# JuliaLinearAlgebra/AlgebraicMultigrid.jl

Measured on AMD Instinct MI355X. Metric: V-cycle unknowns/sec + fine-level SpMV GB/s (% HBM peak), 3-D Poisson 256^3, higher is better.
Workload: dtype f64

## Files before the change

__graft_entry__.py:

```python
import os
import subprocess
import sys

ROOT = os.path.dirname(os.path.abspath(__file__))
PKG = os.path.join(ROOT, "algebraicmultigrid.jl_amd")
if ROOT not in sys.path:
    sys.path.insert(0, ROOT)

HIPCC = os.environ.get("HIPCC", "/opt/rocm/bin/hipcc")
HIP_FLAGS = ["--offload-arch=gfx950", "-O3", "-std=c++17", "-ffp-contract=off", "-fPIC", "-shared",
             "-pthread", "-Wall", "-Wno-unused-value", "-Wno-unused-result"] + os.environ.get("AMGH_EXTRA_HIP_FLAGS", "").split()
CXX_FLAGS = ["-O3", "-std=c++17", "-fopenmp", "-fPIC", "-shared", "-Wall", "-Wextra"]


def _stale(out, srcs):
    if not os.path.exists(out):
        return True
    t = os.path.getmtime(out)
    return any(os.path.getmtime(s) > t for s in srcs)


def build(only_missing=False):
    hip_src = [os.path.join(PKG, "csrc", "hip", f) for f in ("amghip.hip", "amghip_kernels.hpp", "amghip_internal.hpp",
                                                             "gs_schedule.hpp", "csr_ops.hpp")]
    hip_src.append(os.path.join(PKG, "csrc", "hip", "amghip_dist.hpp"))
    hip_src.append(os.path.join(PKG, "csrc", "hip", "amghip_ipc.hpp"))
    hip_src.append(os.path.join(PKG, "csrc", "hip", "amghip_setup.hpp"))
    hip_src.append(os.path.join(PKG, "csrc", "hip", "dev_scan.hpp"))
    hip_src.append(os.path.join(PKG, "csrc", "hip", "gs_merge_dev.hpp"))
    hip_src.append(os.path.join(PKG, "csrc", "hip", "gs_blocks.hpp"))
    hip_src.append(os.path.join(PKG, "csrc", "hip", "gs_flow.hpp"))
    hip_src.append(os.path.join(PKG, "csrc", "hip", "gs_relay.hpp"))
    hip_src.append(os.path.join(PKG, "csrc", "hip", "gmres_kernels.hpp"))
    hip_src.append(os.path.join(PKG, "csrc", "hip", "pcg_block_kernels.hpp"))
    hip_src.append(os.path.join(PKG, "csrc", "hip", "chebyshev.hpp"))
    hip_src.append(os.path.join(PKG, "csrc", "hip", "dist_pcg_kernels.hpp"))
    hip_src.append(os.path.join(ROOT, "include", "amghip.h"))
    hip_out = os.path.join(PKG, "libamghip.so")
    if _stale(hip_out, hip_src) and not (only_missing and os.path.exists(hip_out) and not os.path.exists(HIPCC)):
        extra = os.environ.get("AMGH_EXTRA_HIP_FLAGS", "").split()
        if extra:
            for tool in ("flow_asm_audit.py", "flow_asm_linear.py"):
                r = subprocess.run([sys.executable, os.path.join(ROOT, "tools", tool)], env=dict(os.environ, AUDIT_HIP_FLAGS=" ".join(extra)),
                                   stdout=subprocess.PIPE, stderr=subprocess.STDOUT)
                if r.returncode != 0:
                    raise RuntimeError("AMGH_EXTRA_HIP_FLAGS=%r: tools/%s does not pass with these flags:\n%s" % (" ".join(extra), tool, r.stdout.decode(errors="replace")[-2000:]))
        subprocess.check_call([HIPCC] + HIP_FLAGS + [hip_src[0], "-o", hip_out])
    f32_out = os.path.join(PKG, "libamghip_f32.so")
    if _stale(f32_out, hip_src) and not (only_missing and os.path.exists(f32_out) and not os.path.exists(HIPCC)):
        subprocess.check_call([HIPCC] + HIP_FLAGS + ["-DAMGH_REAL=float", "-DAMGH_NO_SETUP", hip_src[0], "-o", f32_out])
    set_src = [os.path.join(PKG, "csrc", "setup", "amg_setup.cpp"), os.path.join(ROOT, "include", "amgsetup.h")]
    set_out = os.path.join(PKG, "libamgsetup.so")
    if _stale(set_out, set_src):
        subprocess.check_call(["g++"] + CXX_FLAGS + [set_src[0], "-o", set_out])
    tool_src = os.path.join(ROOT, "tools", "spmv_bench.hip")
    tool_out = os.path.join(ROOT, "tools", "spmv_bench")
    if os.path.exists(tool_src) and _stale(tool_out, [tool_src, hip_src[1]]) and os.path.exists(HIPCC):
        subprocess.check_call([HIPCC, "--offload-arch=gfx950", "-O3", "-std=c++17", "-ffp-contract=off", tool_src,
                               "-o", tool_out])
    from oracle import oracle as O
    O.build()
    import amg_amd
    amg_amd.setup_lib()
    amg_amd.hip_lib()
    amg_amd.hip_lib("float32")


def smoke():
    import numpy as np
    build(only_missing=True)
    import amg_amd as AMG
    from oracle import oracle as O
    if not AMG.gpu_available():
        raise RuntimeError("smoke(): no HIP device visible")
    A = AMG.poisson((24, 24, 24))
    b = A @ np.ones(A.m)
    ml = AMG.ruge_stuben(A)
    x, hist = AMG._solve(ml, b, log=True)
    xo, ho, _ = O.OracleHierarchy(ml).solve(b)
    err = np.linalg.norm(x - xo) / np.linalg.norm(xo)
    assert len(hist) == len(ho) and err < 1e-10, (len(hist), len(ho), err)
    jac = AMG.Jacobi(2.0 / 3.0)
    ml2 = AMG.smoothed_aggregation(AMG.poisson((64, 64)), presmoother=jac, postsmoother=jac)
    r = np.linspace(0.0, 1.0, ml2.levels[0].A.m)
    z = AMG.aspreconditioner(ml2).ldiv(r)
    zo = O.OracleHierarchy(ml2).precond(r)
    err2 = np.linalg.norm(z - zo) / np.linalg.norm(zo)
    assert err2 < 1e-10, err2
    print(f"smoke ok: RS/GS solve {len(hist) - 1} cycles rel.err {err:.2e}; SA/Jacobi ldiv rel.err {err2:.2e}")


if __name__ == "__main__":
    build()
    if len(sys.argv) > 1 and sys.argv[1] == "smoke":
        smoke()
```

algebraicmultigrid.jl_amd/_libs.py:

```python
import ctypes as C
import os

_HERE = os.path.dirname(os.path.abspath(__file__))
SETUP_SO = os.path.join(_HERE, "libamgsetup.so")
HIP_SO = os.path.join(_HERE, "libamghip.so")
HIP_F32_SO = os.path.join(_HERE, "libamghip_f32.so")

i32p = C.POINTER(C.c_int32)
f64p = C.POINTER(C.c_double)
i64 = C.c_int64
vp = C.c_void_p


class AMGError(RuntimeError):
    pass


class amgs_options(C.Structure):
    _fields_ = [("theta", C.c_double), ("max_levels", C.c_int32), ("max_coarse", C.c_int32),
                ("hermitian", C.c_int32), ("sa_omega", C.c_double), ("sa_improve_iters", C.c_int32),
                ("sa_B_is_vector", C.c_int32)]


class amgh_smoother_t(C.Structure):
# ... 11 lines not shown

def setup_lib():
    global _setup
    if _setup is not None:
        return _setup
    if not os.path.exists(SETUP_SO):
        raise AMGError(f"{SETUP_SO} not built: run `python -c 'import __graft_entry__ as g; g.build()'`")
    L = C.CDLL(SETUP_SO)
    L.amgs_last_error.restype = C.c_char_p
    L.amgs_set_threads.argtypes = [C.c_int]
    L.amgs_set_threads_here.argtypes = [C.c_int]
    L.amgs_mat_create.restype = vp
    L.amgs_mat_create.argtypes = [i64, i64, vp, vp, vp]
    L.amgs_mat_alloc.restype = vp
    L.amgs_mat_alloc.argtypes = [i64, i64, i64]
    L.amgs_mat_free.argtypes = [vp]
    for f in ("amgs_mat_rows", "amgs_mat_cols", "amgs_mat_nnz"):
        getattr(L, f).restype = i64
        getattr(L, f).argtypes = [vp]
    for f in ("amgs_mat_colptr", "amgs_mat_rowval", "amgs_mat_nzval"):
        getattr(L, f).restype = vp
        getattr(L, f).argtypes = [vp]
    L.amgs_mat_transpose.restype = vp
    L.amgs_mat_transpose.argtypes = [vp]
    L.amgs_mat_spgemm.restype = vp
    L.amgs_mat_spgemm.argtypes = [vp, vp]
    L.amgs_mat_is_symmetric.argtypes = [vp]
    L.amgs_poisson.restype = vp
    L.amgs_poisson.argtypes = [C.c_int, C.POINTER(i64)]
    L.amgs_classical_strength.argtypes = [vp, C.c_double, C.POINTER(vp), C.POINTER(vp)]
    L.amgs_symmetric_strength.restype = vp
    L.amgs_symmetric_strength.argtypes = [vp, C.c_double, C.c_int]
    L.amgs_rs_splitting.argtypes = [vp, vp]
    L.amgs_rs_cf_splitting_patterns.argtypes = [i64, vp, vp, vp, vp, vp]
    L.amgs_direct_interpolation.restype = vp
    L.amgs_direct_interpolation.argtypes = [vp, vp, vp]
    L.amgs_standard_aggregation.restype = vp
    L.amgs_standard_aggregation.argtypes = [vp]
    L.amgs_fit_candidates.restype = vp
    L.amgs_fit_candidates.argtypes = [vp, vp, C.c_int, C.c_int, C.c_double, C.POINTER(vp), C.POINTER(i64)]
    L.amgs_jacobi_prolongation.restype = vp
    L.amgs_jacobi_prolongation.argtypes = [vp, vp, C.c_double]
    L.amgs_improve_candidates.argtypes = [vp, vp, C.c_int, C.c_int]
    L.amgs_free.argtypes = [vp]
    L.amgs_default_options_rs.argtypes = [C.POINTER(amgs_options)]
    L.amgs_default_options_sa.argtypes = [C.POINTER(amgs_options)]
    L.amgs_ruge_stuben.restype = vp
    L.amgs_ruge_stuben.argtypes = [vp, C.POINTER(amgs_options)]
    L.amgs_smoothed_aggregation.restype = vp
    L.amgs_smoothed_aggregation.argtypes = [vp, vp, C.c_int, C.POINTER(amgs_options)]
    L.amgs_hier_free.argtypes = [vp]
    L.amgs_hier_num_levels.argtypes = [vp]
    L.amgs_hier_get.restype = vp
    L.amgs_hier_get.argtypes = [vp, C.c_int, C.c_int]
    _setup = L
    return L


def _bind_solve_phase(L, creal, coarse_fn):
    L.amgh_strerror.restype = C.c_char_p
    L.amgh_strerror.argtypes = [C.c_int]
    L.amgh_create.argtypes = [C.POINTER(vp), C.c_int, C.c_int]
    L.amgh_destroy.argtypes = [vp]
    L.amgh_destroy.restype = None
    L.amgh_push_level.argtypes = [vp, i64, i64] + [vp] * 12 + [C.POINTER(amgh_smoother_t), C.POINTER(amgh_smoother_t)]
    L.amgh_push_level_begin.argtypes = [vp, i64] + [vp] * 6 + [C.POINTER(amgh_smoother_t), C.POINTER(amgh_smoother_t)]
    L.amgh_push_level_end.argtypes = [vp, i64] + [vp] * 6
    L.amgh_push_level_abort.argtypes = [vp]
    L.amgh_level_prepare.argtypes = [C.c_int, i64] + [vp] * 6 + [C.POINTER(amgh_smoother_t), C.POINTER(amgh_smoother_t), C.POINTER(vp)]
    L.amgh_level_prepare_nrhs.argtypes = [C.c_int, C.c_int, i64] + [vp] * 6 + [C.POINTER(amgh_smoother_t), C.POINTER(amgh_smoother_t), C.POINTER(vp)]
    L.amgh_push_level_prepared.argtypes = [vp, vp]
    L.amgh_level_free.argtypes = [vp]
    L.amgh_level_free.restype = None
    L.amgh_set_coarse.argtypes = [vp, i64, vp, vp, vp, vp]
    L.amgh_set_coarse_host.argtypes = [vp, i64, vp, vp, vp, coarse_fn, vp]
    L.amgh_finalize.argtypes = [vp]
    L.amgh_set_chebyshev_bounds.argtypes = [vp, C.c_int, C.c_int, C.c_double, C.c_double, C.c_int]
    L.amgh_chebyshev_bounds.argtypes = [vp, C.c_int, C.c_int, f64p, f64p]
    L.amgh_chebyshev_coefficients.argtypes = [C.c_int, C.c_double, C.c_double, vp]
    L.amgh_level_spectral_radius.argtypes = [vp, C.c_int, C.c_int, f64p]
    L.amgh_csr_spectral_radius.argtypes = [vp, C.c_int, f64p, vp]
    L.amgh_csr_chebyshev_d.argtypes = [vp, C.c_int, C.c_double, C.c_double, vp, vp, vp, vp]
    L.amgh_num_levels.argtypes = [vp]
    L.amgh_tail_dense_build.argtypes = [vp, C.c_int]
    L.amgh_tail_dense_info.argtypes = [vp, C.c_int, C.POINTER(C.c_int), C.POINTER(i64), C.POINTER(C.c_double)]
    L.amgh_level_size.restype = i64
    L.amgh_level_size.argtypes = [vp, C.c_int]
    L.amgh_device_bytes.restype = i64
    L.amgh_device_bytes.argtypes = [vp]
    L.amgh_device_bytes_detail.argtypes = [vp, vp]
    L.amgh_gs_num_dependency_levels.argtypes = [vp, C.c_int]
    L.amgh_gs_num_sweep_steps.argtypes = [vp, C.c_int, C.c_int]
    L.amgh_gs_sweep_stats.argtypes = [vp, C.c_int, C.c_int, vp]
    solve_args = [vp, vp, vp, C.c_int, C.c_int, C.c_double, C.c_double, C.c_int, vp, C.POINTER(C.c_int)]
    L.amgh_solve.argtypes = solve_args
    L.amgh_solve_d.argtypes = solve_args
    L.amgh_precond_apply.argtypes = [vp, vp, vp, C.c_int]
    L.amgh_precond_apply_d.argtypes = [vp, vp, vp, C.c_int]
    pcg_args = [vp, vp, vp, C.c_int, C.c_int, C.c_int, C.c_double, C.c_double, vp, C.POINTER(C.c_int)]
    L.amgh_pcg.argtypes = pcg_args
    L.amgh_pcg_d.argtypes = pcg_args
    gmres_args = [vp, vp, vp, C.c_int, C.c_int, C.c_int, C.c_int, C.c_double, C.c_double, vp, C.POINTER(C.c_int)]
    L.amgh_gmres.argtypes = gmres_args
    L.amgh_gmres_d.argtypes = gmres_args
    L.amgh_debug_gmres_reorth.argtypes = [vp]
    pcg_block_args = [vp, vp, vp, C.c_int, C.c_int, C.c_int, C.c_double, C.c_double, vp, C.c_int, vp]
    L.amgh_pcg_block.argtypes = pcg_block_args
    L.amgh_pcg_block_d.argtypes = pcg_block_args
    L.amgh_level_spmv.argtypes = [vp, C.c_int, C.c_int, vp, vp]
    L.amgh_level_spmv_d.argtypes = [vp, C.c_int, C.c_int, vp, vp]
    L.amgh_level_residual_d.argtypes = [vp, C.c_int, vp, vp, vp]
    L.amgh_level_smooth.argtypes = [vp, C.c_int, C.c_int, vp, vp]
    L.amgh_level_smooth_d.argtypes = [vp, C.c_int, C.c_int, vp, vp]
    L.amgh_debug_level_smooth_block_d.argtypes = [vp, C.c_int, C.c_int, vp, vp]
    L.amgh_csr_create.argtypes = [C.POINTER(vp), C.c_int, i64, i64, vp, vp, vp]
    L.amgh_csr_destroy.argtypes = [vp]
    L.amgh_csr_destroy.restype = None
    L.amgh_csr_prepare.argtypes = [vp, C.c_int, C.c_int]
    L.amgh_csr_spmv_d.argtypes = [vp, vp, vp, vp]
    L.amgh_csr_residual_d.argtypes = [vp, vp, vp, vp, vp]
    L.amgh_csr_spmv_add_d.argtypes = [vp, vp, vp, vp]
    L.amgh_csr_jacobi_d.argtypes = [vp, C.c_double, vp, vp, vp, vp]
    L.amgh_csr_gs_d.argtypes = [vp, C.c_int, C.c_double, C.c_int, vp, vp, vp]
    L.amgh_csr_gs_ex_d.argtypes = [vp, C.c_int, C.c_double, C.c_int, vp, vp, vp, C.c_int]
    L.amgh_gather_d.argtypes = [C.c_int, i64, vp, vp, vp, vp]
    L.amgh_dot_d.argtypes = [C.c_int, i64, vp, vp, vp, C.POINTER(creal), vp]
    L.amgh_cycle_d.argtypes = [vp, C.c_int, vp, vp, C.c_int]
    L.amgh_set_stream.argtypes = [vp, vp]
    L.amgh_dev_alloc.argtypes = [C.c_int, i64, C.POINTER(vp)]
    L.amgh_dev_free.argtypes = [C.c_int, vp]
    L.amgh_dev_upload.argtypes = [C.c_int, vp, vp, i64]
    L.amgh_dev_download.argtypes = [C.c_int, vp, vp, i64]
    L.amgh_dev_sync.argtypes = [C.c_int]
    L.amgh_stream.restype = vp
    L.amgh_stream.argtypes = [vp]
    L.amgh_timer_begin.argtypes = [vp]
    L.amgh_timer_end.argtypes = [vp, C.POINTER(C.c_double)]
    L.amgh_bench_op.argtypes = [vp, C.c_int, C.c_int, C.c_int, C.c_int, C.POINTER(C.c_double)]
    L.amgh_debug_chain_timing.argtypes = [C.c_int, vp]
    L.amgh_debug_merged_sweep_host.argtypes = [i64, i64, vp, vp, vp, C.c_int, C.c_int, C.c_double, vp, vp]
    L.amgh_debug_bw_poll_giveups.argtypes = [vp, C.c_int]
    L.amgh_debug_bw_mode.argtypes = [vp, C.c_int]
    L.amgh_debug_bw_dict.argtypes = [vp, C.c_int]
    L.amgh_debug_bw_late.argtypes = [vp, C.c_int]
    L.amgh_debug_coded_ops.argtypes = [vp, C.c_int]
    L.amgh_debug_set_sell_stream.argtypes = [C.c_int, i64, C.c_int]
    L.amgh_debug_sell_stream_launches.argtypes = [vp, C.c_int, C.c_int]
    L.amgh_debug_sell_stream_padded.argtypes = [vp, C.c_int, C.c_int]
    L.amgh_debug_sell_stream_padded.restype = i64
    L.amgh_debug_csr_sell.argtypes = [vp, C.c_int]
    L.amgh_debug_csr_sell.restype = i64
    L.amgh_debug_csr_sell_launches.argtypes = [vp]
    L.amgh_debug_csr_sell_apply.argtypes = [vp, C.c_int, vp, vp, vp]
    L.amgh_debug_bw_sweep_host.argtypes = [i64, vp, vp, vp, C.c_int, C.c_int, C.c_double, vp, vp, vp]
    L.amgh_debug_bw_dict_sweep_host.argtypes = [i64, vp, vp, vp, C.c_int, C.c_int, vp, vp, vp]
    L.amgh_debug_set_tunable.argtypes = [C.c_char_p, C.c_int]
    L.amgh_debug_get_tunable.argtypes = [C.c_char_p, C.POINTER(C.c_int)]
    L.amgh_profile_enable.argtypes = [vp, C.c_int]
    L.amgh_profile_read.argtypes = [vp, vp, C.c_int]
    L.amgh_set_use_graph.argtypes = [vp, C.c_int]


def _bind_dist(L):
    i64p = C.POINTER(i64)
    L.amgh_dist_rccl_available.argtypes = []
    L.amgh_dist_unique_id.argtypes = [vp]
    L.amgh_dist_create_rccl.argtypes = [C.POINTER(vp), C.c_int, C.c_int, C.c_int, vp]
    L.amgh_local_group_create.argtypes = [C.POINTER(vp), C.c_int]
    L.amgh_local_group_destroy.argtypes = [vp]
    L.amgh_local_group_destroy.restype = None
    L.amgh_local_group_abort.argtypes = [vp]
    L.amgh_local_group_abort.restype = None
    L.amgh_dist_create_local.argtypes = [C.POINTER(vp), C.c_int, C.c_int, vp]
    L.amgh_dist_create_ipc.argtypes = [C.POINTER(vp), C.c_int, C.c_int, C.c_int, C.c_char_p]
    L.amgh_dist_destroy.argtypes = [vp]
    L.amgh_dist_destroy.restype = None
    L.amgh_dist_push_level.argtypes = [vp, i64, i64, vp, vp] + [vp] * 12 + [C.POINTER(amgh_smoother_t),
                                                                            C.POINTER(amgh_smoother_t)]
    L.amgh_dist_set_tail.argtypes = [vp, vp]
    L.amgh_dist_set_host_tail.argtypes = [vp, vp, vp]
    L.amgh_dist_finalize.argtypes = [vp]
    L.amgh_dist_set_gs_mode.argtypes = [vp, C.c_int]
    L.amgh_dist_gs_pipelined.argtypes = [vp, C.c_int]
    L.amgh_dist_pipe_serialized.argtypes = [vp]
    L.amgh_dist_pipe_protocol_failed.argtypes = [vp]
    L.amgh_dist_num_sharded_levels.argtypes = [vp]
    L.amgh_dist_local_range.argtypes = [vp, C.c_int, i64p, i64p]
    L.amgh_dist_precond_apply_d.argtypes = [vp, vp, vp, C.c_int]
    L.amgh_dist_solve_d.argtypes = [vp, vp, vp, C.c_int, C.c_int, C.c_double, C.c_double, C.c_int, vp, C.POINTER(C.c_int)]
    L.amgh_dist_pcg_d.argtypes = [vp, vp, vp, C.c_int, C.c_int, C.c_int, C.c_double, C.c_double, vp, C.POINTER(C.c_int)]
    L.amgh_dist_spmv_d.argtypes = [vp, C.c_int, vp, vp]
    L.amgh_dist_sync.argtypes = [vp]
    L.amgh_dist_barrier.argtypes = [vp]
    L.amgh_dist_allreduce.argtypes = [vp, vp, C.c_int, C.c_int]
    L.amgh_dist_stats.argtypes = [vp, vp, C.c_int]
    L.amgh_dist_device_bytes.restype = i64
    L.amgh_dist_device_bytes.argtypes = [vp]
    L.amgh_dist_stream.restype = vp
    L.amgh_dist_stream.argtypes = [vp]
    L.amgh_dist_plan_info.argtypes = [vp, C.c_int, vp, vp, vp, vp, vp]
    L.amgh_dist_plan_info2.argtypes = [vp, C.c_int, C.c_int, vp, vp, vp, vp, vp]


def hip_lib(dtype=None):
    global _hip
    if dtype is not None and _np_dtype(dtype).itemsize == 4:
        return hip_lib_f32()
    if _hip is not None:
        return _hip
    if not os.path.exists(HIP_SO):
        raise AMGError(f"{HIP_SO} not built: run `python -c 'import __graft_entry__ as g; g.build()'` "
                       "(the solve phase has no CPU fallback)")
    L = C.CDLL(HIP_SO)
    L.real_dtype = "float64"
    _bind_solve_phase(L, C.c_double, COARSE_FN)
    _bind_dist(L)
    L.amgh_dmat_upload.argtypes = [C.POINTER(vp), C.c_int, i64, i64, vp, vp, vp]
    L.amgh_dmat_download.argtypes = [vp, vp, vp, vp]
    L.amgh_dmat_free.argtypes = [vp]
    L.amgh_dmat_free.restype = None
    for f in ("amgh_dmat_rows", "amgh_dmat_cols", "amgh_dmat_nnz"):
        getattr(L, f).restype = i64
        getattr(L, f).argtypes = [vp]
    L.amgh_setup_transpose.argtypes = [vp, C.POINTER(vp)]
    L.amgh_dmat_equal.argtypes = [vp, vp, C.POINTER(C.c_int)]
    L.amgh_setup_classical_strength.argtypes = [vp, C.c_double, C.POINTER(vp), C.POINTER(vp), C.POINTER(vp), C.POINTER(vp)]
    L.amgh_setup_symmetric_strength.restype = C.c_int
    L.amgh_setup_symmetric_strength.argtypes = [vp, C.c_double, C.c_int, C.POINTER(vp)]
    L.amgh_setup_fit_candidates_vector.restype = C.c_int
    L.amgh_setup_fit_candidates_vector.argtypes = [vp, vp, C.c_double, C.POINTER(vp), vp]
    L.amgh_setup_direct_interpolation.argtypes = [vp, vp, vp, C.POINTER(vp), C.POINTER(vp)]
    L.amgh_setup_spgemm.argtypes = [vp, vp, C.POINTER(vp)]
    L.amgh_setup_jacobi_prolongation.argtypes = [vp, vp, C.c_double, C.POINTER(vp)]
    _hip = L
    return L


def _np_dtype(dtype):
    import numpy as np
    return np.dtype(dtype)


def hip_lib_f32():
    global _hip_f32
    if _hip_f32 is not None:
        return _hip_f32
    if not os.path.exists(HIP_F32_SO):
        raise AMGError(f"{HIP_F32_SO} not built: run `python -c 'import __graft_entry__ as g; g.build()'` "
                       "(the solve phase has no CPU fallback)")
    L = C.CDLL(HIP_F32_SO)
    L.real_dtype = "float32"
    _bind_solve_phase(L, C.c_float, COARSE_FN_F32)
    _bind_dist(L)
    _hip_f32 = L
    return L


def hip_check(rc, what=""):
    if rc != 0:
        msg = hip_lib().amgh_strerror(rc).decode()
        raise AMGError(f"libamghip: {what}: {msg} (rc={rc})")


def gpu_available():
    try:
        return hip_lib().amgh_device_count() > 0
    except (AMGError, OSError):
        return False
```

algebraicmultigrid.jl_amd/csrc/hip/amghip.hip:

```cpp
#include "amghip_internal.hpp"
#include "gs_schedule.hpp"
#include "csr_ops.hpp"
#include "chebyshev.hpp"
#include "gmres_kernels.hpp"
#include "pcg_block_kernels.hpp"
#include "dist_pcg_kernels.hpp"

namespace {

constexpr int64_t kGraphAutoRows = 65536;

struct Level {
  int64_t n = 0, nc = 0;
  amgh_csr A, S, P, R;
  bool has_S = false;
  amgh_smoother_t pre{}, post{};
  real *res = nullptr, *cx = nullptr, *cb = nullptr, *tmp = nullptr;
  real* cheb_d = nullptr;
  ChebSide cheb[2];
  const ChebSide& cheb_of(const amgh_smoother_t& s) const { return &s == &post ? cheb[1] : cheb[0]; }
  real* il = nullptr;
  amgh_csr* smat() { return has_S ? &S : &A; }
  amgh_csr Pp, Rp;
  bool lo_ok = false;
// ... 1178 lines not shown
  if ((post ? L->post : L->pre).kind != AMGH_SMOOTH_CHEBYSHEV) return AMGH_EINVAL;
  if (lo) *lo = L->cheb[post].lo;
  if (hi) *hi = L->cheb[post].hi;
  return AMGH_OK;
}

int amgh_chebyshev_coefficients(int degree, double lo, double hi, double* c1c2) {
  if (degree < 1 || degree > kChebMaxDegree || !c1c2 || !cheb_bounds_valid(lo, hi)) return AMGH_EINVAL;
  cheb_coefficients(degree, lo, hi, c1c2);
  return AMGH_OK;
}

int amgh_level_spectral_radius(amgh_t* h, int level, int steps, double* rho) {
  RC_TRY(check_ready(h));
  if (level < 0 || level >= (int)h->levels.size() || !rho || steps < 0) return AMGH_EINVAL;
  HIP_TRY(hipSetDevice(h->device));
  amgh_csr* M = h->levels[level]->smat();
  if (!M->rowptr || !M->col || !M->val) return AMGH_EINVAL;
  return csr_spectral_radius(M, steps ? steps : kLanczosSteps, 0, h->stream, rho);
}

int amgh_csr_spectral_radius(amgh_csr_t* op, int steps, double* rho, void* stream) {
  if (!op || !rho || steps < 0) return AMGH_EINVAL;
  HIP_TRY(hipSetDevice(op->device));
  return csr_spectral_radius(op, steps ? steps : kLanczosSteps, 0, (hipStream_t)stream, rho);
}

int amgh_csr_chebyshev_d(amgh_csr_t* op, int degree, double lo, double hi, real* x_d, const real* b_d, real* work_d, void* stream) {
  if (!op || !x_d || !b_d || !work_d || op->nrows != op->ncols) return AMGH_EINVAL;
  if (degree < 1 || degree > kChebMaxDegree || !cheb_bounds_valid(lo, hi)) return AMGH_EINVAL;
  HIP_TRY(hipSetDevice(op->device));
  hipStream_t st = (hipStream_t)stream;
  RC_TRY(csr_ensure_coded(op, st));
  double c[2 * kChebMaxDegree];
  cheb_coefficients(degree, lo, hi, c);
  const int64_t n = op->nrows;
  real *xc = x_d, *xo = work_d, *d = work_d + n;
  for (int k = 0; k < degree; ++k) {
    RC_TRY(csr_chebyshev(op, (real)c[2 * k], (real)c[2 * k + 1], k == 0, xc, b_d, d, xo, st));
    std::swap(xc, xo);
  }
  if (xc != x_d) HIP_TRY(hipMemcpyAsync(x_d, xc, sizeof(real) * n, hipMemcpyDeviceToDevice, st));
  return AMGH_OK;
}

int amgh_finalize(amgh_t* h) {
  if (!h) return AMGH_EINVAL;
  if (h->finalized || h->ncoarse < 0 || h->pending_level) return AMGH_ESTATE;
  if (h->levels.empty() && !h->has_finalA) return AMGH_ESTATE;
  HIP_TRY(hipSetDevice(h->device));
  for (Level* L : h->levels)
    if (L->pre.kind == AMGH_SMOOTH_CHEBYSHEV || L->post.kind == AMGH_SMOOTH_CHEBYSHEV) RC_TRY(level_chebyshev_setup(h, L));
  int64_t ws = 0;
  h->tail_level = -2;
  if (g_tail_dense_rows > 0 && !h->coarse_fn)
    for (size_t l = 0; l < h->levels.size(); ++l)
      if (h->levels[l]->n <= g_tail_dense_rows) { h->tail_level = (int)l; break; }
  if (h->tail_level >= 0) {
    h->tail_cols = 64;
    h->tail_lo = h->tail_level >= 1 && h->levels[h->tail_level - 1]->coarse_lo;
  }
  for (size_t l = 0; l < h->levels.size(); ++l) {
    Level* L = h->levels[l];
    const int64_t wc = (h->tail_level >= 0 && (int)l >= h->tail_level) ? std::max(h->nrhs, h->tail_cols) : h->nrhs;
    RC_TRY(dev_alloc(&L->res, L->n * wc));
    RC_TRY(dev_alloc(&L->cx, L->nc * wc));
    RC_TRY(dev_alloc(&L->cb, L->nc * wc));
    ws += kRealB * (L->n + 2 * L->nc) * wc;
    if (h->nrhs == 2 || h->nrhs == 4 || h->nrhs == 8 || h->nrhs == 16) {
      RC_TRY(dev_alloc(&L->il, std::max(L->n, L->nc) * h->nrhs));
      ws += kRealB * std::max(L->n, L->nc) * h->nrhs;
    }
    const bool cheb = L->pre.kind == AMGH_SMOOTH_CHEBYSHEV || L->post.kind == AMGH_SMOOTH_CHEBYSHEV;
    if (L->pre.kind == AMGH_SMOOTH_JACOBI || L->post.kind == AMGH_SMOOTH_JACOBI || cheb) {
      RC_TRY(dev_alloc(&L->tmp, L->n * wc));
      ws += kRealB * L->n * wc;
      RC_TRY(csr_ensure_diag(L->smat(), h->stream));
    }
    if (cheb) {
      RC_TRY(dev_alloc(&L->cheb_d, L->n * wc));
      ws += kRealB * L->n * wc;
    }
  }
  for (Level* L : h->levels) {
    GsSchedule* g = L->smat()->gs;
    if (!L->lo_ok || !g || g->nblk != 0 || !g->rowptr || g->compacted) continue;
    RC_TRY(code_values(g->col, L->lo_val ? L->lo_val : g->val, L->n, g->ncols, g->nnz, &L->lo_cc, h->stream));
    RC_TRY(code_values(L->Rp.col, L->Rp.val, L->Rp.nrows, L->Rp.ncols, L->Rp.nnz, &L->Rp.cc, h->stream));
    RC_TRY(code_values(L->Pp.col, L->Pp.val, L->Pp.nrows, L->Pp.ncols, L->Pp.nnz, &L->Pp.cc, h->stream));
    ws += L->lo_cc.bytes + L->Rp.cc.bytes + L->Pp.cc.bytes;
    if (L->il && il_block(h->nrhs) && g_rhs_il == 1) {
      const int bs = h->nrhs;
      const int64_t n = L->n, nc = L->nc;
      auto timed = [&](auto&& fn, double* ms) -> int {
        hipEvent_t e0, e1;
        if (hipEventCreate(&e0) != hipSuccess) return -1001;
        if (hipEventCreate(&e1) != hipSuccess) { hipEventDestroy(e0); return -1001; }
        int rc = fn();
        if (rc == AMGH_OK && hipEventRecord(e0, h->stream) != hipSuccess) rc = -1001;
        for (int r = 0; r < 2 && rc == AMGH_OK; ++r) rc = fn();
        float t = 0.f;
        if (rc == AMGH_OK && (hipEventRecord(e1, h->stream) != hipSuccess || hipEventSynchronize(e1) != hipSuccess ||
                              hipEventElapsedTime(&t, e0, e1) != hipSuccess)) rc = -1001;
        hipEventDestroy(e0); hipEventDestroy(e1);
        *ms = t;
        return rc;
      };
      if (L->Rp.cc.ccol) {
        double t_il = 0, t_st = 0;
        RC_TRY(hipMemsetAsync(L->res, 0, sizeof(real) * n * bs, h->stream) == hipSuccess ? AMGH_OK : -1001);
        RC_TRY(timed([&] { return il_apply(bs, false, L->Rp.rowptr, L->Rp.col, L->Rp.val, nc, L->res, n, n, L->il, L->cb, nc, h->stream, &L->Rp.cc); }, &t_il));
        RC_TRY(timed([&] { return csr_apply(&L->Rp, M_SPMV, L->res, nullptr, L->cb, h->stream, bs); }, &t_st));
        L->r_stream = t_st < 0.95 * t_il;
        if (getenv("AMGH_VERBOSE")) fprintf(stderr, "[amghip] n=%lld restriction of %d columns: interleaved %.3f ms, column by column %.3f ms\n", (long long)n, bs, t_il / 2, t_st / 2);
      }
      if (L->Pp.cc.ccol) {
        double t_il = 0, t_st = 0;
        RC_TRY(hipMemsetAsync(L->cx, 0, sizeof(real) * nc * bs, h->stream) == hipSuccess ? AMGH_OK : -1001);
        RC_TRY(hipMemsetAsync(L->res, 0, sizeof(real) * n * bs, h->stream) == hipSuccess ? AMGH_OK : -1001);
        RC_TRY(timed([&] { return il_apply(bs, true, L->Pp.rowptr, L->Pp.col, L->Pp.val, n, L->cx, nc, nc, L->il, L->res, n, h->stream, &L->Pp.cc); }, &t_il));
        RC_TRY(timed([&] { return raw_apply(M_ADD, L->Pp.rowptr, L->Pp.col, L->Pp.val, n, L->cx, nc, nullptr, 0, L->res, n, h->stream, bs, &L->Pp.cc); }, &t_st));
        L->p_stream = t_st < 0.95 * t_il;
        if (getenv("AMGH_VERBOSE")) fprintf(stderr, "[amghip] n=%lld prolongation of %d columns: interleaved %.3f ms, column by column %.3f ms\n", (long long)n, bs, t_il / 2, t_st / 2);
      }
    }
  }
  if (h->nrhs == 1)
    for (Level* L : h->levels) {
      if (!L->lo_ok || !L->Rp.rowptr || L->Rp.nrows < (1 << 18)) continue;
      if (hipMemsetAsync(L->res, 0, sizeof(real) * L->n, h->stream) != hipSuccess) return -1001;
      double ms[2] = {0, 0};
      int rc = AMGH_OK;
      for (int v = 0; v < 2 && rc == AMGH_OK; ++v) {
        L->Rp.xcd_map = v == 1;
        rc = csr_apply(&L->Rp, M_SPMV, L->res, nullptr, L->cb, h->stream, 1);
        if (rc == AMGH_OK && hipEventRecord(h->t0, h->stream) != hipSuccess) rc = -1001;
        for (int r = 0; r < 4 && rc == AMGH_OK; ++r) rc = csr_apply(&L->Rp, M_SPMV, L->res, nullptr, L->cb, h->stream, 1);
        float t = 0.f;
        if (rc == AMGH_OK && (hipEventRecord(h->t1, h->stream) != hipSuccess || hipEventSynchronize(h->t1) != hipSuccess ||
                              hipEventElapsedTime(&t, h->t0, h->t1) != hipSuccess)) rc = -1001;
        ms[v] = t;
      }
      L->Rp.xcd_map = false;
      RC_TRY(rc);
      L->Rp.xcd_map = ms[1] < 0.93 * ms[0];
      if (getenv("AMGH_VERBOSE")) fprintf(stderr, "[amghip] n=%lld restriction: %.3f ms, XCD-contiguous %.3f ms -> %s\n", (long long)L->n, ms[0] / 4, ms[1] / 4, L->Rp.xcd_map ? "XCD-contiguous" : "plain");
    }
  if (h->nrhs == 1)
    for (Level* L : h->levels) {
      GsSchedule* g = L->smat()->gs;
      const bool cd = g_stream_code != 0;
      if (!(L->lo_ok && g && g->nblk == 0)) {
        for (amgh_csr* M : {&L->A, &L->R, &L->P})
          if (M->rowptr) { RC_TRY(sell_build(M->rowptr, cd ? M->cc.ccol : nullptr, M->col, M->val, M->nrows, M->nnz, &M->sc, h->stream)); ws += M->sc.bytes; }
        continue;
      }
      if (!g->rowptr || g->compacted) continue;
      RC_TRY(sell_build(g->rowptr, cd ? L->lo_cc.ccol : nullptr, g->col, L->lo_val ? L->lo_val : g->val, L->n, g->nnz, &L->lo_sc, h->stream));
      RC_TRY(sell_build(L->Rp.rowptr, cd ? L->Rp.cc.ccol : nullptr, L->Rp.col, L->Rp.val, L->Rp.nrows, L->Rp.nnz, &L->Rp.sc, h->stream));
      RC_TRY(sell_build(L->Pp.rowptr, cd ? L->Pp.cc.ccol : nullptr, L->Pp.col, L->Pp.val, L->Pp.nrows, L->Pp.nnz, &L->Pp.sc, h->stream));
      if (L->n >= (1 << 18) && g_sell_min_rows >= ((int64_t)1 << 18)) {
        real* ty = nullptr;
        RC_TRY(dev_alloc(&ty, L->n));
        int rc = AMGH_OK;
        if (hipMemsetAsync(ty, 0, sizeof(real) * L->n, h->stream) != hipSuccess || hipMemsetAsync(L->res, 0, sizeof(real) * L->n, h->stream) != hipSuccess ||
            hipMemsetAsync(L->cx, 0, sizeof(real) * L->nc, h->stream) != hipSuccess) rc = -1001;
        const real* val = L->lo_val ? L->lo_val : g->val;
        auto run = [&](int which) -> int {
          if (which == AMGH_OP_A) return raw_apply(M_RESID, g->rowptr, g->col, val, L->n, L->res, L->n, L->res, L->n, ty, L->n, h->stream, 1, &L->lo_cc, &L->lo_sc);
          if (which == AMGH_OP_R) return csr_apply(&L->Rp, M_SPMV, L->res, nullptr, L->cb, h->stream, 1, true);
          return raw_apply(M_ADD, L->Pp.rowptr, L->Pp.col, L->Pp.val, L->n, L->cx, L->nc, nullptr, 0, ty, L->n, h->stream, 1, &L->Pp.cc, &L->Pp.sc);
        };
        const int keep = g_sell_stream;
        for (int which : {AMGH_OP_A, AMGH_OP_R, AMGH_OP_P}) {
          SellCols* sc = which == AMGH_OP_A ? &L->lo_sc : which == AMGH_OP_R ? &L->Rp.sc : &L->Pp.sc;
          if (!sc->w || (which == AMGH_OP_R ? L->Rp.nrows : L->n) < (1 << 18)) continue;
          double ms[2] = {0, 0};
          for (int v = 0; v < 2 && rc == AMGH_OK; ++v) {
            g_sell_stream = v;
            rc = run(which);
            if (rc == AMGH_OK && hipEventRecord(h->t0, h->stream) != hipSuccess) rc = -1001;
            for (int r = 0; r < 4 && rc == AMGH_OK; ++r) rc = run(which);
            float t = 0.f;
            if (rc == AMGH_OK && (hipEventRecord(h->t1, h->stream) != hipSuccess || hipEventSynchronize(h->t1) != hipSuccess ||
                                  hipEventElapsedTime(&t, h->t0, h->t1) != hipSuccess)) rc = -1001;
            ms[v] = t;
          }
          sc->launches = 0;
          if (rc != AMGH_OK) break;
          if (getenv("AMGH_VERBOSE")) fprintf(stderr, "[amghip] n=%lld operator %d: csr_stream_kernel %.3f ms, sliced-ELL %.3f ms\n", (long long)L->n, which, ms[0] / 4, ms[1] / 4);
          if (!(ms[1] < 0.97 * ms[0])) sc->free_dev();
        }
        g_sell_stream = keep;
        if (hipStreamSynchronize(h->stream) != hipSuccess && rc == AMGH_OK) rc = -1001;
        hipFree(ty);
        RC_TRY(rc);
      }
      ws += L->lo_sc.bytes + L->Rp.sc.bytes + L->Pp.sc.bytes;
      if (getenv("AMGH_VERBOSE"))
        fprintf(stderr, "[amghip] n=%lld sliced-ELL padded / entries: A %.3f  R %.3f  P %.3f (0: not taken)\n", (long long)L->n, (double)L->lo_sc.padded / std::max<int64_t>(1, g->nnz),
                (double)L->Rp.sc.padded / std::max<int64_t>(1, L->Rp.nnz), (double)L->Pp.sc.padded / std::max<int64_t>(1, L->Pp.nnz));
    }
  if (gs_trim() && g_stream_code && g_trim_coded) {
    HIP_TRY(hipStreamSynchronize(h->stream));
    for (Level* L : h->levels) {
      for (amgh_csr* M : {&L->Rp, &L->Pp})
        if (M->cc.ccol && M->col && M->val) {
          hipFree(M->col); hipFree(M->val); M->col = nullptr; M->val = nullptr;
          M->bytes -= M->nnz * kEntB;
        }
      amgh_csr* S = L->smat();
      GsSchedule* g = S->gs;
      if (L->lo_cc.ccol && g && g->bw.on && g->bw.flow.on && !g->bw.rec && g->segs.empty() && !g->mf && !g->mb && g->col && g->val) {
        hipFree(g->col); hipFree(g->val); g->col = nullptr; g->val = nullptr;
        int64_t freed = g->nnz * kEntB;
        if (L->lo_val) { hipFree(L->lo_val); L->lo_val = nullptr; }
        g->csr_bytes -= freed; g->bytes -= freed; S->bytes -= freed;
      }
    }
  }
  for (size_t l = 0; l + 1 < h->levels.size(); ++l)
    if (h->levels[l]->coarse_lo) RC_TRY(gs_ensure_cols(h->levels[l + 1]->smat(), h->nrhs, h->stream));
  const int64_t n = fine_n(h);
  if (h->levels.empty()) { RC_TRY(dev_alloc(&h->res_final, n * h->nrhs)); ws += kRealB * n * h->nrhs; }
  RC_TRY(dev_alloc(&h->partial, kRedBlocks));
  RC_TRY(dev_alloc(&h->scal, 8));
  RC_TRY(dev_alloc(&h->x0, n * h->nrhs));
  RC_TRY(dev_alloc(&h->b0, n * h->nrhs));
  ws += 2 * kRealB * n * h->nrhs;
  h->ws_bytes = ws;
  if (h->graph_auto && !h->levels.empty() && getenv("AMGH_GRAPH_AUTO") && getenv("AMGH_GRAPH_AUTO")[0] == '1') {
    int64_t widest = 0;
    for (Level* L : h->levels) widest = std::max(widest, L->n);
    h->use_graph = widest <= kGraphAutoRows;
  }
  HIP_TRY(hipStreamSynchronize(h->stream));
  h->finalized = true;
  return AMGH_OK;
}

int amgh_num_levels(const amgh_t* h) { return h ? (int)h->levels.size() : 0; }
int amgh_tail_dense_build(amgh_t* h, int cycle_) {
  RC_TRY(check_ready(h));
  if (cycle_ < 0 || cycle_ > 2) return AMGH_EINVAL;
  HIP_TRY(hipSetDevice(h->device));
  if (!g_tail_dense || h->tail_level < 0) return AMGH_OK;
  RC_TRY(tail_dense_build(h, cycle_));
  if (cycle_ == AMGH_CYCLE_F) RC_TRY(tail_dense_build(h, AMGH_CYCLE_V));
  return AMGH_OK;
}
int amgh_tail_dense_info(const amgh_t* h, int cycle_, int* level, int64_t* rows, double* build_ms) {
  if (!h || cycle_ < 0 || cycle_ > 2) return AMGH_EINVAL;
  const bool on = h->finalized && h->tail_level >= 0 && h->tail[cycle_].built;
  if (level) *level = on ? h->tail_level : -1;
  if (rows) *rows = on ? h->levels[h->tail_level]->n : 0;
  if (build_ms) *build_ms = h->tail_build_ms;
  return AMGH_OK;
}
int64_t amgh_level_size(const amgh_t* h, int l) {
  if (!h || l < 0 || l > (int)h->levels.size()) return -1;
  return l == (int)h->levels.size() ? h->ncoarse : h->levels[l]->n;
}
int64_t amgh_device_bytes(const amgh_t* h) {
  if (!h) return 0;
  int64_t b = h->ws_bytes + ((h->ncoarse > 0 && h->coarse_op) ? h->ncoarse * h->ncoarse * kRealB : 0) + h->finalA.bytes;
  for (Level* L : h->levels) b += L->A.bytes + L->S.bytes + L->P.bytes + L->R.bytes + L->Pp.bytes + L->Rp.bytes;
  return b;
}
int amgh_device_bytes_detail(const amgh_t* h, int64_t* out8) {
  if (!h || !out8) return AMGH_EINVAL;
  for (int q = 0; q < 8; ++q) out8[q] = 0;
  for (Level* L : h->levels) {
    for (const amgh_csr* op : {&L->A, &L->S, &L->P, &L->R})
      if (op->rowptr) out8[0] += (op->nrows + 1) * 4 + op->nnz * kEntB;
    out8[1] += L->Pp.bytes + L->Rp.bytes;
    const GsSchedule* g = L->smat()->gs;
    if (!g) continue;
    out8[1] += g->csr_bytes;
    out8[2] += g->slot_bytes;
    int64_t known = g->csr_bytes + g->slot_bytes;
    for (const GsSchedule* c : {g->mf, g->mb})
      if (c) { out8[3] += c->csr_bytes; out8[4] += c->bytes - c->csr_bytes; known += c->bytes; }
    const int64_t tri = (g->tri_nnz + g->tri_nnz_b) * kEntB + ((g->tri_nnz ? 1 : 0) + (g->tri_nnz_b ? 1 : 0)) * (g->n + 1) * 4;
    out8[5] += tri;
    known += tri;
    out8[6] += std::max<int64_t>(0, g->bytes - known);
  }
  out8[0] += h->finalA.bytes;
  out8[7] = h->ws_bytes + ((h->ncoarse > 0 && h->coarse_op) ? h->ncoarse * h->ncoarse * kRealB : 0);
  return AMGH_OK;
}
int amgh_debug_bw_poll_giveups(const amgh_t* h, int l) {
  if (!h || l < 0 || l >= (int)h->levels.size()) return -1;
  amgh_csr* M = h->levels[l]->smat();
  const GsSchedule* g = M->gs;
  if (!g || !g->bw.on || !g->bw.err) return -1;
  if (hipSetDevice(h->device) != hipSuccess || hipDeviceSynchronize() != hipSuccess) return -1;
  return (int)*(volatile int32_t*)g->bw.err;
}
int amgh_debug_bw_mode(const amgh_t* h, int l) {
  if (!h || l < 0 || l >= (int)h->levels.size()) return -1;
  amgh_csr* M = h->levels[l]->smat();
  const GsSchedule* g = M->gs;
  if (!g || !g->bw.on) return 0;
  if (g->bw.flow.on && (g_gs_bw_flow || !g->bw.rec)) return 3;
  return (g_gs_bw_chain && g->bw.flags) ? 2 : 1;
}
int amgh_debug_bw_dict(const amgh_t* h, int l) {
  if (!h || l < 0 || l >= (int)h->levels.size()) return -1;
  const GsSchedule* g = h->levels[l]->smat()->gs;
  return g && g->bw.on && g->bw.flow.on && g->bw.flow.dict_on && (g_gs_bw_dict || !g->bw.flow.srec) && (g_gs_bw_flow || !g->bw.rec) ? 1 : 0;
}
int amgh_debug_bw_late(const amgh_t* h, int l) {
  if (!h || l < 0 || l >= (int)h->levels.size()) return -1;
  const GsSchedule* g = h->levels[l]->smat()->gs;
  return g && g->bw.on && g->bw.flow.on && g->bw.flow.late_ok && !g_gs_bw_inorder && g_gs_bw_relay > 0 && h->nrhs == 1 && (g_gs_bw_flow || !g->bw.rec) ? 1 : 0;
}
int amgh_debug_coded_ops(const amgh_t* h, int l) {
  if (!h || l < 0 || l >= (int)h->levels.size()) return -1;
  const Level* L = h->levels[l];
  const GsSchedule* g = (L->has_S ? L->S : L->A).gs;
  const bool a_on = L->lo_cc.ccol && (g_stream_code || (g && !g->col));
  const bool r_on = L->Rp.cc.ccol && (g_stream_code || !L->Rp.col), p_on = L->Pp.cc.ccol && (g_stream_code || !L->Pp.col);
  const amgh_csr& M = L->has_S ? L->S : L->A;
  const bool s_on = M.cc.ccol && (g_stream_code || !M.col);
  return (a_on ? 1 : 0) | (r_on ? 2 : 0) | (p_on ? 4 : 0) | (s_on ? 8 : 0);
}
int amgh_gs_num_dependency_levels(const amgh_t* h, int l) {
  if (!h || l < 0 || l >= (int)h->levels.size()) return -1;
  amgh_csr* M = h->levels[l]->smat();
  return M->gs ? M->gs->nlev : 0;
}
int amgh_gs_num_sweep_steps(const amgh_t* h, int l, int backward) {
  if (!h || l < 0 || l >= (int)h->levels.size()) return -1;
  amgh_csr* M = h->levels[l]->smat();
  const GsSchedule* g = M->gs;
  if (!g) return 0;
  if (g->dti_f && g_gs_dense_tri && g_gs_block_inverse) return (int)g->dti_off.size() - 1;
  if (g->nblk > 0 && g_gs_block_inverse) return g->nblk;
  if (g->bw.on) return (int)g->bw.launch_ptr.size() - 1;
  const GsSchedule* c = backward ? g->mb : g->mf;
  return (c && g_gs_merge > 1) ? c->nlev : g->nlev;
}

int amgh_gs_sweep_stats(const amgh_t* h, int l, int backward, int64_t* out6) {
  if (!h || l < 0 || l >= (int)h->levels.size() || !out6) return AMGH_EINVAL;
  for (int q = 0; q < 6; ++q) out6[q] = 0;
  amgh_csr* M = h->levels[l]->smat();
  const GsSchedule* g = M->gs;
  if (!g) return AMGH_OK;
  if (g->dti_f && g_gs_dense_tri && g_gs_block_inverse) {
// ... 761 lines not shown
  }
  for (int64_t p = 0; p < n; ++p) x[P.perm[p]] = xp[p];
  return AMGH_OK;
}

int amgh_debug_merged_sweep_host(int64_t nrows, int64_t ncols, const int32_t* rowptr, const int32_t* col,
                                 const real* val, int m, int backward, double omega, real* x, const real* b) {
  if (nrows < 0 || ncols < nrows || !rowptr || m < 1 || !x || !b || omega == 0.0) return AMGH_EINVAL;
  const int64_t n = nrows;
  HostLevelCsr base;
  std::vector<int32_t> perm;
  level_order(n, ncols, rowptr, col, val, base, perm);
  HostLevelCsr scaled = base;
  for (real& dd : scaled.pdiag) dd /= omega;
  const real shift = (1.0 - omega) / omega;
  MergeResult R = merge_build(scaled, ncols, m, backward != 0);
  if (R.max_row > kBigSlot) return AMGH_EUNSUPPORTED;
  const HostLevelCsr& S = R.sys;
  std::vector<real> ext(ncols + n);
  for (int64_t c = 0; c < ncols; ++c) ext[c] = c < n ? x[perm[c]] : x[c];
  std::vector<int32_t> lev_of(n);
  for (int l = 0; l < base.nlev; ++l)
    for (int32_t p = base.lvl_ptr[l]; p < base.lvl_ptr[l + 1]; ++p) lev_of[p] = l;
  for (int64_t p = 0; p < n; ++p) {
    real s = b[perm[p]];
    for (int32_t j = base.prow[p]; j < base.prow[p + 1]; ++j) {
      const int32_t c = base.pcol[j];
      if (c == p) continue;
      const bool other = c >= n || (backward ? lev_of[c] < lev_of[p] : lev_of[c] > lev_of[p]);
      if (other) s -= base.pval[j] * ext[c];
    }
    if (base.pdiag[p] != 0.0) s += shift * base.pdiag[p] * ext[p];
    ext[ncols + p] = s;
  }
  for (int k = 0; k < S.nlev; ++k) {
    const int q = backward ? S.nlev - 1 - k : k;
    std::vector<real> xn(S.lvl_ptr[q + 1] - S.lvl_ptr[q]);
    for (int32_t p = S.lvl_ptr[q]; p < S.lvl_ptr[q + 1]; ++p) {
      real acc = 0.0;
      for (int32_t j = S.prow[p]; j < S.prow[p + 1]; ++j) acc += S.pval[j] * ext[S.pcol[j]];
      xn[p - S.lvl_ptr[q]] = S.pdiag[p] != 0.0 ? (ext[ncols + p] - acc) / S.pdiag[p] : ext[p];
    }
    for (int32_t p = S.lvl_ptr[q]; p < S.lvl_ptr[q + 1]; ++p) ext[p] = xn[p - S.lvl_ptr[q]];
  }
  for (int64_t p = 0; p < n; ++p) x[perm[p]] = ext[p];
  return S.nlev;
}

int amgh_debug_set_tunable(const char* name, int value) {
  if (!name) return AMGH_EINVAL;
  if (!strcmp(name, "gs_block_inverse")) g_gs_block_inverse = value;
  else if (!strcmp(name, "gs_lpr")) g_gs_lpr = value;
  else if (!strcmp(name, "gs_il")) g_gs_il = value;
  else if (!strcmp(name, "trim_coded")) g_trim_coded = value;
  else if (!strcmp(name, "gs_wave_quad")) g_gs_wave_quad = value;
  else if (!strcmp(name, "pcg_fused")) g_pcg_fused = value;
  else if (!strcmp(name, "tail_dense_rows")) g_tail_dense_rows = value < 0 ? 0 : value;
  else if (!strcmp(name, "tail_dense")) { g_tail_dense = value; g_sched_epoch++; }
  else if (!strcmp(name, "gs_lean")) g_gs_lean = value;
  else if (!strcmp(name, "gs_sell")) g_gs_sell = value;
  else if (!strcmp(name, "gs_tiny")) g_gs_tiny = value;
  else if (!strcmp(name, "gs_bw")) g_gs_bw = value;
  else if (!strcmp(name, "gs_bw_rows")) g_gs_bw_rows = value;
  else if (!strcmp(name, "gs_bw_chain")) g_gs_bw_chain = value;
  else if (!strcmp(name, "gs_bw_flow")) g_gs_bw_flow = value;
  else if (!strcmp(name, "gs_bw_spin")) g_gs_bw_spin = value;
  else if (!strcmp(name, "gs_bw_nc")) g_gs_bw_nc = value;
  else if (!strcmp(name, "gs_bw_nrhs")) g_gs_bw_nrhs = value;
  else if (!strcmp(name, "gs_bw_skip_pub")) g_gs_bw_skip_pub = value;
  else if (!strcmp(name, "gs_bw_two_min_rows")) g_gs_bw_two_min_rows = value;
  else if (!strcmp(name, "gs_flow_xzero")) g_gs_flow_xzero = value;
  else if (!strcmp(name, "gs_bw_dict")) g_gs_bw_dict = value != 0;
  else if (!strcmp(name, "gs_bw_inorder")) g_gs_bw_inorder = value != 0;
  else if (!strcmp(name, "stream_code")) g_stream_code = value != 0;
  else if (!strcmp(name, "gs_bw_relay")) g_gs_bw_relay = value == 0 ? 0 : BW_RELAY_W;
  else if (!strcmp(name, "rhs_il")) g_rhs_il = value;
  else if (!strcmp(name, "jacobi_zero")) g_jacobi_zero = value;
  else if (!strcmp(name, "gs_ept")) g_gs_ept = value;
  else if (!strcmp(name, "gs_merge")) g_gs_merge = value;
  else if (!strcmp(name, "gs_coarse_lo")) g_gs_coarse_lo = value;
  else if (!strcmp(name, "gs_dense_tri")) g_gs_dense_tri = value;
  else if (!strcmp(name, "gs_dense_blk")) g_gs_dense_blk = value;
  else if (!strcmp(name, "gs_bigslot")) g_gs_bigslot = value;
  else if (!strcmp(name, "gs_super")) g_gs_super = value;
  else if (!strcmp(name, "gs_block_pipe")) g_gs_block_pipe = value;
  else return AMGH_EINVAL;
  ++g_sched_epoch;
  return AMGH_OK;
}

int amgh_debug_get_tunable(const char* name, int* value) {
  if (!name || !value) return AMGH_EINVAL;
  if (!strcmp(name, "gs_block_inverse")) *value = g_gs_block_inverse;
  else if (!strcmp(name, "gs_lpr")) *value = g_gs_lpr;
  else if (!strcmp(name, "gs_il")) *value = g_gs_il;
  else if (!strcmp(name, "trim_coded")) *value = g_trim_coded;
  else if (!strcmp(name, "gs_wave_quad")) *value = g_gs_wave_quad;
  else if (!strcmp(name, "pcg_fused")) *value = g_pcg_fused;
  else if (!strcmp(name, "tail_dense_rows")) *value = g_tail_dense_rows;
  else if (!strcmp(name, "tail_dense")) *value = g_tail_dense;
  else if (!strcmp(name, "gs_lean")) *value = g_gs_lean;
  else if (!strcmp(name, "gs_sell")) *value = g_gs_sell;
  else if (!strcmp(name, "gs_tiny")) *value = g_gs_tiny;
  else if (!strcmp(name, "gs_bw")) *value = g_gs_bw;
  else if (!strcmp(name, "gs_bw_rows")) *value = g_gs_bw_rows;
  else if (!strcmp(name, "gs_bw_chain")) *value = g_gs_bw_chain;
  else if (!strcmp(name, "gs_bw_flow")) *value = g_gs_bw_flow;
  else if (!strcmp(name, "gs_bw_spin")) *value = g_gs_bw_spin;
  else if (!strcmp(name, "gs_bw_nc")) *value = g_gs_bw_nc;
  else if (!strcmp(name, "gs_bw_nrhs")) *value = g_gs_bw_nrhs;
  else if (!strcmp(name, "gs_bw_skip_pub")) *value = g_gs_bw_skip_pub;
  else if (!strcmp(name, "gs_bw_two_min_rows")) *value = g_gs_bw_two_min_rows;
  else if (!strcmp(name, "gs_flow_xzero")) *value = g_gs_flow_xzero;
  else if (!strcmp(name, "gs_bw_dict")) *value = g_gs_bw_dict;
  else if (!strcmp(name, "gs_bw_inorder")) *value = g_gs_bw_inorder;
  else if (!strcmp(name, "stream_code")) *value = g_stream_code;
  else if (!strcmp(name, "gs_bw_relay")) *value = g_gs_bw_relay;
  else if (!strcmp(name, "rhs_il")) *value = g_rhs_il;
  else if (!strcmp(name, "jacobi_zero")) *value = g_jacobi_zero;
  else if (!strcmp(name, "gs_ept")) *value = g_gs_ept;
  else if (!strcmp(name, "gs_merge")) *value = g_gs_merge;
  else if (!strcmp(name, "gs_coarse_lo")) *value = g_gs_coarse_lo;
  else if (!strcmp(name, "gs_dense_tri")) *value = g_gs_dense_tri;
  else if (!strcmp(name, "gs_dense_blk")) *value = g_gs_dense_blk;
  else if (!strcmp(name, "gs_bigslot")) *value = g_gs_bigslot;
  else if (!strcmp(name, "gs_super")) *value = g_gs_super;
  else if (!strcmp(name, "gs_block_pipe")) *value = g_gs_block_pipe;
  else return AMGH_EINVAL;
  return AMGH_OK;
}

int amgh_debug_set_perm_io(int on) {
  g_gs_flow_perm_io = on != 0;
  ++g_sched_epoch;
  return AMGH_OK;
}
int amgh_debug_get_perm_io(void) { return g_gs_flow_perm_io; }
int amgh_debug_perm_io_sweeps(int which) { return (which == 0 || which == 1) ? (int)(g_perm_io_sweeps[which] & 0x7fffffffu) : -1; }

int amgh_debug_set_sell_stream(int on, int64_t min_rows, int cap_pct) {
  g_sell_stream = on != 0;
  g_sell_min_rows = min_rows > 0 ? min_rows : (int64_t)1 << 18;
  g_sell_cap_pct = cap_pct > 0 ? cap_pct : 0;
  ++g_sched_epoch;
  return AMGH_OK;
}
int amgh_debug_get_sell_stream(void) { return g_sell_stream; }
static const SellCols* sell_of(const amgh_t* h, int level, int which) {
  if (!h || level < 0 || level >= (int)h->levels.size()) return nullptr;
  const Level* L = h->levels[level];
  const GsSchedule* g = (L->has_S ? L->S : L->A).gs;
  if (!(L->lo_ok && g && g->nblk == 0))
    return which == AMGH_OP_A ? &L->A.sc : which == AMGH_OP_R ? &L->R.sc : which == AMGH_OP_P ? &L->P.sc : nullptr;
  return which == AMGH_OP_A ? &L->lo_sc : which == AMGH_OP_R ? &L->Rp.sc : which == AMGH_OP_P ? &L->Pp.sc : nullptr;
}
int amgh_debug_sell_stream_launches(const amgh_t* h, int level, int which) {
  const SellCols* sc = sell_of(h, level, which);
  return sc ? (int)(sc->launches & 0x7fffffffu) : -1;
}
int64_t amgh_debug_sell_stream_padded(const amgh_t* h, int level, int which) {
  const SellCols* sc = sell_of(h, level, which);
  return sc ? (sc->w ? sc->padded : 0) : -1;
}

int64_t amgh_debug_csr_sell(amgh_csr_t* op, int coded) {
  if (!op) return AMGH_EINVAL;
  HIP_TRY(hipSetDevice(op->device));
  if (coded && !op->cc.ccol) {
    RC_TRY(code_values(op->col, op->val, op->nrows, op->ncols, op->nnz, &op->cc, nullptr, 1));
    op->bytes += op->cc.bytes;
  }
  RC_TRY(sell_build(op->rowptr, coded ? op->cc.ccol : nullptr, op->col, op->val, op->nrows, op->nnz, &op->sc, nullptr));
  op->bytes += op->sc.bytes;
  return op->sc.w ? op->sc.padded : 0;
}
int amgh_debug_csr_sell_apply(amgh_csr_t* op, int mode, const real* x_d, const real* b_d, real* y_d) {
  if (!op || !x_d || !y_d || mode < M_SPMV || mode > M_ADD || (mode == M_RESID && !b_d)) return AMGH_EINVAL;
  HIP_TRY(hipSetDevice(op->device));
  RC_TRY(csr_apply(op, mode, x_d, b_d, y_d, nullptr, 1, true));
  HIP_TRY(hipDeviceSynchronize());
  return AMGH_OK;
}
int amgh_debug_csr_sell_launches(const amgh_csr_t* op) { return op ? (int)(op->sc.launches & 0x7fffffffu) : -1; }

int amgh_debug_chain_timing(int enable, unsigned long long* out8) {
  if (enable && !g_chain_tim) {
    HIP_TRY(hipMalloc((void**)&g_chain_tim, 8 * sizeof(unsigned long long)));
    HIP_TRY(hipMemset(g_chain_tim, 0, 8 * sizeof(unsigned long long)));
  }
  if (out8 && g_chain_tim) {
    HIP_TRY(hipDeviceSynchronize());
    HIP_TRY(hipMemcpy(out8, g_chain_tim, 8 * sizeof(unsigned long long), hipMemcpyDeviceToHost));
    HIP_TRY(hipMemset(g_chain_tim, 0, 8 * sizeof(unsigned long long)));
  }
  if (!enable && g_chain_tim) { hipFree(g_chain_tim); g_chain_tim = nullptr; }
  return AMGH_OK;
}

int amgh_profile_enable(amgh_t* h, int on) {
  if (!h) return AMGH_EINVAL;
  h->profile = on != 0;
  return AMGH_OK;
}
int amgh_profile_read(amgh_t* h, double* out, int reset) {
  if (!h || !out) return AMGH_EINVAL;
  RC_TRY(prof_flush(h));
  const int L1 = (int)h->levels.size() + 1;
  if ((int)h->prof_ms.size() != AMGH_T_COUNT * L1) h->prof_ms.assign(AMGH_T_COUNT * L1, 0.0);
  std::copy(h->prof_ms.begin(), h->prof_ms.end(), out);
  if (reset) std::fill(h->prof_ms.begin(), h->prof_ms.end(), 0.0);
  return AMGH_OK;
}
int amgh_set_use_graph(amgh_t* h, int on) {
  if (!h) return AMGH_EINVAL;
  h->use_graph = on != 0;
  h->graph_auto = false;
  return AMGH_OK;
}

}

#include "amghip_dist.hpp"
#ifndef AMGH_NO_SETUP
#include "amghip_setup.hpp"
#endif
```

algebraicmultigrid.jl_amd/csrc/hip/amghip_internal.hpp:

```cpp
#pragma once
#include "amghip_kernels.hpp"
#include "gs_blocks.hpp"
#include "gs_flow.hpp"

#include <algorithm>
#include <chrono>
#include <cmath>
#include <cstdio>
#include <cstring>
#include <atomic>
#include <mutex>
#include <string>
#include <system_error>
#include <thread>
#include <utility>
#include <vector>

#include "../../../include/amghip.h"

using namespace amgh;

#define HIP_TRY(expr)                                   \
  do {                                                  \
    hipError_t e_ = (expr);                             \
    if (e_ != hipSuccess) return -(1000 + (int)e_);     \
  } while (0)
#define RC_TRY(expr)            \
  do {                          \
    int rc_ = (expr);           \
    if (rc_ != AMGH_OK) return rc_; \
  } while (0)

namespace {

constexpr int64_t kRealB = (int64_t)sizeof(real);
constexpr int64_t kEntB = 4 + (int64_t)sizeof(real);

template <class T>
int dev_alloc(T** p, int64_t count) {
  *p = nullptr;
  if (count <= 0) count = 1;
  hipError_t e = hipMalloc((void**)p, sizeof(T) * (size_t)count);
  if (e == hipErrorOutOfMemory) return AMGH_ENOMEM;
  if (e != hipSuccess) return -(1000 + (int)e);
  return AMGH_OK;
}
struct StageLane {
  hipStream_t stream = nullptr;
  void* buf[2] = {nullptr, nullptr};
  hipEvent_t ev[2] = {nullptr, nullptr};
};
struct StageSet {
  int device = -1;
  std::vector<StageLane> lanes;
};
constexpr size_t kStagePiece = size_t(8) << 20;
constexpr int kStageLanes = 8;
inline std::mutex& stage_mutex() { static std::mutex m; return m; }
inline std::vector<StageSet*>& stage_pool() { static std::vector<StageSet*> p; return p; }

inline StageSet* stage_acquire(int device) {
  {
    std::lock_guard<std::mutex> lk(stage_mutex());
    auto& pool = stage_pool();
    for (size_t i = 0; i < pool.size(); ++i)
      if (pool[i]->device == device) { StageSet* s = pool[i]; pool.erase(pool.begin() + i); return s; }
  }
  StageSet* s = new StageSet;
  s->device = device;
  s->lanes.resize(kStageLanes);
  bool ok = true;
  for (StageLane& L : s->lanes) {
    ok = ok && hipStreamCreateWithFlags(&L.stream, hipStreamNonBlocking) == hipSuccess;
    for (int k = 0; k < 2; ++k) {
      ok = ok && hipHostMalloc(&L.buf[k], kStagePiece, hipHostMallocDefault) == hipSuccess;
      ok = ok && hipEventCreateWithFlags(&L.ev[k], hipEventDisableTiming) == hipSuccess;
    }
  }
  if (!ok) {
    for (StageLane& L : s->lanes) {
      for (int k = 0; k < 2; ++k) { if (L.buf[k]) hipHostFree(L.buf[k]); if (L.ev[k]) hipEventDestroy(L.ev[k]); }
      if (L.stream) hipStreamDestroy(L.stream);
    }
    delete s;
    return nullptr;
  }
  return s;
}
inline void stage_release(StageSet* s) {
  std::lock_guard<std::mutex> lk(stage_mutex());
  stage_pool().push_back(s);
}

inline hipError_t staged_copy(void* dst, const void* src, size_t bytes, hipMemcpyKind kind) {
  if (bytes < 4 * kStagePiece) return hipMemcpy(dst, src, bytes, kind);
  int device = 0;
  hipError_t e0 = hipGetDevice(&device);
  if (e0 != hipSuccess) return e0;
  StageSet* set = stage_acquire(device);
  if (!set) { (void)hipGetLastError(); return hipMemcpy(dst, src, bytes, kind); }
  const size_t npiece = (bytes + kStagePiece - 1) / kStagePiece;
  const int T = (int)std::min<size_t>(kStageLanes, npiece / 2);
  std::vector<hipError_t> err(T, hipSuccess);
  auto lane_fn = [&](int t) {
    hipSetDevice(device);
    StageLane& L = set->lanes[t];
    const size_t p0 = npiece * t / T, p1 = npiece * (t + 1) / T;
    auto piece_len = [&](size_t p) { return std::min(kStagePiece, bytes - p * kStagePiece); };
    hipError_t e = hipSuccess;
    if (kind == hipMemcpyDeviceToHost) {
      if (p0 < p1) {
        e = hipMemcpyAsync(L.buf[0], (const char*)src + p0 * kStagePiece, piece_len(p0), kind, L.stream);
        if (e == hipSuccess) e = hipEventRecord(L.ev[0], L.stream);
      }
      for (size_t p = p0; p < p1 && e == hipSuccess; ++p) {
        const int k = (int)((p - p0) & 1);
        if (p + 1 < p1) {
          e = hipMemcpyAsync(L.buf[k ^ 1], (const char*)src + (p + 1) * kStagePiece, piece_len(p + 1), kind, L.stream);
          if (e == hipSuccess) e = hipEventRecord(L.ev[k ^ 1], L.stream);
          if (e != hipSuccess) break;
        }
        e = hipEventSynchronize(L.ev[k]);
        if (e == hipSuccess) std::memcpy((char*)dst + p * kStagePiece, L.buf[k], piece_len(p));
      }
    } else {
      for (size_t p = p0; p < p1 && e == hipSuccess; ++p) {
        const int k = (int)((p - p0) & 1);
        if (p >= p0 + 2) e = hipEventSynchronize(L.ev[k]);
        if (e != hipSuccess) break;
        std::memcpy(L.buf[k], (const char*)src + p * kStagePiece, piece_len(p));
        e = hipMemcpyAsync((char*)dst + p * kStagePiece, L.buf[k], piece_len(p), kind, L.stream);
        if (e == hipSuccess) e = hipEventRecord(L.ev[k], L.stream);
      }
    }
    hipError_t es = hipStreamSynchronize(L.stream);
    err[t] = e != hipSuccess ? e : es;
  };
  {
    std::vector<std::thread> th;
    int started = 0;
    for (; started < T - 1; ++started) {
      try { th.emplace_back(lane_fn, started); } catch (const std::system_error&) { break; }
    }
    for (int t = started; t < T; ++t) lane_fn(t);
    for (auto& x : th) x.join();
  }
  stage_release(set);
  for (hipError_t e : err) if (e != hipSuccess) return e;
  return hipSuccess;
}

inline hipError_t dev_zero(void* p, size_t bytes, hipStream_t st) {
  const size_t piece = size_t(1) << 30;
  for (size_t o = 0; o < bytes; o += piece) {
    const hipError_t e = hipMemsetAsync((char*)p + o, 0, std::min(piece, bytes - o), st);
    if (e != hipSuccess) return e;
  }
  return hipSuccess;
}

inline void dbg_pending(const char* where) {
  if (!getenv("AMGH_VERBOSE")) return;
  const hipError_t e = hipGetLastError();
  if (e != hipSuccess) fprintf(stderr, "[amghip] pending HIP error at %s: %s\n", where, hipGetErrorString(e));
}

template <class T>
int dev_upload(T** p, const T* src, int64_t count) {
  RC_TRY(dev_alloc(p, count));
  if (count > 0) HIP_TRY(staged_copy(*p, src, sizeof(T) * (size_t)count, hipMemcpyHostToDevice));
  return AMGH_OK;
}
inline int grid_for(int64_t n, int threads = 256) {
  int64_t g = (n + threads - 1) / threads;
  return (int)std::max<int64_t>(1, std::min<int64_t>(g, 256 * 8));
}

struct GsSchedule {
  int nlev = 0;
  std::vector<int32_t> lvl_ptr;
  int32_t* d_lvl_ptr = nullptr;
  int32_t* rowptr = nullptr;
  int32_t* col = nullptr;
  real* val = nullptr;
  int32_t* perm = nullptr;
  int32_t* dpos = nullptr;
  real* diag = nullptr;
  bool diag_shared = false;
  bool tiny_ok = false;
  struct Bw {
    bw::Desc* blocks = nullptr; unsigned char* rec = nullptr; int32_t* ext_col = nullptr;
    std::vector<int32_t> launch_ptr;
    size_t lds_max = 0; int maxk = 0;
    int64_t rec_bytes = 0, rec_entries = 0, sum_depth = 0;
    double est_seconds = 0.0;
    int32_t *dep_ptr = nullptr, *dep = nullptr, *sdep_ptr = nullptr, *sdep = nullptr;
    unsigned int* flags = nullptr; unsigned long long* head = nullptr;
    int32_t* err = nullptr;
    int32_t nblocks = 0;
    bool on = false;
    struct FlowDev {
      bw::FlowDesc* fd = nullptr; unsigned char* srec = nullptr; uint32_t* aux = nullptr;
      int32_t* fl_mb = nullptr; uint16_t* fl_slot = nullptr; void* mbox = nullptr;
      int64_t nmail = 0; size_t lds_max = 0; int64_t bytes = 0;
      int64_t mail_stride = 0;
      int mcols = 0;
      bool on = false;
      bool late_ok = false;
      uint32_t* xaux = nullptr; int32_t* xfl_mb = nullptr; uint16_t* xfl_slot = nullptr; int32_t* xlist = nullptr;
      std::vector<int32_t> h_xfl_mb, h_row_cell_f, h_row_cell_b;
      bool xon = false;
      unsigned char* crec = nullptr; unsigned char* dict = nullptr; int32_t* dict_ent = nullptr;
      size_t dict_lds = 0; bool dict_on = false;
    } flow;
  } bw;
  unsigned char* ww_rec = nullptr; int ww_S = 0, ww_maxk = 0, ww_steps = 0; size_t ww_lds = 0;
  unsigned char* wq_rec = nullptr; int wq_E = 0, wq_steps = 0; size_t wq_lds = 0;
  i4_t* rowmeta = nullptr;
  i4_t* desc = nullptr;
  real* bp = nullptr;
  real* xp = nullptr;
  int cols_alloc = 1;
  real* xil = nullptr;
  int64_t xil_cap = 0;
  int xil_cols = 0;
  int bp_cols = 0;
  int32_t* permx = nullptr;
  std::vector<int32_t> h_perm;
  int64_t n = 0, ncols = 0;
  int64_t bytes = 0;
  bool compacted = false;
  int64_t csr_bytes = 0, slot_bytes = 0;
  int64_t nnz = 0;
  int64_t slot_total = 0;
  int64_t tri_nnz = 0;
  int64_t tri_nnz_b = 0;
  struct Seg {
    int l0, l1; bool chain; int rows; int slot0, nslots;
    int sell_k = 0, sell_chunk0 = 0, sell_nchunks = 0;
  };
  std::vector<Seg> segs;
  int32_t* wcol = nullptr; real* wval = nullptr; int32_t* slot_row = nullptr; i4_t* wmeta = nullptr;
  int slot_entries = kSlot;
  int32_t* scol = nullptr; real* sval = nullptr; i2_t* schunk = nullptr;
  int64_t sell_bytes = 0, sell_total = 0;
  struct Outer {
    int32_t* rowptr = nullptr; int32_t* col = nullptr; real* val = nullptr; real* tinv = nullptr;
    int32_t* near_ptr = nullptr; i2_t* near_pi = nullptr; real* near_val = nullptr;
    int32_t* nx_rowptr = nullptr; int32_t* nx_col = nullptr; real* nx_val = nullptr;
    int32_t* sp_rowptr = nullptr; int32_t* sp_col = nullptr; real* sp_val = nullptr;
  };
  Outer blk_f, blk_b;
  real* blk_diag = nullptr;
  real* blk_s = nullptr;
  int nblk = 0;
  int super = 0;
  double blk_cond = 0.0;
  real* dti_f = nullptr;
  real* dti_b = nullptr;
  int dti_B = 0;
  std::vector<int64_t> dti_off;
  double dti_cond = 0.0;
  GsSchedule* mf = nullptr;
  GsSchedule* mb = nullptr;
  struct Tri { int32_t* rowptr = nullptr; int32_t* col = nullptr; real* val = nullptr; };
  Tri dtri_f, dtri_b;
  Tri tri_f, tri_b;
  int merge_f = 1, merge_b = 1;
  int64_t xstride = 0;
  struct SorSet { real omega = 0.0; GsSchedule* f = nullptr; GsSchedule* b = nullptr; Tri tf, tb; bool built = false; };
  SorSet sor[2];
  int sor_next = 0;
  real s_key = 0.0;
  bool diag_nonzero = false;
  int s_dir = -1;
  void free_dev() {
    for (GsSchedule** c : {&mf, &mb})
      if (*c) { (*c)->free_dev(); delete *c; *c = nullptr; }
    for (Tri* t : {&tri_f, &tri_b}) { hipFree(t->rowptr); hipFree(t->col); hipFree(t->val); *t = Tri(); }
    for (SorSet& ss : sor) {
      for (GsSchedule** c : {&ss.f, &ss.b})
        if (*c) { (*c)->free_dev(); delete *c; *c = nullptr; }
      for (Tri* t : {&ss.tf, &ss.tb}) { hipFree(t->rowptr); hipFree(t->col); hipFree(t->val); *t = Tri(); }
      ss = SorSet();
    }
    for (Outer* o : {&blk_f, &blk_b}) {
      hipFree(o->rowptr); hipFree(o->col); hipFree(o->val); hipFree(o->tinv);
      hipFree(o->near_ptr); hipFree(o->near_pi); hipFree(o->near_val);
      hipFree(o->nx_rowptr); hipFree(o->nx_col); hipFree(o->nx_val);
      hipFree(o->sp_rowptr); hipFree(o->sp_col); hipFree(o->sp_val);
      *o = Outer();
    }
    hipFree(dti_f); if (dti_b != dti_f) hipFree(dti_b);
    dti_f = dti_b = nullptr;
    for (Tri* t : {&dtri_f, &dtri_b}) { hipFree(t->rowptr); hipFree(t->col); hipFree(t->val); *t = Tri(); }
    hipFree(blk_diag); blk_diag = nullptr;
    hipFree(blk_s); blk_s = nullptr;
    hipFree(wcol); hipFree(wval); hipFree(slot_row); hipFree(wmeta); wcol = slot_row = nullptr; wval = nullptr; wmeta = nullptr;
    hipFree(scol); hipFree(sval); hipFree(schunk); scol = nullptr; sval = nullptr; schunk = nullptr;
    hipFree(ww_rec); ww_rec = nullptr;
    hipFree(wq_rec); wq_rec = nullptr;
    hipFree(xil); xil = nullptr; xil_cap = 0; xil_cols = 0;
    hipFree(bw.blocks); hipFree(bw.rec); hipFree(bw.ext_col);
    hipFree(bw.dep_ptr); hipFree(bw.dep); hipFree(bw.sdep_ptr); hipFree(bw.sdep); hipFree(bw.flags); hipFree(bw.head);
    hipFree(bw.flow.fd); hipFree(bw.flow.srec); hipFree(bw.flow.aux); hipFree(bw.flow.fl_mb); hipFree(bw.flow.fl_slot); hipFree(bw.flow.mbox);
    hipFree(bw.flow.xaux); hipFree(bw.flow.xfl_mb); hipFree(bw.flow.xfl_slot); hipFree(bw.flow.xlist);
    hipFree(bw.flow.crec); hipFree(bw.flow.dict); hipFree(bw.flow.dict_ent);
    bw = Bw();
    hipFree(d_lvl_ptr); hipFree(rowptr); hipFree(col); hipFree(val);
    hipFree(perm); hipFree(dpos); if (!diag_shared) hipFree(diag);
    hipFree(rowmeta); hipFree(desc); hipFree(bp); hipFree(xp); hipFree(permx);
    d_lvl_ptr = rowptr = col = perm = dpos = nullptr; val = diag = bp = xp = nullptr; rowmeta = desc = nullptr; permx = nullptr;
  }
};

}

#include "dev_scan.hpp"

struct CodedCols {
  uint32_t* ccol = nullptr; real* vtab = nullptr; int n = 0;
  int64_t bytes = 0;
  void free_dev() { hipFree(ccol); hipFree(vtab); ccol = nullptr; vtab = nullptr; n = 0; bytes = 0; }
};

constexpr int kSellCapPct = 130, kSellCapPlainPct = 110;
constexpr int kSellLongSteps = 12;
struct SellCols {
  uint32_t* w = nullptr; real* v = nullptr; uint2* slice = nullptr; uint8_t* len8 = nullptr;
  int64_t nslices = 0, padded = 0, bytes = 0;
  unsigned launches = 0;
  void free_dev() { hipFree(w); hipFree(v); hipFree(slice); hipFree(len8); w = nullptr; v = nullptr; slice = nullptr; len8 = nullptr; nslices = padded = bytes = 0; }
};

struct amgh_csr {
  CodedCols cc;
  SellCols sc;
  bool cc_tried = false;
  bool xcd_map = false;
  int device = 0;
  int64_t nrows = 0, ncols = 0, nnz = 0;
  int32_t* rowptr = nullptr;
  int32_t* col = nullptr;
  real* val = nullptr;
  int32_t* dpos = nullptr;
  real* diag = nullptr;
  GsSchedule* gs = nullptr;
  int gs_nrhs_hint = 0;
  uint32_t pipe_epoch = 0; const void* pipe_rmbox = nullptr; int pipe_grid = 0;
  int64_t bytes = 0;
};

namespace {

int g_gs_block_pipe = 1;
int g_gs_super = 8;
int g_gs_coarse_lo = 1;
int g_gs_bigslot = 1;
int g_gs_merge = 16;
int g_jacobi_zero = 1;
int g_rhs_il = 1;
int g_gs_tiny = 1;
int g_gs_wave_quad = 1;
int g_gs_bw = 1;
int g_gs_bw_rows = 512;
int g_gs_bw_flow = 1;
int g_gs_bw_spin = 0;
int g_gs_bw_skip_pub = -1;
int g_gs_bw_nc = -1;
int g_gs_bw_nrhs = 1;
int g_gs_bw_chain = 1;
int g_stream_code = 1;
int g_trim_coded = 1;
int g_gs_bw_inorder = 0;
int g_gs_bw_dict = 1;
int g_gs_bw_relay = 3;
int g_gs_flow_xzero = 1;
int g_gs_flow_perm_io = 1;
int g_sell_stream = 1;
int64_t g_sell_min_rows = (int64_t)1 << 18;
int g_sell_cap_pct = 0;
unsigned int g_perm_io_sweeps[2] = {0, 0};
int g_gs_bw_two_min_rows = 200000;
int g_gs_sell = 1;
int g_gs_lean = -1;
int g_gs_ept = 0;
int g_gs_lpr = 0;
int g_gs_il = 1;
int g_pcg_fused = 1;
int g_tail_dense_rows = 6144;
int g_tail_dense = 1;
int g_gs_dense_blk = 4096;
int g_gs_dense_tri = 1;
int g_gs_block_inverse = 1;

std::atomic<unsigned long long> g_sched_epoch{0};

unsigned long long* g_chain_tim = nullptr;

constexpr int kChainWidth = 1024;

__global__ void find_diag_kernel(const int32_t* rowptr, const int32_t* col, const real* val, int n,
                                 int32_t* dpos, real* diag) {
  const int i = blockIdx.x * blockDim.x + threadIdx.x;
  if (i >= n) return;
  int dp = -1;
  real d = 0.0;
  for (int j = rowptr[i]; j < rowptr[i + 1]; ++j)
    if (col[j] == i) { dp = j; d = val[j]; }
  dpos[i] = dp;
  diag[i] = d;
}

int csr_upload(amgh_csr* op, int device, int64_t nrows, int64_t ncols, const int32_t* rowptr,
               const int32_t* col, const real* val) {
  if (nrows < 0 || ncols < 0 || !rowptr) return AMGH_EINVAL;
  if (nrows >= INT32_MAX || ncols >= INT32_MAX) return AMGH_EUNSUPPORTED;
  const int64_t nnz = rowptr[nrows];
  if (rowptr[0] != 0 || nnz < 0) return AMGH_EINVAL;
  if (nnz > 0 && (!col || !val)) return AMGH_EINVAL;
  op->device = device;
  op->nrows = nrows;
  op->ncols = ncols;
  op->nnz = nnz;
  RC_TRY(dev_upload(&op->rowptr, rowptr, nrows + 1));
  RC_TRY(dev_upload(&op->col, col, nnz));
  RC_TRY(dev_upload(&op->val, val, nnz));
  op->bytes = (nrows + 1) * 4 + nnz * kEntB;
  return AMGH_OK;
}

void csr_free(amgh_csr* op) {
  if (!op) return;
  hipFree(op->rowptr); hipFree(op->col); hipFree(op->val);
  hipFree(op->dpos); hipFree(op->diag);
  op->cc.free_dev();
  op->sc.free_dev();
  if (op->gs) { op->gs->free_dev(); delete op->gs; }
  op->rowptr = op->col = op->dpos = nullptr; op->val = op->diag = nullptr; op->gs = nullptr;
}

int csr_ensure_diag(amgh_csr* op, hipStream_t st) {
  if (op->dpos) return AMGH_OK;
  const int64_t n = std::min(op->nrows, op->ncols);
  RC_TRY(dev_alloc(&op->dpos, op->nrows));
  RC_TRY(dev_alloc(&op->diag, op->nrows));
  if (n < op->nrows) {
    HIP_TRY(hipMemsetAsync(op->dpos, 0xff, sizeof(int32_t) * op->nrows, st));
    HIP_TRY(hipMemsetAsync(op->diag, 0, sizeof(real) * op->nrows, st));
  }
  if (n > 0)
    hipLaunchKernelGGL(find_diag_kernel, dim3((unsigned)((n + 255) / 256)), dim3(256), 0, st, op->rowptr, op->col,
                       op->val, (int)n, op->dpos, op->diag);
  HIP_TRY(hipGetLastError());
  op->bytes += op->nrows * kEntB;
  return AMGH_OK;
}


}
```

algebraicmultigrid.jl_amd/csrc/hip/amghip_kernels.hpp:

```cpp
#pragma once
#include <hip/hip_runtime.h>
#include <stdint.h>

#ifndef AMGH_REAL
#define AMGH_REAL double
#endif

namespace amgh {

using real = AMGH_REAL;

constexpr int kWave = 64;
constexpr int kThreads = 256;
constexpr int kNumXcd = 8;

enum StreamMode : int {
  M_SPMV = 0,
  M_RESID = 1,
  M_ADD = 2,
  M_JACOBI = 3,
  M_GS = 4,
  M_SOR = 5,
  M_CHEB1 = 6,
  M_CHEB = 7
// ... 121 lines not shown
    __syncthreads();
  }
  constexpr bool SK = CFG::ROWS > 64;
  __shared__ real s_prod[LDSN + (LDSN >> 5) + 2];
  int bid, cv;
  multi_column_block(a.ncolv, bid, cv);
  if (cv > 0) {
    a.x += cv * a.ldx;
    a.y += cv * a.ldy;
    if (a.b) a.b += cv * a.ldb;
    if (MODE >= M_CHEB1) a.d += cv * a.ldd;
  }

  const int nrows = a.row_end - a.row_begin;
  const int nb = (nrows + CFG::ROWS - 1) / CFG::ROWS;
  const int lb = CFG::XCD ? xcd_block(bid, nb) : bid;
  if (lb >= nb) return;
  const int r0 = a.row_begin + lb * CFG::ROWS;
  const int r1 = min(r0 + CFG::ROWS, a.row_end);
  const int tid = threadIdx.x;

  int rs[RPT], re[RPT], dp[RPT], gi[RPT];
  real acc[RPT], gd[RPT], gb[RPT];
#pragma unroll
  for (int q = 0; q < RPT; ++q) {
    const int r = r0 + tid + q * T;
    gi[q] = 0; gd[q] = 0.0; gb[q] = 0.0;
    if (tid + q * T < CFG::ROWS && r < r1) {
      rs[q] = a.rowptr[r];
      re[q] = a.rowptr[r + 1];
      dp[q] = kSkipDiag<MODE> ? a.dpos[r] : -1;
      if (kLevelRows<MODE>) {
        gi[q] = a.perm ? a.perm[r] : r;
        gd[q] = a.diag[r];
        gb[q] = a.b[r];
      }
    } else {
      rs[q] = re[q] = 0;
      dp[q] = -1;
    }
    acc[q] = 0.0;
  }
  const int p0 = a.rowptr[r0];
  const int p1 = a.rowptr[r1];

  for (int c0 = p0; c0 < p1; c0 += LDSN) {
    const int c1 = min(c0 + LDSN, p1);
    if (VEC == 1) {
      for (int k = c0 + tid; k < c1; k += T) {
        const real v = ld_stream<NT>(a.val + k);
        const int c = ld_stream<NT>(a.col + k);
        s_prod[lidx<SK>(k - c0)] = v * a.x[c];
      }
    } else {
      const int a0 = c0 & ~(VEC - 1);
      for (int k = a0 + VEC * tid; k < c1; k += VEC * T) {
        if (k >= c0 && k + VEC <= c1) {
          real v[VEC];
          int c[VEC];
          if (VEC == 2) {
            const d2_t vv = ld_stream<NT>((const d2_t*)(a.val + k));
            const i2_t cc = ld_stream<NT>((const i2_t*)(a.col + k));
            v[0] = vv.x; v[1] = vv.y; c[0] = cc.x; c[1] = cc.y;
          } else if (CODED) {
            const u4_t cc = ld_stream<NT>((const u4_t*)(a.ccol + k));
            c[0] = (int)(cc.x & ((1u << kCodeBits) - 1)); c[1] = (int)(cc.y & ((1u << kCodeBits) - 1));
            c[VEC - 2] = (int)(cc.z & ((1u << kCodeBits) - 1)); c[VEC - 1] = (int)(cc.w & ((1u << kCodeBits) - 1));
            v[0] = s_tab[cc.x >> kCodeBits]; v[1] = s_tab[cc.y >> kCodeBits];
            v[VEC - 2] = s_tab[cc.z >> kCodeBits]; v[VEC - 1] = s_tab[cc.w >> kCodeBits];
          } else {
            const d2_t v0 = ld_stream<NT>((const d2_t*)(a.val + k));
            const d2_t v1 = ld_stream<NT>((const d2_t*)(a.val + k + 2));
            const i4_t cc = ld_stream<NT>((const i4_t*)(a.col + k));
            v[0] = v0.x; v[1] = v0.y; v[VEC - 2] = v1.x; v[VEC - 1] = v1.y;
            c[0] = cc.x; c[1] = cc.y; c[VEC - 2] = cc.z; c[VEC - 1] = cc.w;
          }
          real xv[VEC];
#pragma unroll
          for (int e = 0; e < VEC; ++e) xv[e] = a.x[c[e]];
#pragma unroll
          for (int e = 0; e < VEC; ++e) s_prod[lidx<SK>(k + e - c0)] = v[e] * xv[e];
        } else {
#pragma unroll
          for (int e = 0; e < VEC; ++e) {
            const int kk = k + e;
            if (CODED) {
              if (kk >= c0 && kk < c1) { const unsigned w = a.ccol[kk]; s_prod[lidx<SK>(kk - c0)] = s_tab[w >> kCodeBits] * a.x[w & ((1u << kCodeBits) - 1)]; }
            } else
            if (kk >= c0 && kk < c1) s_prod[lidx<SK>(kk - c0)] = a.val[kk] * a.x[a.col[kk]];
          }
        }
      }
    }
    __syncthreads();
#pragma unroll
    for (int q = 0; q < RPT; ++q) {
      const int lo = max(rs[q], c0), hi = min(re[q], c1);
      if (SK) acc[q] = seq_sum<kSkipDiag<MODE>>(s_prod, lo, hi, c0, dp[q], acc[q]);
      else acc[q] = seq_sum_skip(s_prod, lo - c0, hi - c0, kSkipDiag<MODE> ? dp[q] - c0 : -1, acc[q]);
    }
    if (c1 < p1) __syncthreads();
  }

#pragma unroll
  for (int q = 0; q < RPT; ++q) {
    const int r = r0 + tid + q * T;
    if (tid + q * T >= CFG::ROWS || r >= r1) continue;
    if (MODE == M_SPMV) {
      a.y[r] = acc[q];
    } else if (MODE == M_RESID) {
      a.y[r] = a.b[r] - acc[q];
    } else if (MODE == M_ADD) {
      a.y[r] = a.y[r] + acc[q];
    } else if (MODE == M_JACOBI) {
      const real d = a.diag[r];
      const real t = a.x[r];
      const real cand = (1.0 - a.omega) * t + a.omega * ((a.b[r] - acc[q]) / d);
      a.y[r] = (d == 0.0) ? t : cand;
    } else if (MODE == M_CHEB1 || MODE == M_CHEB) {
      const real dg = a.diag[r];
      const real t = a.x[r];
      real dn = a.c2 * ((a.b[r] - acc[q]) / dg);
      if (MODE == M_CHEB) dn = a.c1 * a.d[r] + dn;
      a.d[r] = (dg == 0.0) ? (real)0.0 : dn;
      a.y[r] = (dg == 0.0) ? t : t + dn;
    } else {
      const int i = gi[q];
      const real d = gd[q];
      if (d != 0.0) {
        if (MODE == M_GS) {
          a.y[i] = (gb[q] - acc[q]) / d;
        } else {
          a.y[i] = (1.0 - a.omega) * a.y[i] + (a.omega / d) * (gb[q] - acc[q]);
        }
      }
    }
  }
}

using DefaultCfg = StreamCfg<1024, 1024, 8192, 4, false, false>;

struct SellStreamArgs {
  const uint32_t* w;
  const real* v;
  const uint2* slice;
  const uint8_t* len;
  const int32_t* rowptr;
  const real* vtab;
  int32_t vtab_n;
  int32_t nrows, nslices;
  const real* x;
  const real* b;
  real* y;
};
template <int MODE, bool CODED, int B>
__global__ __launch_bounds__(kThreads) void sell_stream_kernel(SellStreamArgs a) {
  static_assert(MODE == M_SPMV || MODE == M_RESID || MODE == M_ADD, "SpMV-type passes only");
  __shared__ real s_tab[CODED ? kCodeMax : 1];
  if (CODED) {
    if ((int)threadIdx.x < a.vtab_n) s_tab[threadIdx.x] = a.vtab[threadIdx.x];
    __syncthreads();
  }
  const int s = (int)blockIdx.x * (kThreads / kWave) + __builtin_amdgcn_readfirstlane((int)(threadIdx.x >> 6));
  if (s >= a.nslices) return;
  const int lane = threadIdx.x & (kWave - 1);
  const int r = s * kWave + lane;
  const bool live = r < a.nrows;
  int len = 0;
  if (live) len = a.len ? (int)a.len[r] : a.rowptr[r + 1] - a.rowptr[r];
  const uint2 sd = a.slice[s];
  const int nit = (int)sd.y;
  const int64_t base = (int64_t)sd.x * kWave + lane;
  uint32_t w[B];
  real v[B];
#pragma unroll
  for (int e = 0; e < B; ++e) {
    w[e] = 0; v[e] = 0.0;
    if (e < nit) { w[e] = a.w[base + (int64_t)e * kWave]; if (!CODED) v[e] = a.v[base + (int64_t)e * kWave]; }
  }
  real acc = 0.0;
  for (int t = 0; t < nit; t += B) {
    uint32_t wn[B];
    real vn[B];
#pragma unroll
    for (int e = 0; e < B; ++e) {
      wn[e] = 0; vn[e] = 0.0;
      if (t + B + e < nit) { wn[e] = a.w[base + (int64_t)(t + B + e) * kWave]; if (!CODED) vn[e] = a.v[base + (int64_t)(t + B + e) * kWave]; }
    }
    real xv[B];
#pragma unroll
    for (int e = 0; e < B; ++e) {
      const uint32_t c = CODED ? (w[e] & ((1u << kCodeBits) - 1)) : w[e];
      xv[e] = t + e < len ? a.x[c] : (real)0.0;
      if (CODED) v[e] = s_tab[w[e] >> kCodeBits];
    }
#pragma unroll
    for (int e = 0; e < B; ++e)
      if (t + e < len) acc = acc + v[e] * xv[e];
#pragma unroll
    for (int e = 0; e < B; ++e) { w[e] = wn[e]; v[e] = vn[e]; }
  }
  if (!live) return;
  if (MODE == M_SPMV) a.y[r] = acc;
  else if (MODE == M_RESID) a.y[r] = a.b[r] - acc;
  else a.y[r] = a.y[r] + acc;
}
__global__ void sell_steps_kernel(const int32_t* rowptr, int nrows, int nslices, int32_t* steps) {
  const int s = blockIdx.x * blockDim.x + threadIdx.x;
  if (s >= nslices) return;
  const int r1 = min(s * kWave + kWave, nrows);
  int m = 0;
  for (int r = s * kWave; r < r1; ++r) m = max(m, rowptr[r + 1] - rowptr[r]);
  steps[s] = m;
}
__global__ void sell_stream_fill_kernel(const int32_t* rowptr, const uint32_t* w_in, const real* v_in, const uint2* slice, int nrows,
                                        int nslices, uint32_t* w, real* v, uint8_t* len8) {
  const int64_t gid = (int64_t)blockIdx.x * blockDim.x + threadIdx.x;
  const int s = (int)(gid >> 6), lane = (int)(gid & 63);
  if (s >= nslices) return;
  const uint2 sd = slice[s];
  const int r = s * kWave + lane;
  int32_t a0 = 0, len = 0;
  if (r < nrows) { a0 = rowptr[r]; len = rowptr[r + 1] - a0; if (len8) len8[r] = (uint8_t)len; }
  const int64_t base = (int64_t)sd.x * kWave + lane;
  for (int t = 0; t < (int)sd.y; ++t) {
    w[base + (int64_t)t * kWave] = t < len ? w_in[a0 + t] : 0u;
    if (v) v[base + (int64_t)t * kWave] = t < len ? v_in[a0 + t] : (real)0.0;
  }
}

__device__ __forceinline__ real seq_sum_range(const real* s, int lo, int hi, real acc) {
  int j = lo;
  if (hi - j >= 8) {
    real p[8], q[8];
#pragma unroll
    for (int e = 0; e < 8; ++e) p[e] = s[j + e];
    j += 8;
    while (hi - j >= 16) {
#pragma unroll
      for (int e = 0; e < 8; ++e) q[e] = s[j + e];
#pragma unroll
      for (int e = 0; e < 8; ++e) acc += p[e];
#pragma unroll
      for (int e = 0; e < 8; ++e) p[e] = s[j + 8 + e];
#pragma unroll
      for (int e = 0; e < 8; ++e) acc += q[e];
      j += 16;
    }
    if (hi - j >= 8) {
#pragma unroll
      for (int e = 0; e < 8; ++e) q[e] = s[j + e];
#pragma unroll
      for (int e = 0; e < 8; ++e) acc += p[e];
#pragma unroll
      for (int e = 0; e < 8; ++e) acc += q[e];
      j += 8;
    } else {
#pragma unroll
      for (int e = 0; e < 8; ++e) acc += p[e];
    }
  }
  if (j < hi) {
    real r[7];
#pragma unroll
    for (int e = 0; e < 7; ++e) r[e] = s[min(j + e, hi - 1)];
#pragma unroll
    for (int e = 0; e < 7; ++e)
      if (j + e < hi) acc += r[e];
  }
  return acc;
}
__device__ __forceinline__ real seq_sum_skip(const real* s, int lo, int hi, int dp, real acc) {
  if (dp >= lo && dp < hi) {
    acc = seq_sum_range(s, lo, dp, acc);
    return seq_sum_range(s, dp + 1, hi, acc);
  }
  return seq_sum_range(s, lo, hi, acc);
}

__global__ void gather_perm_kernel(const real* __restrict__ b, const int32_t* __restrict__ perm,
                                   real* __restrict__ bp, int n, int64_t ld_src, int64_t ld_dst) {
  b += blockIdx.y * ld_src;
  bp += blockIdx.y * ld_dst;
  for (int r = blockIdx.x * blockDim.x + threadIdx.x; r < n; r += gridDim.x * blockDim.x) bp[r] = b[perm[r]];
}
__global__ void scatter_perm_kernel(const real* __restrict__ xp, const int32_t* __restrict__ perm,
                                    real* __restrict__ x, int n, int64_t ld_src, int64_t ld_dst) {
  xp += blockIdx.y * ld_src;
  x += blockIdx.y * ld_dst;
  for (int r = blockIdx.x * blockDim.x + threadIdx.x; r < n; r += gridDim.x * blockDim.x) x[perm[r]] = xp[r];
}

__global__ void gs_flip_rhs_kernel(const real* __restrict__ bp, const real* __restrict__ diag,
                                   const real* __restrict__ xp, real* __restrict__ sp, int n, int64_t ldb, int64_t ldx,
                                   real scale) {
  bp += blockIdx.y * ldb;
  xp += blockIdx.y * ldx;
  sp += blockIdx.y * ldx;
  for (int r = blockIdx.x * blockDim.x + threadIdx.x; r < n; r += gridDim.x * blockDim.x)
    sp[r] = bp[r] - sp[r] + scale * (diag[r] * xp[r]);
}

__global__ void copy_cols_kernel(real* __restrict__ dst, const real* __restrict__ src, int n, int64_t ld_dst,
                                 int64_t ld_src) {
  dst += blockIdx.y * ld_dst;
  src += blockIdx.y * ld_src;
  for (int r = blockIdx.x * blockDim.x + threadIdx.x; r < n; r += gridDim.x * blockDim.x) dst[r] = src[r];
}

template <int BS>
__global__ void gs_flip_rhs_il_kernel(const real* __restrict__ bp, const real* __restrict__ diag, const real* __restrict__ xp,
                                      real* __restrict__ sp, int n, int64_t ldb, int64_t ldx, real scale, real* __restrict__ sil) {
  for (int r = blockIdx.x * blockDim.x + threadIdx.x; r < n; r += gridDim.x * blockDim.x) {
    const real d = diag[r];
#pragma unroll
    for (int q = 0; q < BS; ++q) {
      const real v = bp[r + q * ldb] - sp[r + q * ldx] + scale * (d * xp[r + q * ldx]);
      sp[r + q * ldx] = v;
      sil[(int64_t)r * BS + q] = v;
    }
  }
}
template <int BS>
__global__ void copy_cols_il_kernel(real* __restrict__ dst, const real* __restrict__ src, int n, int64_t ld_dst, int64_t ld_src,
                                    real* __restrict__ sil) {
  for (int r = blockIdx.x * blockDim.x + threadIdx.x; r < n; r += gridDim.x * blockDim.x) {
#pragma unroll
    for (int q = 0; q < BS; ++q) {
      const real v = src[r + q * ld_src];
      dst[r + q * ld_dst] = v;
      sil[(int64_t)r * BS + q] = v;
    }
  }
}

__device__ __forceinline__ void lds_barrier() {
  __builtin_amdgcn_fence(__ATOMIC_RELEASE, "workgroup", "local");
  __builtin_amdgcn_s_barrier();
  __builtin_amdgcn_fence(__ATOMIC_ACQUIRE, "workgroup", "local");
}

struct ChainArgs {
  const int32_t* col;
  const real* val;
  real* x;
  const real* bp;
  const real* diag;
  const i4_t* rowmeta;
  const i4_t* desc;
  real omega;
  int32_t lvl_begin;
  int32_t lvl_end;
  int32_t step;
  unsigned long long* tim;
  int64_t ldx, ldb;
};

constexpr int kChainThreads = 1024;
constexpr int kChainLds = 8192;
constexpr int kChainLdsX = 8192;

template <int PF>
struct ChainRow {
  i4_t m;
  real d, b;
  real pv[PF];
  int pc[PF];
};

template <int T, int PF>
__device__ __forceinline__ void chain_prefetch(const ChainArgs& a, const i4_t ds, int tid, ChainRow<PF>& o) {
  const int r = ds.x + tid;
  if (r < ds.y) {
    o.m = a.rowmeta[r];
    o.d = a.diag[r];
    o.b = a.bp[r];
// ... 1526 lines not shown
```

algebraicmultigrid.jl_amd/csrc/hip/csr_ops.hpp:

```cpp
#pragma once
#include <atomic>

namespace {


template <int MODE, class CFG = DefaultCfg, bool CODED = false>
int launch_stream(const StreamArgs& a0, hipStream_t st, int ncolv = 1) {
  const int nrows = a0.row_end - a0.row_begin;
  if (nrows <= 0) return AMGH_OK;
  StreamArgs a = a0;
  a.ncolv = ncolv;
  const int nb = (nrows + CFG::ROWS - 1) / CFG::ROWS;
  const int64_t grid = (CFG::XCD || ncolv > 1) ? (int64_t)((nb + kNumXcd - 1) / kNumXcd) * kNumXcd * ncolv : nb;
  hipLaunchKernelGGL((csr_stream_kernel<MODE, CFG, CODED>), dim3((unsigned)grid), dim3(CFG::THREADS), 0, st, a);
  HIP_TRY(hipGetLastError());
  return AMGH_OK;
}

constexpr int kGsBlockTarget = 256;
constexpr int kGsMinRows = 4;
constexpr int kGsNnzPerWg = 256;
template <int MODE>
int launch_gs_level(const StreamArgs& a, int rows, hipStream_t st, int ncolv = 1) {
  const int width = a.row_end - a.row_begin;
  const int avg16 = std::max(16, rows);
  rows = 256;
  while (rows > kGsMinRows && (int64_t)rows * avg16 > (int64_t)kGsNnzPerWg * 16) rows >>= 1;
  while (rows > kGsMinRows && width / rows < kGsBlockTarget && (int64_t)rows * avg16 > 16 * 64) rows >>= 1;
  switch (rows) {
    case 4: return launch_stream<MODE, StreamCfg<256, 4, 2048, 1, false, false>>(a, st, ncolv);
    case 8: return launch_stream<MODE, StreamCfg<256, 8, 2048, 1, false, false>>(a, st, ncolv);
    case 16: return launch_stream<MODE, StreamCfg<256, 16, 2048, 1, false, false>>(a, st, ncolv);
    case 32: return launch_stream<MODE, StreamCfg<256, 32, 2048, 1, false, false>>(a, st, ncolv);
    case 64: return launch_stream<MODE, StreamCfg<256, 64, 2048, 1, false, false>>(a, st, ncolv);
    case 128: return launch_stream<MODE, StreamCfg<256, 128, 2048, 1, false, false>>(a, st, ncolv);
    default: return launch_stream<MODE, StreamCfg<256, 256, 2048, 2, false, false>>(a, st, ncolv);
  }
}

using SmallCfg = StreamCfg<256, 64, 4096, 2, false, false>;
#ifndef AMGH_CODED_CFG
#define AMGH_CODED_CFG 1024, 1024, 8192, 4
#endif
using CodedCfg = StreamCfg<AMGH_CODED_CFG, false, false>;
template <int MODE>
int launch_stream_sized(const StreamArgs& a, hipStream_t st, int ncolv, bool xcd = false) {
  if (a.row_end - a.row_begin < (1 << 18)) return launch_stream<MODE, SmallCfg>(a, st, ncolv);
  if constexpr (MODE == M_SPMV) {
    if (xcd && ncolv == 1) {
      if (a.ccol && (g_stream_code || !a.col)) return launch_stream<MODE, StreamCfg<1024, 1024, 8192, 4, false, true>, true>(a, st, ncolv);
      return launch_stream<MODE, StreamCfg<1024, 1024, 8192, 4, false, true>>(a, st, ncolv);
    }
  }
  if (a.ccol && (g_stream_code || !a.col)) return launch_stream<MODE, CodedCfg, true>(a, st, ncolv);
  return launch_stream<MODE>(a, st, ncolv);
}

typedef std::conditional<sizeof(real) == 8, unsigned long long, unsigned int>::type rbits_t;
__device__ __forceinline__ rbits_t real_bits(real v) { rbits_t b; __builtin_memcpy(&b, &v, sizeof(real)); return b; }
constexpr int kCodeMiss = 4096;
__device__ __forceinline__ int code_find(const rbits_t* tab, int ntab, rbits_t v) {
  int lo = 0, hi = ntab;
  while (lo < hi) { const int mid = (lo + hi) >> 1; if (tab[mid] < v) lo = mid + 1; else hi = mid; }
  return (lo < ntab && tab[lo] == v) ? lo : -1;
}
__global__ void code_probe_kernel(const real* val, int64_t nnz, const real* tab, int ntab, unsigned* miss_cnt, real* miss) {
  __shared__ rbits_t s_tab[kCodeMax];
  if ((int)threadIdx.x < ntab) s_tab[threadIdx.x] = real_bits(tab[threadIdx.x]);
  __syncthreads();
  for (int64_t k = (int64_t)blockIdx.x * blockDim.x + threadIdx.x; k < nnz; k += (int64_t)gridDim.x * blockDim.x) {
    const real v = val[k];
    if (code_find(s_tab, ntab, real_bits(v)) >= 0) continue;
    if (__hip_atomic_load(miss_cnt, __ATOMIC_RELAXED, __HIP_MEMORY_SCOPE_AGENT) >= (unsigned)kCodeMiss) continue;
    const unsigned i = atomicAdd(miss_cnt, 1u);
    if (i < (unsigned)kCodeMiss) miss[i] = v;
  }
}
__global__ void code_encode_kernel(const int32_t* col, const real* val, int64_t nnz, const real* tab, int ntab, uint32_t* ccol) {
  __shared__ rbits_t s_tab[kCodeMax];
  if ((int)threadIdx.x < ntab) s_tab[threadIdx.x] = real_bits(tab[threadIdx.x]);
  __syncthreads();
  for (int64_t k = (int64_t)blockIdx.x * blockDim.x + threadIdx.x; k < nnz; k += (int64_t)gridDim.x * blockDim.x)
    ccol[k] = (uint32_t)col[k] | ((uint32_t)code_find(s_tab, ntab, real_bits(val[k])) << kCodeBits);
}
int code_values(const int32_t* col, const real* val, int64_t nrows, int64_t ncols, int64_t nnz, CodedCols* out, hipStream_t st,
                int64_t min_rows = (int64_t)1 << 18) {
  if (!g_stream_code || out->ccol || nrows < min_rows || ncols > ((int64_t)1 << kCodeBits) || nnz <= 0 || !col || !val) return AMGH_OK;
  unsigned* d_cnt = nullptr; real *d_miss = nullptr, *d_tab = nullptr;
  RC_TRY(dev_alloc(&d_cnt, 1));
  int rc = dev_alloc(&d_miss, kCodeMiss);
  if (rc == AMGH_OK) rc = dev_alloc(&d_tab, kCodeMax);
  std::vector<rbits_t> tab;
  std::vector<real> miss((size_t)kCodeMiss);
  bool ok = rc == AMGH_OK;
  for (int pass = 0; ok && pass < 8; ++pass) {
    const int64_t span = pass == 0 ? std::min<int64_t>(nnz, 1 << 20) : nnz;
    const int ntab = (int)tab.size();
    if (hipMemsetAsync(d_cnt, 0, 4, st) != hipSuccess) { rc = -1001; break; }
    if (ntab > 0) {
      std::vector<real> tv((size_t)ntab);
      for (int i = 0; i < ntab; ++i) std::memcpy(&tv[(size_t)i], &tab[(size_t)i], sizeof(real));
      if (hipMemcpyAsync(d_tab, tv.data(), sizeof(real) * (size_t)ntab, hipMemcpyHostToDevice, st) != hipSuccess) { rc = -1001; break; }
      if (hipStreamSynchronize(st) != hipSuccess) { rc = -1001; break; }
    }
    hipLaunchKernelGGL(code_probe_kernel, dim3((unsigned)std::min<int64_t>((span + 255) / 256, 8192)), dim3(256), 0, st, val, span, (const real*)d_tab, ntab, d_cnt, d_miss);
    unsigned cnt = 0;
    if (hipMemcpyAsync(&cnt, d_cnt, 4, hipMemcpyDeviceToHost, st) != hipSuccess || hipStreamSynchronize(st) != hipSuccess) { rc = -1001; break; }
    if (cnt == 0) { if (pass > 0) break; else continue; }
    const unsigned got = std::min<unsigned>(cnt, (unsigned)kCodeMiss);
    if (hipMemcpy(miss.data(), d_miss, sizeof(real) * got, hipMemcpyDeviceToHost) != hipSuccess) { rc = -1001; break; }
    for (unsigned i = 0; i < got; ++i) { rbits_t b; std::memcpy(&b, &miss[i], sizeof(real)); tab.push_back(b); }
    std::sort(tab.begin(), tab.end());
    tab.erase(std::unique(tab.begin(), tab.end()), tab.end());
    if ((int)tab.size() > kCodeMax) ok = false;
    if (pass == 7) ok = false;
  }
  if (rc == AMGH_OK && ok && !tab.empty()) {
    std::vector<real> tv(tab.size());
    for (size_t i = 0; i < tab.size(); ++i) std::memcpy(&tv[i], &tab[i], sizeof(real));
    rc = dev_alloc(&out->ccol, nnz + 4);
    if (rc == AMGH_OK) rc = dev_alloc(&out->vtab, kCodeMax);
    if (rc == AMGH_OK && hipMemcpyAsync(d_tab, tv.data(), sizeof(real) * tv.size(), hipMemcpyHostToDevice, st) != hipSuccess) rc = -1001;
    if (rc == AMGH_OK && hipMemcpyAsync(out->vtab, tv.data(), sizeof(real) * tv.size(), hipMemcpyHostToDevice, st) != hipSuccess) rc = -1001;
    if (rc == AMGH_OK) {
      hipLaunchKernelGGL(code_encode_kernel, dim3((unsigned)std::min<int64_t>((nnz + 255) / 256, 8192)), dim3(256), 0, st, col, val, nnz, (const real*)d_tab, (int)tab.size(), out->ccol);
      if (hipGetLastError() != hipSuccess || hipStreamSynchronize(st) != hipSuccess) rc = -1001;
    }
    if (rc == AMGH_OK) { out->n = (int)tab.size(); out->bytes = nnz * 4 + kCodeMax * kRealB; }
    else out->free_dev();
  }
  hipFree(d_cnt); hipFree(d_miss); hipFree(d_tab);
  if (rc == AMGH_ENOMEM) { (void)hipGetLastError(); out->free_dev(); return AMGH_OK; }
  return rc;
}

int sell_build(const int32_t* rowptr, const uint32_t* ccol, const int32_t* col, const real* val, int64_t nrows, int64_t nnz,
               SellCols* out, hipStream_t st) {
  if (out->w || nrows < g_sell_min_rows || nrows <= 0 || nnz <= 0 || !rowptr || (!ccol && !(col && val))) return AMGH_OK;
  const int64_t ns = (nrows + kWave - 1) / kWave;
  int32_t* d_steps = nullptr;
  RC_TRY(dev_alloc(&d_steps, ns));
  hipLaunchKernelGGL(sell_steps_kernel, dim3((unsigned)((ns + 255) / 256)), dim3(256), 0, st, rowptr, (int)nrows, (int)ns, d_steps);
  std::vector<int32_t> steps((size_t)ns);
  if (hipMemcpyAsync(steps.data(), d_steps, sizeof(int32_t) * ns, hipMemcpyDeviceToHost, st) != hipSuccess || hipStreamSynchronize(st) != hipSuccess) { hipFree(d_steps); return -1001; }
  hipFree(d_steps);
  std::vector<uint2> sd((size_t)ns);
  int64_t off = 0;
  int longest = 0;
  for (int64_t s = 0; s < ns; ++s) { sd[(size_t)s] = make_uint2((unsigned)off, (unsigned)steps[(size_t)s]); off += steps[(size_t)s]; longest = std::max(longest, steps[(size_t)s]); }
  const int64_t padded = off * kWave;
  const bool coded = ccol != nullptr;
  if (off >= ((int64_t)1 << 32) || padded * 100 > nnz * (int64_t)(g_sell_cap_pct > 0 ? g_sell_cap_pct : coded ? kSellCapPct : kSellCapPlainPct)) return AMGH_OK;
  int rc = dev_alloc(&out->w, padded);
  if (rc == AMGH_OK && !coded) rc = dev_alloc(&out->v, padded);
  if (rc == AMGH_OK) rc = dev_alloc(&out->slice, ns);
  if (rc == AMGH_OK && longest <= 255) rc = dev_alloc(&out->len8, nrows);
  if (rc == AMGH_OK && hipMemcpyAsync(out->slice, sd.data(), sizeof(uint2) * ns, hipMemcpyHostToDevice, st) != hipSuccess) rc = -1001;
  if (rc == AMGH_OK) {
    hipLaunchKernelGGL(sell_stream_fill_kernel, dim3((unsigned)((ns * kWave + 255) / 256)), dim3(256), 0, st, rowptr,
                       coded ? ccol : (const uint32_t*)col, coded ? (const real*)nullptr : val, (const uint2*)out->slice, (int)nrows, (int)ns,
                       out->w, out->v, out->len8);
    if (hipGetLastError() != hipSuccess || hipStreamSynchronize(st) != hipSuccess) rc = -1001;
  }
  if (rc != AMGH_OK) { out->free_dev(); if (rc == AMGH_ENOMEM) { (void)hipGetLastError(); return AMGH_OK; } return rc; }
  out->nslices = ns; out->padded = padded;
  out->bytes = padded * (coded ? 4 : kEntB) + ns * 8 + (out->len8 ? nrows : 0);
  return AMGH_OK;
}
bool sell_apply(int mode, const StreamArgs& a, const SellCols* sc, hipStream_t st, int ncolv, int* rc) {
  if (!sc || !sc->w || !g_sell_stream || ncolv != 1 || (!sc->v && !a.vtab)) return false;
  SellStreamArgs s{};
  s.w = sc->w; s.v = sc->v; s.slice = sc->slice; s.len = sc->len8; s.rowptr = a.rowptr; s.vtab = a.vtab; s.vtab_n = a.vtab_n;
  s.nrows = a.row_end; s.nslices = (int32_t)sc->nslices; s.x = a.x; s.b = a.b; s.y = a.y;
  const dim3 grid((unsigned)((sc->nslices + kThreads / kWave - 1) / (kThreads / kWave))), block(kThreads);
  const bool coded = sc->v == nullptr;
  const bool b8 = coded && sc->padded >= (int64_t)kSellLongSteps * kWave * sc->nslices;
#define AMGH_SELL_LAUNCH(M) \
  do { \
    if (b8) hipLaunchKernelGGL((sell_stream_kernel<M, true, 8>), grid, block, 0, st, s); \
    else if (coded) hipLaunchKernelGGL((sell_stream_kernel<M, true, 4>), grid, block, 0, st, s); \
    else hipLaunchKernelGGL((sell_stream_kernel<M, false, 4>), grid, block, 0, st, s); \
  } while (0)
  switch (mode) {
    case M_SPMV: AMGH_SELL_LAUNCH(M_SPMV); break;
    case M_RESID: AMGH_SELL_LAUNCH(M_RESID); break;
    case M_ADD: AMGH_SELL_LAUNCH(M_ADD); break;
    default: return false;
  }
#undef AMGH_SELL_LAUNCH
  ++const_cast<SellCols*>(sc)->launches;
  *rc = hipGetLastError() == hipSuccess ? AMGH_OK : -1001;
  return true;
}

int csr_apply(const amgh_csr* op, int mode, const real* x, const real* b, real* y, hipStream_t st,
              int ncolv = 1, bool sell = false) {
  StreamArgs a{};
  a.rowptr = op->rowptr; a.col = op->col; a.val = op->val;
  a.ccol = op->cc.ccol; a.vtab = op->cc.vtab; a.vtab_n = op->cc.n;
  a.x = x; a.y = y; a.b = b;
  a.row_begin = 0; a.row_end = (int32_t)op->nrows;
  a.ldx = op->ncols; a.ldy = op->nrows; a.ldb = op->nrows;
  int rc = AMGH_OK;
  if (sell && sell_apply(mode, a, &op->sc, st, ncolv, &rc)) return rc;
  switch (mode) {
    case M_SPMV: return launch_stream_sized<M_SPMV>(a, st, ncolv, op->xcd_map);
    case M_RESID: return launch_stream_sized<M_RESID>(a, st, ncolv);
    case M_ADD: return launch_stream_sized<M_ADD>(a, st, ncolv);
  }
  return AMGH_EINVAL;
}

int csr_jacobi(amgh_csr* op, real omega, const real* xin, const real* b, real* xout, hipStream_t st,
               int ncolv = 1) {
  RC_TRY(csr_ensure_diag(op, st));
  StreamArgs a{};
  a.rowptr = op->rowptr; a.col = op->col; a.val = op->val;
  a.x = xin; a.y = xout; a.b = b; a.dpos = op->dpos; a.diag = op->diag; a.omega = omega;
  a.row_begin = 0; a.row_end = (int32_t)op->nrows;
  a.ldx = op->ncols; a.ldy = op->nrows; a.ldb = op->nrows;
  return launch_stream_sized<M_JACOBI>(a, st, ncolv);
}

int csr_jacobi_zero(amgh_csr* op, real omega, const real* b, real* xout, hipStream_t st, int ncolv = 1) {
  RC_TRY(csr_ensure_diag(op, st));
  if (op->nrows > 0)
    hipLaunchKernelGGL(jacobi_zero_kernel, dim3((unsigned)std::min<int64_t>((op->nrows + 255) / 256, 1 << 20), ncolv), dim3(256), 0, st,
                       b, (const real*)op->diag, xout, (int64_t)op->nrows, omega, (int64_t)op->nrows, (int64_t)op->nrows);
  HIP_TRY(hipGetLastError());
  return AMGH_OK;
}

int csr_chebyshev(amgh_csr* op, real c1, real c2, bool first, const real* xin, const real* b, real* d, real* xout, hipStream_t st,
                  int ncolv = 1) {
  RC_TRY(csr_ensure_diag(op, st));
  StreamArgs a{};
  a.rowptr = op->rowptr; a.col = op->col; a.val = op->val;
  a.ccol = op->cc.ccol; a.vtab = op->cc.vtab; a.vtab_n = op->cc.n;
  a.x = xin; a.y = xout; a.b = b; a.diag = op->diag; a.d = d; a.c1 = c1; a.c2 = c2;
  a.row_begin = 0; a.row_end = (int32_t)op->nrows;
  a.ldx = op->ncols; a.ldy = op->nrows; a.ldb = op->nrows; a.ldd = op->nrows;
  return first ? launch_stream_sized<M_CHEB1>(a, st, ncolv) : launch_stream_sized<M_CHEB>(a, st, ncolv);
}
int csr_chebyshev_zero(amgh_csr* op, real c2, const real* b, real* d, real* xout, hipStream_t st, int ncolv = 1) {
  RC_TRY(csr_ensure_diag(op, st));
  if (op->nrows > 0)
    hipLaunchKernelGGL(cheb_zero_kernel, dim3((unsigned)std::min<int64_t>((op->nrows + 255) / 256, 1 << 20), ncolv), dim3(256), 0, st,
                       b, (const real*)op->diag, xout, d, (int64_t)op->nrows, c2, (int64_t)op->nrows, (int64_t)op->nrows, (int64_t)op->nrows);
  HIP_TRY(hipGetLastError());
  return AMGH_OK;
}
int csr_ensure_coded(amgh_csr* op, hipStream_t st) {
  if (op->cc_tried || !g_stream_code) return AMGH_OK;
  op->cc_tried = true;
  RC_TRY(code_values(op->col, op->val, op->nrows, op->ncols, op->nnz, &op->cc, st));
  op->bytes += op->cc.bytes;
  return AMGH_OK;
}

template <int T, int PF>
int launch_chain_t(const ChainArgs& c, bool sor, bool ldsx, int nx, hipStream_t st, int ncolv) {
  if (sor && ldsx) hipLaunchKernelGGL((gs_chain_kernel<true, true, T, PF>), dim3(ncolv), dim3(T), 0, st, c, nx);
  else if (sor) hipLaunchKernelGGL((gs_chain_kernel<true, false, T, PF>), dim3(ncolv), dim3(T), 0, st, c, nx);
  else if (ldsx) hipLaunchKernelGGL((gs_chain_kernel<false, true, T, PF>), dim3(ncolv), dim3(T), 0, st, c, nx);
  else hipLaunchKernelGGL((gs_chain_kernel<false, false, T, PF>), dim3(ncolv), dim3(T), 0, st, c, nx);
  HIP_TRY(hipGetLastError());
  return AMGH_OK;
}
template <int MAXK, int DIR>
int launch_wave_kd(const WaveArgs& a, bool sor, size_t lds, hipStream_t st, int ncolv) {
  static std::atomic<uint64_t> attr_set{0};
  int dev = 0;
  if (lds > 64 * 1024 && hipGetDevice(&dev) == hipSuccess && !((attr_set.load() >> (dev & 63)) & 1)) {
    (void)hipFuncSetAttribute((const void*)gs_wave_kernel<false, DIR, MAXK>, hipFuncAttributeMaxDynamicSharedMemorySize, 160 * 1024);
    (void)hipFuncSetAttribute((const void*)gs_wave_kernel<true, DIR, MAXK>, hipFuncAttributeMaxDynamicSharedMemorySize, 160 * 1024);
    attr_set.fetch_or((uint64_t)1 << (dev & 63));
  }
  if (sor) hipLaunchKernelGGL((gs_wave_kernel<true, DIR, MAXK>), dim3(ncolv), dim3(kWaveThreads), lds, st, a);
  else hipLaunchKernelGGL((gs_wave_kernel<false, DIR, MAXK>), dim3(ncolv), dim3(kWaveThreads), lds, st, a);
  HIP_TRY(hipGetLastError());
  return AMGH_OK;
}
template <int MAXK>
int launch_wave_k(const WaveArgs& a, bool sor, int dir, size_t lds, hipStream_t st, int ncolv) {
  switch (dir) {
    case 0: return launch_wave_kd<MAXK, 0>(a, sor, lds, st, ncolv);
    case 1: return launch_wave_kd<MAXK, 1>(a, sor, lds, st, ncolv);
    default: return launch_wave_kd<MAXK, 2>(a, sor, lds, st, ncolv);
  }
}
int launch_wave(const WaveArgs& a, int maxk, bool sor, int dir, size_t lds, hipStream_t st, int ncolv) {
  switch (maxk) {
    case 6: return launch_wave_k<6>(a, sor, dir, lds, st, ncolv);
    case 12: return launch_wave_k<12>(a, sor, dir, lds, st, ncolv);
    case 18: return launch_wave_k<18>(a, sor, dir, lds, st, ncolv);
    case 24: return launch_wave_k<24>(a, sor, dir, lds, st, ncolv);
    case 30: return launch_wave_k<30>(a, sor, dir, lds, st, ncolv);
    case 36: return launch_wave_k<36>(a, sor, dir, lds, st, ncolv);
  }
  return AMGH_EINVAL;
}
template <int E, int DIR>
int launch_waveq_ed(const WaveArgs& a, bool sor, size_t lds, hipStream_t st, int ncolv) {
  static std::atomic<uint64_t> attr_set{0};
  int dev = 0;
  if (lds > 64 * 1024 && hipGetDevice(&dev) == hipSuccess && !((attr_set.load() >> (dev & 63)) & 1)) {
    (void)hipFuncSetAttribute((const void*)gs_waveq_kernel<false, DIR, E>, hipFuncAttributeMaxDynamicSharedMemorySize, 160 * 1024);
    (void)hipFuncSetAttribute((const void*)gs_waveq_kernel<true, DIR, E>, hipFuncAttributeMaxDynamicSharedMemorySize, 160 * 1024);
    attr_set.fetch_or((uint64_t)1 << (dev & 63));
  }
  if (sor) hipLaunchKernelGGL((gs_waveq_kernel<true, DIR, E>), dim3(ncolv), dim3(kWaveThreads), lds, st, a);
  else hipLaunchKernelGGL((gs_waveq_kernel<false, DIR, E>), dim3(ncolv), dim3(kWaveThreads), lds, st, a);
  HIP_TRY(hipGetLastError());
  return AMGH_OK;
}
template <int E>
int launch_waveq_e(const WaveArgs& a, bool sor, int dir, size_t lds, hipStream_t st, int ncolv) {
  switch (dir) {
    case 0: return launch_waveq_ed<E, 0>(a, sor, lds, st, ncolv);
    case 1: return launch_waveq_ed<E, 1>(a, sor, lds, st, ncolv);
    default: return launch_waveq_ed<E, 2>(a, sor, lds, st, ncolv);
  }
}
int launch_waveq(const WaveArgs& a, int e, bool sor, int dir, size_t lds, hipStream_t st, int ncolv) {
  switch (e) {
    case 3: return launch_waveq_e<3>(a, sor, dir, lds, st, ncolv);
    case 5: return launch_waveq_e<5>(a, sor, dir, lds, st, ncolv);
    case 7: return launch_waveq_e<7>(a, sor, dir, lds, st, ncolv);
    case 9: return launch_waveq_e<9>(a, sor, dir, lds, st, ncolv);
  }
  return AMGH_EINVAL;
// ... 265 lines not shown
      else RC_TRY((launch_stream<M_RESID, StreamCfg<256, 64, 4096, 2, false, false>>(ra, st, ncolv)));
      const real* Xk = (const real*)((backward ? g->dti_b : g->dti_f) + g->dti_off[k]);
      constexpr int RB = 4;
      const unsigned rgrid = (unsigned)((rb + RB - 1) / RB);
      if (ncolv % 8 == 0) hipLaunchKernelGGL((tri_gemm_kernel<8, RB>), dim3(rgrid, ncolv / 8), dim3(kThreads), 0, st, Xk, (const real*)(g->blk_s + r0), x + r0, rb, backward ? 1 : 0, (int64_t)g->n, (int64_t)g->n);
      else if (ncolv % 4 == 0) hipLaunchKernelGGL((tri_gemm_kernel<4, RB>), dim3(rgrid, ncolv / 4), dim3(kThreads), 0, st, Xk, (const real*)(g->blk_s + r0), x + r0, rb, backward ? 1 : 0, (int64_t)g->n, (int64_t)g->n);
      else if (ncolv % 2 == 0) hipLaunchKernelGGL((tri_gemm_kernel<2, RB>), dim3(rgrid, ncolv / 2), dim3(kThreads), 0, st, Xk, (const real*)(g->blk_s + r0), x + r0, rb, backward ? 1 : 0, (int64_t)g->n, (int64_t)g->n);
      else hipLaunchKernelGGL(tri_gemv_kernel<1>, dim3((unsigned)rb, ncolv), dim3(kThreads), 0, st, Xk, (const real*)(g->blk_s + r0), x + r0, rb, backward ? 1 : 0, (int64_t)g->n, (int64_t)g->n);
    }
    HIP_TRY(hipGetLastError());
    return AMGH_OK;
  }
  if (g->nblk > 0 && g_gs_block_inverse && !sor) {
    g->bp_cols = 0;
    BlockArgs ba{};
    const GsSchedule::Outer& o = backward ? g->blk_b : g->blk_f;
    ba.rowptr = o.rowptr; ba.col = o.col; ba.val = o.val; ba.tinv = o.tinv; ba.diag = g->blk_diag;
    const bool single = g->nblk <= kBlkSingle;
    if (!single) {
      StreamArgs ra{};
      ra.rowptr = o.nx_rowptr; ra.col = o.nx_col; ra.val = o.nx_val;
      ra.x = x; ra.b = b; ra.y = g->blk_s;
      ra.row_begin = 0; ra.row_end = (int32_t)g->n;
      ra.ldx = g->n; ra.ldy = g->n; ra.ldb = g->n;
      RC_TRY((launch_stream<M_RESID, StreamCfg<256, 64, 4096, 2, false, false>>(ra, st, ncolv)));
    }
    ba.x = x; ba.b = single ? b : g->blk_s; ba.n = (int32_t)g->n; ba.backward = backward ? 1 : 0;
    ba.ld = g->n;
    ba.tim = g_chain_tim;
    ba.near_ptr = o.near_ptr; ba.near_pi = o.near_pi; ba.near_val = o.near_val;
    const int S = g->super > 0 ? g->super : g->nblk;
    const int nsuper = (g->nblk + S - 1) / S;
    for (int q = 0; q < nsuper; ++q) {
      const int J = backward ? nsuper - 1 - q : q;
      ba.blk0 = J * S;
      ba.nblk = std::min(S, g->nblk - ba.blk0);
      if (q > 0) {
        StreamArgs pa{};
        pa.rowptr = o.sp_rowptr; pa.col = o.sp_col; pa.val = o.sp_val;
        pa.x = x; pa.b = g->blk_s; pa.y = g->blk_s;
        pa.row_begin = ba.blk0 * kBlk; pa.row_end = (int32_t)std::min<int64_t>(g->n, (int64_t)(ba.blk0 + ba.nblk) * kBlk);
        pa.ldx = g->n; pa.ldy = g->n; pa.ldb = g->n;
        RC_TRY((launch_stream<M_RESID, StreamCfg<256, 16, 2048, 2, false, false>>(pa, st, ncolv)));
      }
      if (g_gs_block_pipe && !single) hipLaunchKernelGGL(gs_block_pipe_kernel, dim3(ncolv), dim3(kPipeThreads), 0, st, ba);
      else hipLaunchKernelGGL(gs_block_kernel, dim3(ncolv), dim3(kBlkThreads), 0, st, ba);
    }
    HIP_TRY(hipGetLastError());
    return AMGH_OK;
  }
  GsSchedule* lay = g;
  GsSchedule::Tri* tri = nullptr;
  real s_key = 0.0, flip_scale = 1.0;
  bool both_dirs = false;
  if (g_gs_merge > 1 && !sor && (backward ? g->mb : g->mf)) {
    lay = backward ? g->mb : g->mf;
    tri = backward ? &g->tri_b : &g->tri_f;
    s_key = 1.0;
    both_dirs = g->mf && g->mb;
  } else if (g_gs_merge > 1 && sor) {
    GsSchedule::SorSet* ss = sor_children(g, omega);
    if (ss && (ss->f || ss->b) && g->xstride == g->ncols && first && !x_resident) {
      HIP_TRY(hipStreamSynchronize(st));
      RC_TRY(gs_grow_xp_for_merged(g, &op->bytes));
    }
    if (ss && (backward ? ss->b : ss->f) && g->xstride > g->ncols) {
      lay = backward ? ss->b : ss->f;
      tri = backward ? &ss->tb : &ss->tf;
      s_key = omega;
      flip_scale = 2.0 - omega;
      both_dirs = ss->f && ss->b;
      sor = false;
    }
  }
  const int64_t xs = g->xstride;
  const bool il = g_gs_il && g_gs_lpr != 1 && lay != g && !g->bw.on && (ncolv == 8 || ncolv == 4 || ncolv == 2);
  if (first || !il) g->xil_cols = 0;
  bool il_s_ok = false;
  if (il && g->xil_cap < xs * ncolv) {
    HIP_TRY(hipStreamSynchronize(st));
    ++g_sched_epoch;
    hipFree(g->xil); g->xil = nullptr; g->xil_cap = 0;
    RC_TRY(dev_alloc(&g->xil, xs * ncolv));
    g->xil_cap = xs * ncolv;
    g->bytes += (int64_t)sizeof(real) * xs * ncolv; op->bytes += (int64_t)sizeof(real) * xs * ncolv;
    g->xil_cols = 0;
  }
  const bool perm_io = g_gs_flow_perm_io && ncolv == 1 && g->ncols == g->n && lay == g && !op->pipe_epoch && g_gs_bw_relay > 0 &&
                       g->bw.on && g->bw.flow.on && (g_gs_bw_flow || !g->bw.rec) &&
                       (int64_t)sizeof(real) * g->n < 0x7ffffff0ll;
  const bool fuse_b = perm_io && first && !(reuse_b && g->bp_cols == ncolv);
  const bool fuse_x = perm_io && last && !no_scatter && bw::relay_perm_x_ok<real>(g->bw.maxk, g->bw.flow.dict_on && (g_gs_bw_dict || !g->bw.flow.srec)) &&
                      ((g->bw.flow.dict_on && (g_gs_bw_dict || !g->bw.flow.srec)) ? g->bw.flow.dict_lds : g->bw.flow.lds_max) + bw::relay_perm_lds<real>(g->bw.flow.lds_max) <= 64 * 1024;
  if (first) {
    if (!(reuse_b && g->bp_cols == ncolv) && !fuse_b)
      hipLaunchKernelGGL(gather_perm_kernel, dim3(grid_for(g->n), ncolv), dim3(256), 0, st, b, g->perm, g->bp, (int)g->n,
                         (int64_t)g->n, (int64_t)g->n);
    g->bp_cols = ncolv;
    if (x_resident) {
    } else if (xzero) {
      const bool flow_zero = g_gs_flow_xzero && g->bw.on && g->bw.flow.on && (g_gs_bw_flow || !g->bw.rec) && g->ncols == g->n && lay == g;
      if (!flow_zero) {
        const int64_t cnt = xs * ncolv;
        hipLaunchKernelGGL(fill_kernel, dim3(grid_for(cnt)), dim3(256), 0, st, g->xp, cnt, 0.0);
        if (il) {
          const int64_t ci = g->ncols * ncolv;
          hipLaunchKernelGGL(fill_kernel, dim3(grid_for(ci)), dim3(256), 0, st, g->xil, ci, 0.0);
          g->xil_cols = ncolv;
        }
      }
    } else {
      hipLaunchKernelGGL(gather_perm_kernel, dim3(grid_for(g->ncols), ncolv), dim3(256), 0, st, (const real*)x, g->permx,
                         g->xp, (int)g->ncols, (int64_t)g->ncols, xs);
    }
    HIP_TRY(hipGetLastError());
  }
  real* xp = g->xp;
  const real* rhs = g->bp;
  int64_t ldb = g->n;
  if (first) g->s_dir = -1;
  if (lay != g) {
    const bool flip = g->ncols == g->n && g->diag_nonzero && both_dirs &&
                      g->s_dir == (backward ? 0 : 1) && g->s_key == s_key;
    if (flip) {
      if (il) {
        real* sil = g->xil + g->ncols * ncolv;
#define AMGH_FLIP_IL(BS_) hipLaunchKernelGGL((gs_flip_rhs_il_kernel<BS_>), dim3(grid_for(g->n)), dim3(256), 0, st, (const real*)g->bp, \
                         (const real*)lay->diag, (const real*)xp, xp + g->ncols, (int)g->n, (int64_t)g->n, xs, flip_scale, sil)
        if (ncolv == 8) AMGH_FLIP_IL(8); else if (ncolv == 4) AMGH_FLIP_IL(4); else AMGH_FLIP_IL(2);
#undef AMGH_FLIP_IL
        il_s_ok = true;
      } else
      hipLaunchKernelGGL(gs_flip_rhs_kernel, dim3(grid_for(g->n), ncolv), dim3(256), 0, st, (const real*)g->bp,
                         (const real*)lay->diag, (const real*)xp, xp + g->ncols, (int)g->n, (int64_t)g->n, xs,
                         flip_scale);
      HIP_TRY(hipGetLastError());
    } else if (first && xzero) {
      if (il) {
        real* sil = g->xil + g->ncols * ncolv;
#define AMGH_COPY_IL(BS_) hipLaunchKernelGGL((copy_cols_il_kernel<BS_>), dim3(grid_for(g->n)), dim3(256), 0, st, xp + g->ncols, \
                         (const real*)g->bp, (int)g->n, xs, (int64_t)g->n, sil)
        if (ncolv == 8) AMGH_COPY_IL(8); else if (ncolv == 4) AMGH_COPY_IL(4); else AMGH_COPY_IL(2);
#undef AMGH_COPY_IL
        il_s_ok = true;
      } else
      hipLaunchKernelGGL(copy_cols_kernel, dim3(grid_for(g->n), ncolv), dim3(256), 0, st, xp + g->ncols,
                         (const real*)g->bp, (int)g->n, xs, (int64_t)g->n);
      HIP_TRY(hipGetLastError());
    } else {
      if (!tri->rowptr && g->n > 0 && tri == (backward ? &g->tri_b : &g->tri_f)) {
        HIP_TRY(hipStreamSynchronize(st));
        const int64_t before = g->bytes;
        RC_TRY(tri_build_dev(tri, g, backward, &g->bytes, 0.0, backward ? &g->tri_nnz_b : &g->tri_nnz));
        op->bytes += g->bytes - before;
      }
      StreamArgs ra{};
      ra.rowptr = tri->rowptr; ra.col = tri->col; ra.val = tri->val;
      ra.x = xp; ra.b = g->bp; ra.y = xp + g->ncols;
      ra.row_begin = 0; ra.row_end = (int32_t)g->n;
      ra.ldx = xs; ra.ldy = xs; ra.ldb = g->n;
      RC_TRY(launch_stream<M_RESID>(ra, st, ncolv));
    }
    g->s_dir = backward ? 1 : 0;
    g->s_key = s_key;
    rhs = xp + g->ncols;
    ldb = xs;
  } else {
    g->s_dir = -1;
  }
  if (op->pipe_epoch && !(g->bw.on && g->bw.flow.on && (g_gs_bw_flow || !g->bw.rec))) return AMGH_ESTATE;
  if (g->bw.on) {
    hipError_t e = hipSuccess;
    const bool flow = g->bw.flow.on && (g_gs_bw_flow || !g->bw.rec);
    if (flow) {
      bw::FlowArgs<real> fa{g->bw.blocks, g->bw.flow.fd, g->bw.flow.srec, g->bw.flow.aux, g->bw.ext_col, g->bw.flow.fl_mb, g->bw.flow.fl_slot,
                            g->bw.flow.mbox, rhs, xp, omega, g->bw.head + 1, g->bw.nblocks, (int32_t)g->bw.flow.nmail,
                            g->bw.err, nullptr, (unsigned)g_gs_bw_spin, (int32_t)g_gs_bw_skip_pub};
      fa.ldb = ldb; fa.ldx = xs; fa.mail_stride = g->bw.flow.mail_stride;
      fa.xzero = (g_gs_flow_xzero && first && xzero && !x_resident && g->ncols == g->n) ? 1 : 0;
      if (ncolv > g->bw.flow.mcols) return AMGH_ESTATE;
      const bool dict = g->bw.flow.dict_on && (g_gs_bw_dict || !g->bw.flow.srec);
      if (op->pipe_epoch) {
        if (ncolv != 1 || !g->bw.flow.xon) return AMGH_ESTATE;
        fa.aux = g->bw.flow.xaux; fa.fl_mb = g->bw.flow.xfl_mb; fa.fl_slot = g->bw.flow.xfl_slot; fa.xlist = g->bw.flow.xlist;
        fa.epoch = op->pipe_epoch; fa.rmbox = op->pipe_rmbox; fa.grid = op->pipe_grid;
        if (dict) { fa.crec = g->bw.flow.crec; fa.dict = g->bw.flow.dict; fa.dict_ent = g->bw.flow.dict_ent; }
        e = bw::sweep_relay<real>(fa, g->bw.maxk, dict ? g->bw.flow.dict_lds : g->bw.flow.lds_max, sor, backward, st, BW_RELAY_W);
      } else if (ncolv == 1 && g_gs_bw_relay > 0) {
        constexpr int kBwGrid = 0, kBwGridLong = 512;
        fa.grid = g->bw.maxk > 6 ? (dict ? 0 : kBwGridLong) : kBwGrid;
        fa.late = (g->bw.flow.late_ok && !g_gs_bw_inorder) ? 1 : 0;
        if (dict) { fa.crec = g->bw.flow.crec; fa.dict = g->bw.flow.dict; fa.dict_ent = g->bw.flow.dict_ent; }
        if (fuse_b) { fa.perm_b = g->perm; fa.b_nat = b; }
        if (fuse_x) { fa.perm_x = g->perm; fa.x_nat = x; }
        if (fuse_b || fuse_x) {
          e = bw::sweep_relay_io<real>(fa, g->bw.maxk, dict ? g->bw.flow.dict_lds : g->bw.flow.lds_max, g->bw.flow.lds_max, sor, backward, st);
          g_perm_io_sweeps[0] += fuse_b ? 1u : 0u; g_perm_io_sweeps[1] += fuse_x ? 1u : 0u;
        } else
        e = bw::sweep_relay<real>(fa, g->bw.maxk, dict ? g->bw.flow.dict_lds : g->bw.flow.lds_max, sor, backward, st, BW_RELAY_W);
      } else {
        if (dict) {
          fa.crec = g->bw.flow.crec; fa.dict = g->bw.flow.dict; fa.dict_ent = g->bw.flow.dict_ent;
          fa.dict_lds = (int32_t)(g->bw.flow.dict_lds - g->bw.flow.lds_max);
        }
        e = bw::sweep_flow<real>(fa, g->bw.maxk, g->bw.flow.lds_max, sor, backward, st, ncolv, g_gs_bw_nc >= 0 ? g_gs_bw_nc : (fa.crec ? 3 : 2));
      }
    } else {
      bw::Args<real> ba{g->bw.blocks, g->bw.rec, g->bw.ext_col, rhs, xp, ldb, xs, omega, 0, nullptr};
      if (g_gs_bw_chain && ncolv == 1 && g->bw.flags) {
        bw::ChainArgs<real> ca{ba, backward ? g->bw.sdep_ptr : g->bw.dep_ptr, backward ? g->bw.sdep : g->bw.dep, g->bw.flags, g->bw.head,
                               g->bw.nblocks, g->bw.err};
        e = bw::sweep_chain<real>(ca, g->bw.maxk, g->bw.lds_max, sor, backward, st);
      } else {
        e = bw::sweep<real>(ba, g->bw.maxk, g->bw.launch_ptr, g->bw.lds_max, sor, backward, ncolv, st);
      }
    }
    if (e != hipSuccess) return -(1000 + (int)e);
  }
  if (il) {
    if (g->xil_cols != ncolv) RC_TRY(il_copy_rows(ncolv, xp, xs, g->xil, 0, il_s_ok ? g->ncols : xs, st));
    else if (!il_s_ok) RC_TRY(il_copy_rows(ncolv, xp, xs, g->xil, g->ncols, g->n, st));
    g->xil_cols = ncolv;
  }
  const int ns = (int)lay->segs.size();
  for (int k = 0; k < ns; ++k) {
    const GsSchedule::Seg& s = lay->segs[backward ? ns - 1 - k : k];
    if (s.chain) {
      ChainArgs c{};
      c.col = lay->col; c.val = lay->val; c.x = xp; c.bp = rhs; c.diag = lay->diag;
      c.rowmeta = lay->rowmeta; c.desc = lay->desc; c.omega = omega; c.tim = g_chain_tim;
      if (!backward) { c.lvl_begin = s.l0; c.lvl_end = s.l1; c.step = 1; }
      else { c.lvl_begin = s.l1 - 1; c.lvl_end = s.l0 - 1; c.step = -1; }
      c.ldx = xs; c.ldb = ldb;
      const int64_t nx = lay == g ? g->ncols : xs;
      const bool ldsx = nx <= kChainLdsX;
      if (lay == g && g->ww_rec && g->ncols == g->n && g_gs_tiny == 1 && !g_chain_tim && s.l0 == 0 && s.l1 == g->nlev) {
        WaveArgs wa{};
        wa.rec = g->ww_rec; wa.bp = rhs; wa.x = xp; wa.ldb = ldb; wa.ldx = xs; wa.omega = omega;
        wa.n = (int32_t)g->n; wa.steps = g->ww_steps;
        if (g->wq_rec && g_gs_wave_quad) {
          wa.rec = g->wq_rec; wa.steps = g->wq_steps;
          RC_TRY(launch_waveq(wa, g->wq_E, sor, sym_pair ? 2 : backward ? 1 : 0, g->wq_lds, st, ncolv));
          continue;
        }
        RC_TRY(launch_wave(wa, g->ww_maxk, sor, sym_pair ? 2 : backward ? 1 : 0, g->ww_lds, st, ncolv));
        continue;
      }
      if (lay == g && g->tiny_ok && g->ncols == g->n && g_gs_tiny && !g_chain_tim) {
        RC_TRY(launch_chain_tiny(c, sor, s.rows, (int)g->n, (int)g->nnz, g->nlev, st, ncolv));
        continue;
      }
      RC_TRY(launch_chain(c, sor, ldsx, s.rows, (int)nx, st, ncolv));
      if (il) RC_TRY(il_copy_rows(ncolv, xp, xs, g->xil, lay->lvl_ptr[s.l0], lay->lvl_ptr[s.l1] - lay->lvl_ptr[s.l0], st));
    } else if (s.sell_k > 0 && lay->scol && g_gs_sell) {
      SellArgs la{};
      la.scol = lay->scol; la.sval = lay->sval; la.chunk = lay->schunk; la.diag = lay->diag; la.bp = rhs; la.x = xp;
      la.omega = omega; la.row0 = lay->lvl_ptr[s.l0]; la.nrows = lay->lvl_ptr[s.l0 + 1] - lay->lvl_ptr[s.l0];
      la.chunk0 = s.sell_chunk0; la.nchunks = s.sell_nchunks;
      la.ldx = xs; la.ldb = ldb;
      const int nwg = (s.sell_nchunks + 3) / 4;
      la.xcd_map = nwg >= 768 ? 1 : 0;
      const int grid = la.xcd_map ? ((nwg + kNumXcd - 1) / kNumXcd) * kNumXcd : nwg;
      if (il && sell_il_shape(s.sell_k, ncolv)) {
        SellIlArgs ia{};
        ia.scol = la.scol; ia.sval = la.sval; ia.chunk = la.chunk; ia.diag = la.diag; ia.xil = g->xil; ia.x = xp; ia.omega = omega;
        ia.row0 = la.row0; ia.nrows = la.nrows; ia.chunk0 = la.chunk0; ia.nchunks = la.nchunks; ia.xcd_map = la.xcd_map;
        ia.soff = (int32_t)g->ncols; ia.ldx = xs;
        RC_TRY(launch_sell_il(ia, sor, s.sell_k, ncolv, grid, st));
        HIP_TRY(hipGetLastError());
        continue;
      }
      RC_TRY(launch_sell(la, sor, s.sell_k, grid, ncolv, st));
      HIP_TRY(hipGetLastError());
      if (il) RC_TRY(il_copy_rows(ncolv, xp, xs, g->xil, la.row0, la.nrows, st));
    } else if (s.nslots > 0) {
      SlotArgs sa{};
      sa.wcol = lay->wcol; sa.wval = lay->wval; sa.slot_row = lay->slot_row; sa.wmeta = lay->wmeta;
      sa.diag = lay->diag; sa.bp = rhs; sa.x = xp; sa.omega = omega; sa.slot0 = s.slot0;
      const bool xmap = s.nslots >= 768 || ncolv > 1;
      sa.nslots = s.nslots; sa.xcd_map = xmap ? 1 : 0;
      sa.ldx = xs; sa.ldb = ldb;
      if (lay->slot_entries == kBigSlot) {
        sa.ncolv = ncolv;
        const int grid = ((xmap || ncolv > 1) ? ((s.nslots + kNumXcd - 1) / kNumXcd) * kNumXcd : s.nslots) * ncolv;
        if (sor) hipLaunchKernelGGL(gs_bigslot_kernel<true>, dim3(grid), dim3(kSlot), 0, st, sa);
        else hipLaunchKernelGGL(gs_bigslot_kernel<false>, dim3(grid), dim3(kSlot), 0, st, sa);
        HIP_TRY(hipGetLastError());
        if (il) RC_TRY(il_copy_rows(ncolv, xp, xs, g->xil, lay->lvl_ptr[s.l0], lay->lvl_ptr[s.l1] - lay->lvl_ptr[s.l0], st));
        continue;
      }
      if (il) {
        SlotIlArgs ia{};
        ia.wcol = sa.wcol; ia.wval = sa.wval; ia.slot_row = sa.slot_row; ia.wmeta = sa.wmeta; ia.diag = sa.diag;
        ia.xil = g->xil; ia.x = xp; ia.omega = omega; ia.slot0 = s.slot0; ia.nslots = s.nslots;
        ia.xcd_map = s.nslots >= 768 ? 1 : 0;
        ia.soff = (int32_t)g->ncols; ia.ldx = xs;
        const int grid = ia.xcd_map ? ((s.nslots + kNumXcd - 1) / kNumXcd) * kNumXcd : s.nslots;
        RC_TRY(launch_slot_il(ia, sor, ncolv, grid, st));
        HIP_TRY(hipGetLastError());
        continue;
      }
      const int ncv = (ncolv % 8 == 0) ? 8 : (ncolv % 4 == 0) ? 4 : (ncolv % 2 == 0) ? 2 : 1;
      sa.ncolv = ncolv / ncv;
      const int grid = ((xmap || sa.ncolv > 1) ? ((s.nslots + kNumXcd - 1) / kNumXcd) * kNumXcd : s.nslots) * sa.ncolv;
      int lpr = 1;
      if (lay != g && ncolv == 1 && g_gs_lpr != 1) {
        const int avg = s.rows / 16;
        lpr = g_gs_lpr > 1 ? g_gs_lpr : (avg >= 56 ? 16 : avg >= 48 ? 8 : 1);
      }
      int ept = 1;
      if (lay != g && ncolv == 1) ept = g_gs_ept > 0 ? g_gs_ept : ((s.nslots > 1024 && lpr == 1 && s.rows / 16 < 16) ? 2 : 1);
      if (lpr > 1 || ept > 1) { RC_TRY(launch_slot_lpr(sa, sor, lpr, ept, grid, st)); HIP_TRY(hipGetLastError()); continue; }
      RC_TRY(launch_slot(sa, sor, ncv, grid, st));
      HIP_TRY(hipGetLastError());
// ... 20 lines not shown
```

include/amghip.h:

```cpp
#ifndef AMGHIP_H
#define AMGHIP_H

#include <stdint.h>

#ifdef __cplusplus
extern "C" {
#endif

#ifndef AMGH_REAL
#define AMGH_REAL double
#endif
typedef AMGH_REAL amgh_real;

typedef struct amgh_handle amgh_t;
typedef struct amgh_csr amgh_csr_t;

#define AMGH_OK 0
#define AMGH_EINVAL (-2)
#define AMGH_ESTATE (-3)
#define AMGH_ENOMEM (-4)
#define AMGH_EUNSUPPORTED (-5)

enum { AMGH_SMOOTH_NONE = 0, AMGH_SMOOTH_GS = 1, AMGH_SMOOTH_JACOBI = 2, AMGH_SMOOTH_SOR = 3, AMGH_SMOOTH_CHEBYSHEV = 4 };
enum { AMGH_SWEEP_FORWARD = 0, AMGH_SWEEP_BACKWARD = 1, AMGH_SWEEP_SYMMETRIC = 2 };
// ... 88 lines not shown
int amgh_pcg_d(amgh_t* h, const amgh_real* b_d, amgh_real* x_d, int cycle, int use_precond,
               int maxiter, double abstol, double reltol, amgh_real* resid_hist, int* iters);

int amgh_gmres(amgh_t* h, const amgh_real* b, amgh_real* x, int cycle, int use_precond, int restart,
               int maxiter, double abstol, double reltol, amgh_real* resid_hist, int* iters);
int amgh_gmres_d(amgh_t* h, const amgh_real* b_d, amgh_real* x_d, int cycle, int use_precond, int restart,
                 int maxiter, double abstol, double reltol, amgh_real* resid_hist, int* iters);
int amgh_debug_gmres_reorth(const amgh_t* h);

int amgh_pcg_block(amgh_t* h, const amgh_real* B, amgh_real* X, int cycle, int use_precond, int maxiter,
                   double abstol, double reltol, amgh_real* resid_hist, int ldh, int* iters);
int amgh_pcg_block_d(amgh_t* h, const amgh_real* B_d, amgh_real* X_d, int cycle, int use_precond, int maxiter,
                     double abstol, double reltol, amgh_real* resid_hist, int ldh, int* iters);

int amgh_level_spmv(amgh_t* h, int level, int which, const amgh_real* x, amgh_real* y);
int amgh_level_spmv_d(amgh_t* h, int level, int which, const amgh_real* x_d, amgh_real* y_d);
int amgh_level_residual_d(amgh_t* h, int level, const amgh_real* x_d, const amgh_real* b_d, amgh_real* r_d);
int amgh_level_smooth(amgh_t* h, int level, int post, amgh_real* x, const amgh_real* b);
int amgh_level_smooth_d(amgh_t* h, int level, int post, amgh_real* x_d, const amgh_real* b_d);
int amgh_debug_level_smooth_block_d(amgh_t* h, int level, int post, amgh_real* x_d, const amgh_real* b_d);

int amgh_csr_create(amgh_csr_t** op, int device, int64_t nrows, int64_t ncols,
                    const int32_t* rowptr, const int32_t* col, const amgh_real* val);
void amgh_csr_destroy(amgh_csr_t* op);
int amgh_csr_prepare(amgh_csr_t* op, int jacobi, int gs);
int amgh_csr_spmv_d(amgh_csr_t* op, const amgh_real* x_d, amgh_real* y_d, void* stream);
int amgh_csr_residual_d(amgh_csr_t* op, const amgh_real* x_d, const amgh_real* b_d, amgh_real* r_d, void* stream);
int amgh_csr_spmv_add_d(amgh_csr_t* op, const amgh_real* x_d, amgh_real* y_d, void* stream);
int amgh_csr_jacobi_d(amgh_csr_t* op, double omega, const amgh_real* xin_d, const amgh_real* b_d,
                      amgh_real* xout_d, void* stream);
int amgh_csr_chebyshev_d(amgh_csr_t* op, int degree, double lo, double hi, amgh_real* x_d, const amgh_real* b_d,
                         amgh_real* work_d, void* stream);
int amgh_csr_spectral_radius(amgh_csr_t* op, int steps, double* rho, void* stream);
int amgh_csr_gs_d(amgh_csr_t* op, int backward, double omega, int is_sor, amgh_real* x_d,
                  const amgh_real* b_d, void* stream);
#define AMGH_GS_REUSE_B 1
int amgh_csr_gs_ex_d(amgh_csr_t* op, int backward, double omega, int is_sor, amgh_real* x_d, const amgh_real* b_d,
                     void* stream, int flags);

int amgh_gather_d(int device, int64_t n, const int32_t* idx_d, const amgh_real* src_d, amgh_real* dst_d, void* stream);
int amgh_dot_d(int device, int64_t n, const amgh_real* x_d, const amgh_real* y_d, amgh_real* scratch_d, amgh_real* out,
               void* stream);

typedef struct amgh_dist amgh_dist_t;
typedef struct amgh_local_group amgh_local_group_t;
#define AMGH_DIST_ID_BYTES 128
int amgh_dist_rccl_available(void);
int amgh_dist_unique_id(void* id128);
int amgh_dist_create_rccl(amgh_dist_t** d, int device, int rank, int nranks, const void* id128);
int amgh_local_group_create(amgh_local_group_t** g, int nranks);
void amgh_local_group_destroy(amgh_local_group_t* g);
void amgh_local_group_abort(amgh_local_group_t* g);
int amgh_dist_create_local(amgh_dist_t** d, int device, int rank, amgh_local_group_t* g);
int amgh_dist_create_ipc(amgh_dist_t** d, int device, int rank, int nranks, const char* shm_name);
void amgh_dist_destroy(amgh_dist_t* d);
int amgh_dist_push_level(amgh_dist_t* d, int64_t n_global, int64_t nc_global,
                         const int64_t* row_cuts, const int64_t* crow_cuts,
                         const int32_t* A_rowptr, const int32_t* A_col, const amgh_real* A_val,
                         const int32_t* S_rowptr, const int32_t* S_col, const amgh_real* S_val,
                         const int32_t* P_rowptr, const int32_t* P_col, const amgh_real* P_val,
                         const int32_t* R_rowptr, const int32_t* R_col, const amgh_real* R_val,
                         const amgh_smoother_t* pre, const amgh_smoother_t* post);
int amgh_dist_set_tail(amgh_dist_t* d, amgh_t* tail);
int amgh_dist_set_host_tail(amgh_dist_t* d, amgh_coarse_fn fn, void* user);
int amgh_dist_finalize(amgh_dist_t* d);
int amgh_dist_set_gs_mode(amgh_dist_t* d, int mode);
int amgh_dist_gs_pipelined(const amgh_dist_t* d, int level);
int amgh_dist_pipe_serialized(const amgh_dist_t* d);
int amgh_dist_pipe_protocol_failed(const amgh_dist_t* d);
int amgh_dist_num_sharded_levels(const amgh_dist_t* d);
int amgh_dist_local_range(const amgh_dist_t* d, int level, int64_t* r0, int64_t* r1);
int amgh_dist_precond_apply_d(amgh_dist_t* d, const amgh_real* r_loc_d, amgh_real* z_loc_d, int cycle);
int amgh_dist_solve_d(amgh_dist_t* d, const amgh_real* b_loc_d, amgh_real* x_loc_d, int cycle, int maxiter,
                      double abstol, double reltol, int calculate_residual,
                      amgh_real* resid_hist , int* iters);
int amgh_dist_pcg_d(amgh_dist_t* d, const amgh_real* b_loc_d, amgh_real* x_loc_d, int cycle, int use_precond,
                    int maxiter, double abstol, double reltol, amgh_real* resid_hist , int* iters);
int amgh_dist_spmv_d(amgh_dist_t* d, int level, const amgh_real* x_loc_d, amgh_real* y_loc_d);
int amgh_dist_sync(amgh_dist_t* d);
int amgh_dist_barrier(amgh_dist_t* d);
int amgh_dist_allreduce(amgh_dist_t* d, double* v, int n, int max_op);
int amgh_dist_stats(amgh_dist_t* d, int64_t* out2, int reset);
int64_t amgh_dist_device_bytes(const amgh_dist_t* d);
void* amgh_dist_stream(amgh_dist_t* d);
int amgh_dist_plan_info(const amgh_dist_t* d, int level, int64_t* out_counts, int64_t* halo_globals,
                        int32_t* send_idx, int64_t* send_cnt_per_peer, int64_t* recv_cnt_per_peer);
int amgh_dist_plan_info2(const amgh_dist_t* d, int level, int which, int64_t* out_counts,
                         int64_t* halo_globals, int32_t* send_idx, int64_t* send_cnt_per_peer,
                         int64_t* recv_cnt_per_peer);

typedef struct amgh_dmat amgh_dmat_t;
int amgh_dmat_upload(amgh_dmat_t** M, int device, int64_t m, int64_t n, const int32_t* colptr,
                     const int32_t* rowval, const double* nzval);
int amgh_dmat_download(const amgh_dmat_t* M, int32_t* colptr, int32_t* rowval, double* nzval);
void amgh_dmat_free(amgh_dmat_t* M);
int64_t amgh_dmat_rows(const amgh_dmat_t* M);
int64_t amgh_dmat_cols(const amgh_dmat_t* M);
int64_t amgh_dmat_nnz(const amgh_dmat_t* M);
int amgh_setup_transpose(const amgh_dmat_t* A, amgh_dmat_t** At);
int amgh_dmat_equal(const amgh_dmat_t* A, const amgh_dmat_t* B, int* same);
int amgh_setup_classical_strength(const amgh_dmat_t* At, double theta, amgh_dmat_t** S, amgh_dmat_t** T,
                                  amgh_dmat_t** Sn, amgh_dmat_t** Tn);
int amgh_setup_symmetric_strength(const amgh_dmat_t* A, double theta, int bsr_flag, amgh_dmat_t** S);
int amgh_setup_fit_candidates_vector(const amgh_dmat_t* AggOp, const double* B, double tol, amgh_dmat_t** T, double* Bc);
int amgh_setup_direct_interpolation(const amgh_dmat_t* At, const amgh_dmat_t* T, const int32_t* splitting,
                                    amgh_dmat_t** R, amgh_dmat_t** P);
int amgh_setup_spgemm(const amgh_dmat_t* X, const amgh_dmat_t* Y, amgh_dmat_t** C);
int amgh_setup_jacobi_prolongation(const amgh_dmat_t* A, const amgh_dmat_t* T, double omega, amgh_dmat_t** P);

int amgh_dev_alloc(int device, int64_t bytes, void** ptr_d);
int amgh_dev_free(int device, void* ptr_d);
int amgh_dev_upload(int device, void* dst_d, const void* src, int64_t bytes);
int amgh_dev_download(int device, void* dst, const void* src_d, int64_t bytes);
int amgh_dev_sync(int device);
void* amgh_stream(amgh_t* h);

int amgh_timer_begin(amgh_t* h);
int amgh_timer_end(amgh_t* h, double* ms);
int amgh_bench_op(amgh_t* h, int level, int which, int reps, int warmup, double* avg_ms);

int amgh_profile_enable(amgh_t* h, int on);
int amgh_profile_read(amgh_t* h, double* out, int reset);

int amgh_debug_chain_timing(int enable, unsigned long long* out8);
int amgh_debug_merged_sweep_host(int64_t nrows, int64_t ncols, const int32_t* rowptr, const int32_t* col,
                                 const amgh_real* val, int m, int backward, double omega ,
                                 amgh_real* x, const amgh_real* b);

int amgh_debug_bw_sweep_host(int64_t nrows, const int32_t* rowptr, const int32_t* col, const amgh_real* val, int target_rows,
                             int backward, double omega, amgh_real* x, const amgh_real* b, int64_t* stats4);

int amgh_debug_bw_dict_sweep_host(int64_t nrows, const int32_t* rowptr, const int32_t* col, const amgh_real* val, int target_rows,
                                  int backward, amgh_real* x, const amgh_real* b, int64_t* stats5);

int amgh_debug_bw_poll_giveups(const amgh_t* h, int l);

int amgh_debug_bw_mode(const amgh_t* h, int l);
int amgh_debug_bw_dict(const amgh_t* h, int l);
int amgh_debug_bw_late(const amgh_t* h, int l);
int amgh_debug_coded_ops(const amgh_t* h, int l);

int amgh_debug_set_tunable(const char* name, int value);
int amgh_debug_get_tunable(const char* name, int* value);
int amgh_debug_set_perm_io(int on);
int amgh_debug_get_perm_io(void);
int amgh_debug_perm_io_sweeps(int which);
int amgh_debug_set_sell_stream(int on, int64_t min_rows, int cap_pct);
int amgh_debug_get_sell_stream(void);
int amgh_debug_sell_stream_launches(const amgh_t* h, int level, int which);
int64_t amgh_debug_sell_stream_padded(const amgh_t* h, int level, int which);
int64_t amgh_debug_csr_sell(amgh_csr_t* op, int coded);
int amgh_debug_csr_sell_apply(amgh_csr_t* op, int mode, const amgh_real* x_d, const amgh_real* b_d, amgh_real* y_d);
int amgh_debug_csr_sell_launches(const amgh_csr_t* op);

int amgh_set_use_graph(amgh_t* h, int on);

#ifdef __cplusplus
}
#endif
#endif
```

Before: 1.225 billion.

## Add row-reordered sliced-ELL variants with autotuned selection, extended to GS triangular operators

Adds row-permuted sliced-ELL builds, either sorted by row length within windows or sorted by source key such as the aggregate, with an optional XCD-contiguous block remap. At setup each large operator (A, R, P, and now the forward and backward Gauss-Seidel triangular residual operators) is timed as CSR-stream, plain sliced-ELL, by-length and by-source, and the fastest is kept. The aim is to cut padding and improve x-vector locality in the bandwidth-bound SpMV and smoother residual. The cost is longer setup, extra rowmap memory, and an indirect row lookup in the mapped kernel.

```diff
diff --git a/__graft_entry__.py b/__graft_entry__.py
--- a/__graft_entry__.py
+++ b/__graft_entry__.py
@@ -35,6 +35,7 @@
     hip_src.append(os.path.join(PKG, "csrc", "hip", "pcg_block_kernels.hpp"))
     hip_src.append(os.path.join(PKG, "csrc", "hip", "chebyshev.hpp"))
     hip_src.append(os.path.join(PKG, "csrc", "hip", "dist_pcg_kernels.hpp"))
+    hip_src.append(os.path.join(PKG, "csrc", "hip", "sell_order.hpp"))
     hip_src.append(os.path.join(ROOT, "include", "amghip.h"))
     hip_out = os.path.join(PKG, "libamghip.so")
     if _stale(hip_out, hip_src) and not (only_missing and os.path.exists(hip_out) and not os.path.exists(HIPCC)):
diff --git a/algebraicmultigrid.jl_amd/_libs.py b/algebraicmultigrid.jl_amd/_libs.py
--- a/algebraicmultigrid.jl_amd/_libs.py
+++ b/algebraicmultigrid.jl_amd/_libs.py
@@ -187,6 +187,10 @@
     L.amgh_debug_csr_sell.restype = i64
     L.amgh_debug_csr_sell_launches.argtypes = [vp]
     L.amgh_debug_csr_sell_apply.argtypes = [vp, C.c_int, vp, vp, vp]
+    L.amgh_debug_set_sell_order.argtypes = [C.c_int]
+    L.amgh_debug_set_sell_windows.argtypes = [i64, i64]
+    L.amgh_debug_sell_order.argtypes = [vp, C.c_int, C.c_int]
+    L.amgh_debug_csr_sell_order.argtypes = [vp]
     L.amgh_debug_bw_sweep_host.argtypes = [i64, vp, vp, vp, C.c_int, C.c_int, C.c_double, vp, vp, vp]
     L.amgh_debug_bw_dict_sweep_host.argtypes = [i64, vp, vp, vp, C.c_int, C.c_int, vp, vp, vp]
     L.amgh_debug_set_tunable.argtypes = [C.c_char_p, C.c_int]
diff --git a/algebraicmultigrid.jl_amd/csrc/hip/amghip.hip b/algebraicmultigrid.jl_amd/csrc/hip/amghip.hip
--- a/algebraicmultigrid.jl_amd/csrc/hip/amghip.hip
+++ b/algebraicmultigrid.jl_amd/csrc/hip/amghip.hip
@@ -1354,51 +1354,98 @@
       const bool cd = g_stream_code != 0;
       if (!(L->lo_ok && g && g->nblk == 0)) {
         for (amgh_csr* M : {&L->A, &L->R, &L->P})
-          if (M->rowptr) { RC_TRY(sell_build(M->rowptr, cd ? M->cc.ccol : nullptr, M->col, M->val, M->nrows, M->nnz, &M->sc, h->stream)); ws += M->sc.bytes; }
+          if (M->rowptr) { RC_TRY(sell_build_mode(M->rowptr, cd ? M->cc.ccol : nullptr, M->col, M->val, M->nrows, M->nnz, &M->sc, h->stream)); ws += M->sc.bytes; }
         continue;
       }
       if (!g->rowptr || g->compacted) continue;
-      RC_TRY(sell_build(g->rowptr, cd ? L->lo_cc.ccol : nullptr, g->col, L->lo_val ? L->lo_val : g->val, L->n, g->nnz, &L->lo_sc, h->stream));
-      RC_TRY(sell_build(L->Rp.rowptr, cd ? L->Rp.cc.ccol : nullptr, L->Rp.col, L->Rp.val, L->Rp.nrows, L->Rp.nnz, &L->Rp.sc, h->stream));
-      RC_TRY(sell_build(L->Pp.rowptr, cd ? L->Pp.cc.ccol : nullptr, L->Pp.col, L->Pp.val, L->Pp.nrows, L->Pp.nnz, &L->Pp.sc, h->stream));
+      RC_TRY(sell_build_mode(g->rowptr, cd ? L->lo_cc.ccol : nullptr, g->col, L->lo_val ? L->lo_val : g->val, L->n, g->nnz, &L->lo_sc, h->stream));
+      RC_TRY(sell_build_mode(L->Rp.rowptr, cd ? L->Rp.cc.ccol : nullptr, L->Rp.col, L->Rp.val, L->Rp.nrows, L->Rp.nnz, &L->Rp.sc, h->stream));
+      RC_TRY(sell_build_mode(L->Pp.rowptr, cd ? L->Pp.cc.ccol : nullptr, L->Pp.col, L->Pp.val, L->Pp.nrows, L->Pp.nnz, &L->Pp.sc, h->stream));
+      const bool tri_ok = (g->mf || g->mb) && g->xp && g->bp && g->xstride >= g->ncols + g->n;
+      for (int dir = 0; dir < 2 && tri_ok; ++dir) {
+        GsSchedule::Tri* t = dir ? &g->tri_b : &g->tri_f;
+        if (t->rowptr) RC_TRY(sell_build_mode(t->rowptr, nullptr, t->col, t->val, g->n, dir ? g->tri_nnz_b : g->tri_nnz, &t->sc, h->stream));
+      }
       if (L->n >= (1 << 18) && g_sell_min_rows >= ((int64_t)1 << 18)) {
         real* ty = nullptr;
         RC_TRY(dev_alloc(&ty, L->n));
         int rc = AMGH_OK;
         if (hipMemsetAsync(ty, 0, sizeof(real) * L->n, h->stream) != hipSuccess || hipMemsetAsync(L->res, 0, sizeof(real) * L->n, h->stream) != hipSuccess ||
             hipMemsetAsync(L->cx, 0, sizeof(real) * L->nc, h->stream) != hipSuccess) rc = -1001;
+        if (tri_ok && hipMemsetAsync(g->xp, 0, sizeof(real) * g->xstride, h->stream) != hipSuccess) rc = -1001;
         const real* val = L->lo_val ? L->lo_val : g->val;
         auto run = [&](int which) -> int {
           if (which == AMGH_OP_A) return raw_apply(M_RESID, g->rowptr, g->col, val, L->n, L->res, L->n, L->res, L->n, ty, L->n, h->stream, 1, &L->lo_cc, &L->lo_sc);
           if (which == AMGH_OP_R) return csr_apply(&L->Rp, M_SPMV, L->res, nullptr, L->cb, h->stream, 1, true);
-          return raw_apply(M_ADD, L->Pp.rowptr, L->Pp.col, L->Pp.val, L->n, L->cx, L->nc, nullptr, 0, ty, L->n, h->stream, 1, &L->Pp.cc, &L->Pp.sc);
+          if (which == AMGH_OP_P) return raw_apply(M_ADD, L->Pp.rowptr, L->Pp.col, L->Pp.val, L->n, L->cx, L->nc, nullptr, 0, ty, L->n, h->stream, 1, &L->Pp.cc, &L->Pp.sc);
+          const GsSchedule::Tri* t = which == kOpTriB ? &g->tri_b : &g->tri_f;
+          return raw_apply(M_RESID, t->rowptr, t->col, t->val, g->n, g->xp, g->xstride, g->bp, g->n, g->xp + g->ncols, g->xstride, h->stream, 1, nullptr, &t->sc);
         };
         const int keep = g_sell_stream;
-        for (int which : {AMGH_OP_A, AMGH_OP_R, AMGH_OP_P}) {
-          SellCols* sc = which == AMGH_OP_A ? &L->lo_sc : which == AMGH_OP_R ? &L->Rp.sc : &L->Pp.sc;
-          if (!sc->w || (which == AMGH_OP_R ? L->Rp.nrows : L->n) < (1 << 18)) continue;
-          double ms[2] = {0, 0};
-          for (int v = 0; v < 2 && rc == AMGH_OK; ++v) {
-            g_sell_stream = v;
+        for (int which : {(int)AMGH_OP_A, (int)AMGH_OP_R, (int)AMGH_OP_P, kOpTriF, kOpTriB}) {
+          GsSchedule::Tri* tri = which == kOpTriF ? &g->tri_f : which == kOpTriB ? &g->tri_b : nullptr;
+          if (tri && !(tri_ok && tri->rowptr)) continue;
+          SellCols* sc = tri ? &tri->sc : which == AMGH_OP_A ? &L->lo_sc : which == AMGH_OP_R ? &L->Rp.sc : &L->Pp.sc;
+          const amgh_csr* M = which == AMGH_OP_R ? &L->Rp : &L->Pp;
+          const int64_t nr = which == AMGH_OP_R ? L->Rp.nrows : L->n;
+          const bool small_r = which == AMGH_OP_R && nr < (1 << 18);
+          if (nr < (1 << 18) && !(small_r && g_sell_order == 1)) continue;
+          if (small_r && !sc->w) rc = sell_build(M->rowptr, cd ? M->cc.ccol : nullptr, M->col, M->val, M->nrows, M->nnz, sc, h->stream, amgh_sell::kOrderRows, 1);
+          if (rc != AMGH_OK) break;
+          if (sc->w && g_sell_order >= 2 && sc->order == std::min(g_sell_order - 1, (int)amgh_sell::kOrderSource)) continue;
+          if (!sc->w && g_sell_order != 1) continue;
+          auto time4 = [&](int on, double* ms) {
+            g_sell_stream = on;
             rc = run(which);
             if (rc == AMGH_OK && hipEventRecord(h->t0, h->stream) != hipSuccess) rc = -1001;
             for (int r = 0; r < 4 && rc == AMGH_OK; ++r) rc = run(which);
             float t = 0.f;
             if (rc == AMGH_OK && (hipEventRecord(h->t1, h->stream) != hipSuccess || hipEventSynchronize(h->t1) != hipSuccess ||
                                   hipEventElapsedTime(&t, h->t0, h->t1) != hipSuccess)) rc = -1001;
-            ms[v] = t;
+            *ms = t;
+          };
+          double ms[4] = {0, 0, 0, 0};
+          if (rc == AMGH_OK) time4(0, &ms[0]);
+          double best = 0.97 * ms[0];
+          const bool had = sc->w != nullptr;
+          if (had && rc == AMGH_OK) {
+            time4(1, &ms[1]);
+            if (rc == AMGH_OK && ms[1] < best) best = 0.97 * ms[1]; else sc->free_dev();
+          }
+          const int64_t nnz_op = tri ? (which == kOpTriB ? g->tri_nnz_b : g->tri_nnz) : which == AMGH_OP_A ? g->nnz : M->nnz;
+          for (int order = amgh_sell::kOrderLength; g_sell_order == 1 && order <= amgh_sell::kOrderSource && rc == AMGH_OK; ++order) {
+            if (order == amgh_sell::kOrderLength && had) continue;
+            if (order == amgh_sell::kOrderSource && which != AMGH_OP_R) continue;
+            SellCols cand;
+            if (tri) rc = sell_build(tri->rowptr, nullptr, tri->col, tri->val, g->n, nnz_op, &cand, h->stream, order);
+            else if (which == AMGH_OP_A) rc = sell_build(g->rowptr, cd ? L->lo_cc.ccol : nullptr, g->col, val, L->n, g->nnz, &cand, h->stream, order);
+            else rc = sell_build(M->rowptr, cd ? M->cc.ccol : nullptr, M->col, M->val, M->nrows, M->nnz, &cand, h->stream, order, small_r ? 1 : -1);
+            if (rc != AMGH_OK || !cand.w) continue;
+            std::swap(*sc, cand);
+            time4(1, &ms[1 + order]);
+            if (order == amgh_sell::kOrderSource && rc == AMGH_OK) {
+              double ms_xcd = 0;
+              sc->xcd = true;
+              time4(1, &ms_xcd);
+              if (rc == AMGH_OK && ms_xcd < 0.97 * ms[1 + order]) ms[1 + order] = ms_xcd; else sc->xcd = false;
+            }
+            if (rc == AMGH_OK && ms[1 + order] < best) best = 0.97 * ms[1 + order]; else std::swap(*sc, cand);
+            cand.free_dev();
           }
           sc->launches = 0;
           if (rc != AMGH_OK) break;
-          if (getenv("AMGH_VERBOSE")) fprintf(stderr, "[amghip] n=%lld operator %d: csr_stream_kernel %.3f ms, sliced-ELL %.3f ms\n", (long long)L->n, which, ms[0] / 4, ms[1] / 4);
-          if (!(ms[1] < 0.97 * ms[0])) sc->free_dev();
+          if (getenv("AMGH_VERBOSE"))
+            fprintf(stderr, "[amghip] n=%lld operator %d: csr_stream_kernel %.3f ms, sliced-ELL %.3f ms, by length %.3f ms, by source %.3f ms (0: not built) -> %s, padded / entries %.3f\n",
+                    (long long)L->n, which, ms[0] / 4, ms[1] / 4, ms[2] / 4, ms[3] / 4,
+                    !sc->w ? "csr" : sc->order == amgh_sell::kOrderLength ? "by length" : sc->order == amgh_sell::kOrderSource ? (sc->xcd ? "by source, XCD-contiguous" : "by source") : "sliced-ELL",
+                    (double)sc->padded / (double)std::max<int64_t>(1, nnz_op));
         }
         g_sell_stream = keep;
         if (hipStreamSynchronize(h->stream) != hipSuccess && rc == AMGH_OK) rc = -1001;
         hipFree(ty);
         RC_TRY(rc);
       }
-      ws += L->lo_sc.bytes + L->Rp.sc.bytes + L->Pp.sc.bytes;
+      ws += L->lo_sc.bytes + L->Rp.sc.bytes + L->Pp.sc.bytes + g->tri_f.sc.bytes + g->tri_b.sc.bytes;
       if (getenv("AMGH_VERBOSE"))
         fprintf(stderr, "[amghip] n=%lld sliced-ELL padded / entries: A %.3f  R %.3f  P %.3f (0: not taken)\n", (long long)L->n, (double)L->lo_sc.padded / std::max<int64_t>(1, g->nnz),
                 (double)L->Rp.sc.padded / std::max<int64_t>(1, L->Rp.nnz), (double)L->Pp.sc.padded / std::max<int64_t>(1, L->Pp.nnz));
@@ -2466,6 +2513,7 @@
   const GsSchedule* g = (L->has_S ? L->S : L->A).gs;
   if (!(L->lo_ok && g && g->nblk == 0))
     return which == AMGH_OP_A ? &L->A.sc : which == AMGH_OP_R ? &L->R.sc : which == AMGH_OP_P ? &L->P.sc : nullptr;
+  if (which == kOpTriF || which == kOpTriB) return (g->mf || g->mb) ? (which == kOpTriF ? &g->tri_f.sc : &g->tri_b.sc) : nullptr;
   return which == AMGH_OP_A ? &L->lo_sc : which == AMGH_OP_R ? &L->Rp.sc : which == AMGH_OP_P ? &L->Pp.sc : nullptr;
 }
 int amgh_debug_sell_stream_launches(const amgh_t* h, int level, int which) {
@@ -2476,6 +2524,23 @@
   const SellCols* sc = sell_of(h, level, which);
   return sc ? (sc->w ? sc->padded : 0) : -1;
 }
+int amgh_debug_set_sell_order(int mode) {
+  if (mode < 0 || mode > 4) return AMGH_EINVAL;
+  g_sell_order = mode;
+  ++g_sched_epoch;
+  return AMGH_OK;
+}
+int amgh_debug_set_sell_windows(int64_t w, int64_t ws) {
+  g_sell_w = w > 0 ? w : 0;
+  g_sell_ws = ws > 0 ? ws : 0;
+  return AMGH_OK;
+}
+static int sell_order_code(const SellCols* sc) { return !sc->w ? 0 : sc->order == amgh_sell::kOrderLength ? 2 : sc->order == amgh_sell::kOrderSource ? 3 : 1; }
+int amgh_debug_sell_order(const amgh_t* h, int level, int which) {
+  const SellCols* sc = sell_of(h, level, which);
+  return sc ? sell_order_code(sc) : -1;
+}
+int amgh_debug_csr_sell_order(const amgh_csr_t* op) { return op ? sell_order_code(&op->sc) : -1; }
 
 int64_t amgh_debug_csr_sell(amgh_csr_t* op, int coded) {
   if (!op) return AMGH_EINVAL;
@@ -2484,7 +2549,7 @@
     RC_TRY(code_values(op->col, op->val, op->nrows, op->ncols, op->nnz, &op->cc, nullptr, 1));
     op->bytes += op->cc.bytes;
   }
-  RC_TRY(sell_build(op->rowptr, coded ? op->cc.ccol : nullptr, op->col, op->val, op->nrows, op->nnz, &op->sc, nullptr));
+  RC_TRY(sell_build_mode(op->rowptr, coded ? op->cc.ccol : nullptr, op->col, op->val, op->nrows, op->nnz, &op->sc, nullptr));
   op->bytes += op->sc.bytes;
   return op->sc.w ? op->sc.padded : 0;
 }
diff --git a/algebraicmultigrid.jl_amd/csrc/hip/amghip_internal.hpp b/algebraicmultigrid.jl_amd/csrc/hip/amghip_internal.hpp
--- a/algebraicmultigrid.jl_amd/csrc/hip/amghip_internal.hpp
+++ b/algebraicmultigrid.jl_amd/csrc/hip/amghip_internal.hpp
@@ -175,6 +175,19 @@
   int64_t g = (n + threads - 1) / threads;
   return (int)std::max<int64_t>(1, std::min<int64_t>(g, 256 * 8));
 }
+
+constexpr int kSellCapPct = 130, kSellCapPlainPct = 110;
+constexpr int kSellLongSteps = 12;
+constexpr int64_t kSellW = 256, kSellWs = 0;
+struct SellCols {
+  uint32_t* w = nullptr; real* v = nullptr; uint2* slice = nullptr; uint8_t* len8 = nullptr;
+  uint32_t* rowmap = nullptr;
+  int order = 0;
+  bool xcd = false;
+  int64_t nslices = 0, padded = 0, bytes = 0;
+  unsigned launches = 0;
+  void free_dev() { hipFree(w); hipFree(v); hipFree(slice); hipFree(len8); hipFree(rowmap); w = nullptr; v = nullptr; slice = nullptr; len8 = nullptr; rowmap = nullptr; order = 0; xcd = false; nslices = padded = bytes = 0; }
+};
 
 struct GsSchedule {
   int nlev = 0;
@@ -263,7 +276,7 @@
   double dti_cond = 0.0;
   GsSchedule* mf = nullptr;
   GsSchedule* mb = nullptr;
-  struct Tri { int32_t* rowptr = nullptr; int32_t* col = nullptr; real* val = nullptr; };
+  struct Tri { int32_t* rowptr = nullptr; int32_t* col = nullptr; real* val = nullptr; SellCols sc; };
   Tri dtri_f, dtri_b;
   Tri tri_f, tri_b;
   int merge_f = 1, merge_b = 1;
@@ -277,7 +290,7 @@
   void free_dev() {
     for (GsSchedule** c : {&mf, &mb})
       if (*c) { (*c)->free_dev(); delete *c; *c = nullptr; }
-    for (Tri* t : {&tri_f, &tri_b}) { hipFree(t->rowptr); hipFree(t->col); hipFree(t->val); *t = Tri(); }
+    for (Tri* t : {&tri_f, &tri_b}) { hipFree(t->rowptr); hipFree(t->col); hipFree(t->val); t->sc.free_dev(); *t = Tri(); }
     for (SorSet& ss : sor) {
       for (GsSchedule** c : {&ss.f, &ss.b})
         if (*c) { (*c)->free_dev(); delete *c; *c = nullptr; }
@@ -322,15 +335,6 @@
   uint32_t* ccol = nullptr; real* vtab = nullptr; int n = 0;
   int64_t bytes = 0;
   void free_dev() { hipFree(ccol); hipFree(vtab); ccol = nullptr; vtab = nullptr; n = 0; bytes = 0; }
-};
-
-constexpr int kSellCapPct = 130, kSellCapPlainPct = 110;
-constexpr int kSellLongSteps = 12;
-struct SellCols {
-  uint32_t* w = nullptr; real* v = nullptr; uint2* slice = nullptr; uint8_t* len8 = nullptr;
-  int64_t nslices = 0, padded = 0, bytes = 0;
-  unsigned launches = 0;
-  void free_dev() { hipFree(w); hipFree(v); hipFree(slice); hipFree(len8); w = nullptr; v = nullptr; slice = nullptr; len8 = nullptr; nslices = padded = bytes = 0; }
 };
 
 struct amgh_csr {
@@ -380,6 +384,9 @@
 int g_sell_stream = 1;
 int64_t g_sell_min_rows = (int64_t)1 << 18;
 int g_sell_cap_pct = 0;
+int g_sell_order = 1;
+constexpr int kOpTriF = 8, kOpTriB = 9;
+int64_t g_sell_w = 0, g_sell_ws = 0;
 unsigned int g_perm_io_sweeps[2] = {0, 0};
 int g_gs_bw_two_min_rows = 200000;
 int g_gs_sell = 1;
diff --git a/algebraicmultigrid.jl_amd/csrc/hip/amghip_kernels.hpp b/algebraicmultigrid.jl_amd/csrc/hip/amghip_kernels.hpp
--- a/algebraicmultigrid.jl_amd/csrc/hip/amghip_kernels.hpp
+++ b/algebraicmultigrid.jl_amd/csrc/hip/amghip_kernels.hpp
@@ -297,8 +297,11 @@
   const real* x;
   const real* b;
   real* y;
+  const uint32_t* rowmap;
+  int32_t xcd;
 };
-template <int MODE, bool CODED, int B>
+constexpr uint32_t kSellNoRow = 0xFFFFFFFFu;
+template <int MODE, bool CODED, int B, bool MAPPED = false>
 __global__ __launch_bounds__(kThreads) void sell_stream_kernel(SellStreamArgs a) {
   static_assert(MODE == M_SPMV || MODE == M_RESID || MODE == M_ADD, "SpMV-type passes only");
   __shared__ real s_tab[CODED ? kCodeMax : 1];
@@ -306,13 +309,23 @@
     if ((int)threadIdx.x < a.vtab_n) s_tab[threadIdx.x] = a.vtab[threadIdx.x];
     __syncthreads();
   }
-  const int s = (int)blockIdx.x * (kThreads / kWave) + __builtin_amdgcn_readfirstlane((int)(threadIdx.x >> 6));
+  int wg = (int)blockIdx.x;
+  if (MAPPED && a.xcd) wg = xcd_block(wg, (a.nslices + kThreads / kWave - 1) / (kThreads / kWave));
+  const int s = wg * (kThreads / kWave) + __builtin_amdgcn_readfirstlane((int)(threadIdx.x >> 6));
   if (s >= a.nslices) return;
   const int lane = threadIdx.x & (kWave - 1);
-  const int r = s * kWave + lane;
-  const bool live = r < a.nrows;
+  int r = s * kWave + lane;
+  bool live = r < a.nrows;
   int len = 0;
-  if (live) len = a.len ? (int)a.len[r] : a.rowptr[r + 1] - a.rowptr[r];
+  if (MAPPED) {
+    const int slot = r;
+    const uint32_t m = a.rowmap[slot];
+    live = m != kSellNoRow;
+    r = (int)m;
+    if (live) len = a.len ? (int)a.len[slot] : a.rowptr[r + 1] - a.rowptr[r];
+  } else {
+    if (live) len = a.len ? (int)a.len[r] : a.rowptr[r + 1] - a.rowptr[r];
+  }
   const uint2 sd = a.slice[s];
   const int nit = (int)sd.y;
   const int64_t base = (int64_t)sd.x * kWave + lane;
@@ -349,6 +362,12 @@
   if (MODE == M_SPMV) a.y[r] = acc;
   else if (MODE == M_RESID) a.y[r] = a.b[r] - acc;
   else a.y[r] = a.y[r] + acc;
+}
+__global__ void sell_key_kernel(const int32_t* rowptr, const uint32_t* w_in, int nrows, uint32_t mask, uint32_t* key) {
+  const int r = blockIdx.x * blockDim.x + threadIdx.x;
+  if (r >= nrows) return;
+  const int32_t a0 = rowptr[r];
+  key[r] = rowptr[r + 1] > a0 ? (w_in[a0] & mask) : 0u;
 }
 __global__ void sell_steps_kernel(const int32_t* rowptr, int nrows, int nslices, int32_t* steps) {
   const int s = blockIdx.x * blockDim.x + threadIdx.x;
@@ -359,14 +378,17 @@
   steps[s] = m;
 }
 __global__ void sell_stream_fill_kernel(const int32_t* rowptr, const uint32_t* w_in, const real* v_in, const uint2* slice, int nrows,
-                                        int nslices, uint32_t* w, real* v, uint8_t* len8) {
+                                        int nslices, uint32_t* w, real* v, uint8_t* len8, const uint32_t* rowmap) {
   const int64_t gid = (int64_t)blockIdx.x * blockDim.x + threadIdx.x;
   const int s = (int)(gid >> 6), lane = (int)(gid & 63);
   if (s >= nslices) return;
   const uint2 sd = slice[s];
-  const int r = s * kWave + lane;
+  const int slot = s * kWave + lane;
+  const uint32_t m = rowmap ? rowmap[slot] : (slot < nrows ? (uint32_t)slot : kSellNoRow);
+  const int r = (int)m;
   int32_t a0 = 0, len = 0;
-  if (r < nrows) { a0 = rowptr[r]; len = rowptr[r + 1] - a0; if (len8) len8[r] = (uint8_t)len; }
+  if (m != kSellNoRow) { a0 = rowptr[r]; len = rowptr[r + 1] - a0; if (len8) len8[rowmap ? slot : r] = (uint8_t)len; }
+  else if (len8 && rowmap) len8[slot] = 0;
   const int64_t base = (int64_t)sd.x * kWave + lane;
   for (int t = 0; t < (int)sd.y; ++t) {
     w[base + (int64_t)t * kWave] = t < len ? w_in[a0 + t] : 0u;
diff --git a/algebraicmultigrid.jl_amd/csrc/hip/csr_ops.hpp b/algebraicmultigrid.jl_amd/csrc/hip/csr_ops.hpp
--- a/algebraicmultigrid.jl_amd/csrc/hip/csr_ops.hpp
+++ b/algebraicmultigrid.jl_amd/csrc/hip/csr_ops.hpp
@@ -1,5 +1,6 @@
 #pragma once
 #include <atomic>
+#include "sell_order.hpp"
 
 namespace {
 
@@ -135,48 +136,87 @@
 }
 
 int sell_build(const int32_t* rowptr, const uint32_t* ccol, const int32_t* col, const real* val, int64_t nrows, int64_t nnz,
-               SellCols* out, hipStream_t st) {
-  if (out->w || nrows < g_sell_min_rows || nrows <= 0 || nnz <= 0 || !rowptr || (!ccol && !(col && val))) return AMGH_OK;
+               SellCols* out, hipStream_t st, int order = amgh_sell::kOrderRows, int64_t min_rows = -1) {
+  if (out->w || nrows < (min_rows >= 0 ? min_rows : g_sell_min_rows) || nrows <= 0 || nnz <= 0 || !rowptr || (!ccol && !(col && val))) return AMGH_OK;
   const int64_t ns = (nrows + kWave - 1) / kWave;
-  int32_t* d_steps = nullptr;
-  RC_TRY(dev_alloc(&d_steps, ns));
-  hipLaunchKernelGGL(sell_steps_kernel, dim3((unsigned)((ns + 255) / 256)), dim3(256), 0, st, rowptr, (int)nrows, (int)ns, d_steps);
-  std::vector<int32_t> steps((size_t)ns);
-  if (hipMemcpyAsync(steps.data(), d_steps, sizeof(int32_t) * ns, hipMemcpyDeviceToHost, st) != hipSuccess || hipStreamSynchronize(st) != hipSuccess) { hipFree(d_steps); return -1001; }
-  hipFree(d_steps);
+  const bool coded = ccol != nullptr;
+  std::vector<int32_t> steps;
+  amgh_sell::RowOrder ro;
+  if (order == amgh_sell::kOrderRows) {
+    int32_t* d_steps = nullptr;
+    RC_TRY(dev_alloc(&d_steps, ns));
+    hipLaunchKernelGGL(sell_steps_kernel, dim3((unsigned)((ns + 255) / 256)), dim3(256), 0, st, rowptr, (int)nrows, (int)ns, d_steps);
+    steps.resize((size_t)ns);
+    if (hipMemcpyAsync(steps.data(), d_steps, sizeof(int32_t) * ns, hipMemcpyDeviceToHost, st) != hipSuccess || hipStreamSynchronize(st) != hipSuccess) { hipFree(d_steps); return -1001; }
+    hipFree(d_steps);
+  } else {
+    std::vector<int32_t> hrp((size_t)nrows + 1);
+    if (hipMemcpyAsync(hrp.data(), rowptr, sizeof(int32_t) * (nrows + 1), hipMemcpyDeviceToHost, st) != hipSuccess || hipStreamSynchronize(st) != hipSuccess) return -1001;
+    if (order == amgh_sell::kOrderLength) {
+      amgh_sell::order_by_length(hrp.data(), nrows, g_sell_w > 0 ? g_sell_w : kSellW, &ro);
+    } else {
+      uint32_t* d_key = nullptr;
+      RC_TRY(dev_alloc(&d_key, nrows));
+      hipLaunchKernelGGL(sell_key_kernel, dim3((unsigned)((nrows + 255) / 256)), dim3(256), 0, st, rowptr, coded ? ccol : (const uint32_t*)col, (int)nrows,
+                         coded ? (1u << kCodeBits) - 1 : 0xFFFFFFFFu, d_key);
+      std::vector<uint32_t> key((size_t)nrows);
+      if (hipMemcpyAsync(key.data(), d_key, sizeof(uint32_t) * nrows, hipMemcpyDeviceToHost, st) != hipSuccess || hipStreamSynchronize(st) != hipSuccess) { hipFree(d_key); return -1001; }
+      hipFree(d_key);
+      amgh_sell::order_by_source(hrp.data(), key.data(), nrows, g_sell_ws > 0 ? g_sell_ws : kSellWs, &ro);
+    }
+    steps.swap(ro.steps);
+  }
   std::vector<uint2> sd((size_t)ns);
   int64_t off = 0;
   int longest = 0;
   for (int64_t s = 0; s < ns; ++s) { sd[(size_t)s] = make_uint2((unsigned)off, (unsigned)steps[(size_t)s]); off += steps[(size_t)s]; longest = std::max(longest, steps[(size_t)s]); }
   const int64_t padded = off * kWave;
-  const bool coded = ccol != nullptr;
   if (off >= ((int64_t)1 << 32) || padded * 100 > nnz * (int64_t)(g_sell_cap_pct > 0 ? g_sell_cap_pct : coded ? kSellCapPct : kSellCapPlainPct)) return AMGH_OK;
+  const bool mapped = order != amgh_sell::kOrderRows;
+  const int64_t nlen = mapped ? ns * kWave : nrows;
   int rc = dev_alloc(&out->w, padded);
   if (rc == AMGH_OK && !coded) rc = dev_alloc(&out->v, padded);
   if (rc == AMGH_OK) rc = dev_alloc(&out->slice, ns);
-  if (rc == AMGH_OK && longest <= 255) rc = dev_alloc(&out->len8, nrows);
+  if (rc == AMGH_OK && longest <= 255) rc = dev_alloc(&out->len8, nlen);
+  if (rc == AMGH_OK && mapped) rc = dev_alloc(&out->rowmap, ns * kWave);
   if (rc == AMGH_OK && hipMemcpyAsync(out->slice, sd.data(), sizeof(uint2) * ns, hipMemcpyHostToDevice, st) != hipSuccess) rc = -1001;
+  if (rc == AMGH_OK && mapped && hipMemcpyAsync(out->rowmap, ro.map.data(), sizeof(uint32_t) * ns * kWave, hipMemcpyHostToDevice, st) != hipSuccess) rc = -1001;
   if (rc == AMGH_OK) {
     hipLaunchKernelGGL(sell_stream_fill_kernel, dim3((unsigned)((ns * kWave + 255) / 256)), dim3(256), 0, st, rowptr,
                        coded ? ccol : (const uint32_t*)col, coded ? (const real*)nullptr : val, (const uint2*)out->slice, (int)nrows, (int)ns,
-                       out->w, out->v, out->len8);
+                       out->w, out->v, out->len8, (const uint32_t*)out->rowmap);
     if (hipGetLastError() != hipSuccess || hipStreamSynchronize(st) != hipSuccess) rc = -1001;
   }
   if (rc != AMGH_OK) { out->free_dev(); if (rc == AMGH_ENOMEM) { (void)hipGetLastError(); return AMGH_OK; } return rc; }
-  out->nslices = ns; out->padded = padded;
-  out->bytes = padded * (coded ? 4 : kEntB) + ns * 8 + (out->len8 ? nrows : 0);
-  return AMGH_OK;
+  out->nslices = ns; out->padded = padded; out->order = order;
+  out->bytes = padded * (coded ? 4 : kEntB) + ns * 8 + (out->len8 ? nlen : 0) + (mapped ? ns * kWave * 4 : 0);
+  return AMGH_OK;
+}
+int sell_build_mode(const int32_t* rowptr, const uint32_t* ccol, const int32_t* col, const real* val, int64_t nrows, int64_t nnz,
+                    SellCols* out, hipStream_t st) {
+  if (g_sell_order >= 2 && !out->w) {
+    RC_TRY(sell_build(rowptr, ccol, col, val, nrows, nnz, out, st, std::min(g_sell_order - 1, (int)amgh_sell::kOrderSource)));
+    out->xcd = out->w && g_sell_order == 4;
+  }
+  return sell_build(rowptr, ccol, col, val, nrows, nnz, out, st);
 }
 bool sell_apply(int mode, const StreamArgs& a, const SellCols* sc, hipStream_t st, int ncolv, int* rc) {
   if (!sc || !sc->w || !g_sell_stream || ncolv != 1 || (!sc->v && !a.vtab)) return false;
   SellStreamArgs s{};
   s.w = sc->w; s.v = sc->v; s.slice = sc->slice; s.len = sc->len8; s.rowptr = a.rowptr; s.vtab = a.vtab; s.vtab_n = a.vtab_n;
-  s.nrows = a.row_end; s.nslices = (int32_t)sc->nslices; s.x = a.x; s.b = a.b; s.y = a.y;
-  const dim3 grid((unsigned)((sc->nslices + kThreads / kWave - 1) / (kThreads / kWave))), block(kThreads);
+  s.nrows = a.row_end; s.nslices = (int32_t)sc->nslices; s.x = a.x; s.b = a.b; s.y = a.y; s.rowmap = sc->rowmap; s.xcd = (sc->rowmap && sc->xcd) ? 1 : 0;
+  const int64_t nwg = (sc->nslices + kThreads / kWave - 1) / (kThreads / kWave);
+  const dim3 grid((unsigned)(s.xcd ? (nwg + kNumXcd - 1) / kNumXcd * kNumXcd : nwg)), block(kThreads);
   const bool coded = sc->v == nullptr;
   const bool b8 = coded && sc->padded >= (int64_t)kSellLongSteps * kWave * sc->nslices;
+  const bool mapped = sc->rowmap != nullptr;
 #define AMGH_SELL_LAUNCH(M) \
   do { \
+    if (mapped) { \
+      if (b8) hipLaunchKernelGGL((sell_stream_kernel<M, true, 8, true>), grid, block, 0, st, s); \
+      else if (coded) hipLaunchKernelGGL((sell_stream_kernel<M, true, 4, true>), grid, block, 0, st, s); \
+      else hipLaunchKernelGGL((sell_stream_kernel<M, false, 4, true>), grid, block, 0, st, s); \
+    } else \
     if (b8) hipLaunchKernelGGL((sell_stream_kernel<M, true, 8>), grid, block, 0, st, s); \
     else if (coded) hipLaunchKernelGGL((sell_stream_kernel<M, true, 4>), grid, block, 0, st, s); \
     else hipLaunchKernelGGL((sell_stream_kernel<M, false, 4>), grid, block, 0, st, s); \
@@ -748,6 +788,10 @@
         HIP_TRY(hipStreamSynchronize(st));
         const int64_t before = g->bytes;
         RC_TRY(tri_build_dev(tri, g, backward, &g->bytes, 0.0, backward ? &g->tri_nnz_b : &g->tri_nnz));
+        if (ncolv == 1 && (g_sell_order >= 2 || g_sell_min_rows < ((int64_t)1 << 18))) {
+          RC_TRY(sell_build_mode(tri->rowptr, nullptr, tri->col, tri->val, g->n, backward ? g->tri_nnz_b : g->tri_nnz, &tri->sc, st));
+          g->bytes += tri->sc.bytes;
+        }
         op->bytes += g->bytes - before;
       }
       StreamArgs ra{};
@@ -755,7 +799,9 @@
       ra.x = xp; ra.b = g->bp; ra.y = xp + g->ncols;
       ra.row_begin = 0; ra.row_end = (int32_t)g->n;
       ra.ldx = xs; ra.ldy = xs; ra.ldb = g->n;
-      RC_TRY(launch_stream<M_RESID>(ra, st, ncolv));
+      int src = AMGH_OK;
+      if (sell_apply(M_RESID, ra, &tri->sc, st, ncolv, &src)) RC_TRY(src);
+      else RC_TRY(launch_stream<M_RESID>(ra, st, ncolv));
     }
     g->s_dir = backward ? 1 : 0;
     g->s_key = s_key;
diff --git a/algebraicmultigrid.jl_amd/csrc/hip/sell_order.hpp b/algebraicmultigrid.jl_amd/csrc/hip/sell_order.hpp
--- /dev/null
+++ b/algebraicmultigrid.jl_amd/csrc/hip/sell_order.hpp
@@ -0,0 +1,99 @@
+#pragma once
+#include <algorithm>
+#include <cstdint>
+#include <vector>
+
+namespace amgh_sell {
+
+constexpr uint32_t kNoRow = 0xFFFFFFFFu;
+constexpr int kSlice = 64;
+enum { kOrderRows = 0, kOrderLength = 1, kOrderSource = 2 };
+
+struct RowOrder {
+  std::vector<uint32_t> map;
+  std::vector<int32_t> steps;
+  std::vector<uint8_t> len8;
+  int longest = 0;
+};
+
+inline int64_t round_window(int64_t w, int64_t nrows) {
+  if (w <= 0 || w >= nrows) return std::max<int64_t>(kSlice, (nrows + kSlice - 1) / kSlice * kSlice);
+  return (w + kSlice - 1) / kSlice * kSlice;
+}
+
+inline void finish_order(const int32_t* rowptr, RowOrder* o) {
+  const int64_t ns = (int64_t)o->map.size() / kSlice;
+  o->steps.assign((size_t)ns, 0);
+  o->len8.assign(o->map.size(), 0);
+  o->longest = 0;
+  for (int64_t s = 0; s < ns; ++s) {
+    int m = 0;
+    for (int l = 0; l < kSlice; ++l) {
+      const uint32_t r = o->map[(size_t)(s * kSlice + l)];
+      if (r == kNoRow) continue;
+      const int len = rowptr[r + 1] - rowptr[r];
+      o->len8[(size_t)(s * kSlice + l)] = (uint8_t)std::min(len, 255);
+      m = std::max(m, len);
+    }
+    o->steps[(size_t)s] = m;
+    o->longest = std::max(o->longest, m);
+  }
+}
+
+inline void sort_by_length(const int32_t* rowptr, uint32_t* slot, int64_t n, std::vector<uint32_t>* tmp) {
+  int64_t cnt[257] = {0};
+  auto bucket = [&](uint32_t r) { return r == kNoRow ? 256 : 255 - std::min(rowptr[r + 1] - rowptr[r], 255); };
+  for (int64_t i = 0; i < n; ++i) ++cnt[bucket(slot[i])];
+  int64_t at = 0;
+  for (int b = 0; b < 257; ++b) { const int64_t c = cnt[b]; cnt[b] = at; at += c; }
+  tmp->resize((size_t)n);
+  for (int64_t i = 0; i < n; ++i) (*tmp)[(size_t)cnt[bucket(slot[i])]++] = slot[i];
+  std::copy(tmp->begin(), tmp->begin() + n, slot);
+}
+
+inline void order_by_length(const int32_t* rowptr, int64_t nrows, int64_t w, RowOrder* o) {
+  const int64_t W = round_window(w, nrows);
+  const int64_t nslot = (nrows + kSlice - 1) / kSlice * kSlice;
+  o->map.assign((size_t)nslot, kNoRow);
+  for (int64_t r = 0; r < nrows; ++r) o->map[(size_t)r] = (uint32_t)r;
+  std::vector<uint32_t> tmp;
+  for (int64_t a = 0; a < nrows; a += W) sort_by_length(rowptr, o->map.data() + a, std::min(W, nrows - a), &tmp);
+  finish_order(rowptr, o);
+}
+
+inline void order_by_source(const int32_t* rowptr, const uint32_t* key, int64_t nrows, int64_t ws, RowOrder* o) {
+  const int64_t W = round_window(ws, nrows);
+  const int64_t nslot = (nrows + kSlice - 1) / kSlice * kSlice;
+  o->map.assign((size_t)nslot, kNoRow);
+  uint32_t kmax = 0;
+  for (int64_t r = 0; r < nrows; ++r)
+    if (rowptr[r + 1] > rowptr[r]) kmax = std::max(kmax, key[r]);
+  const uint64_t kempty = (uint64_t)kmax + 1;
+  int bits = 1;
+  while ((kempty >> bits) != 0) ++bits;
+  constexpr int kDigit = 11;
+  std::vector<uint64_t> a, b;
+  for (int64_t w0 = 0; w0 < nrows; w0 += W) {
+    const int64_t n = std::min(W, nrows - w0);
+    a.resize((size_t)n); b.resize((size_t)n);
+    for (int64_t i = 0; i < n; ++i) {
+      const int64_t r = w0 + i;
+      const uint64_t k = rowptr[r + 1] > rowptr[r] ? (uint64_t)key[r] : kempty;
+      a[(size_t)i] = (k << 32) | (uint64_t)r;
+    }
+    for (int sh = 0; sh < bits; sh += kDigit) {
+      int64_t cnt[1 << kDigit] = {0};
+      for (int64_t i = 0; i < n; ++i) ++cnt[(a[(size_t)i] >> (32 + sh)) & ((1u << kDigit) - 1)];
+      int64_t at = 0;
+      for (int d = 0; d < (1 << kDigit); ++d) { const int64_t c = cnt[d]; cnt[d] = at; at += c; }
+      for (int64_t i = 0; i < n; ++i) b[(size_t)cnt[(a[(size_t)i] >> (32 + sh)) & ((1u << kDigit) - 1)]++] = a[(size_t)i];
+      a.swap(b);
+    }
+    for (int64_t i = 0; i < n; ++i) o->map[(size_t)(w0 + i)] = (uint32_t)(a[(size_t)i] & 0xFFFFFFFFu);
+  }
+  std::vector<uint32_t> tmp;
+  for (int64_t s = 0; s < nslot; s += kSlice) sort_by_length(rowptr, o->map.data() + s, kSlice, &tmp);
+  finish_order(rowptr, o);
+}
+
+}
diff --git a/include/amghip.h b/include/amghip.h
--- a/include/amghip.h
+++ b/include/amghip.h
@@ -264,6 +264,10 @@
 int64_t amgh_debug_csr_sell(amgh_csr_t* op, int coded);
 int amgh_debug_csr_sell_apply(amgh_csr_t* op, int mode, const amgh_real* x_d, const amgh_real* b_d, amgh_real* y_d);
 int amgh_debug_csr_sell_launches(const amgh_csr_t* op);
+int amgh_debug_set_sell_order(int mode);
+int amgh_debug_set_sell_windows(int64_t w, int64_t ws);
+int amgh_debug_sell_order(const amgh_t* h, int level, int which);
+int amgh_debug_csr_sell_order(const amgh_csr_t* op);
 
 int amgh_set_use_graph(amgh_t* h, int on);
 
```

Result: no change. 1.233 billion, median of 6 (+0.6%).
